# sp-uhh/disentangled-vae

Measured on AMD Instinct MI355X. Metric: spectrogram frames/sec (train step), M2 VAE 513-bin, higher is better.
Workload: dtype bf16x3; 1 GPU; M2 VAE train step (fwd+ELBO+bwd+Adam), x_dim 513, y_dim 513, z 16, h [128,128], 8192 frames/step/GPU, 16 kHz / 1024-pt STFT power frames; parallelism=dp1, min_hbm_bytes_per_frame=4168

## Files before the change

### disentangled-vae_amd/csrc/rows_common.hpp

```cpp
#pragma once
#include "fused_tiles.hpp"
#include "apply_types.hpp"
#include "../../include/dvae_train.h"

namespace dvae {
namespace fused {

__device__ __forceinline__ void philox_normal4(unsigned long long seed, unsigned long long frame, unsigned long long step, unsigned draw,
                                               float (&out)[4]) {
    unsigned c0 = (unsigned)frame, c1 = (unsigned)(frame >> 32), c2 = (unsigned)step, c3 = ((unsigned)(step >> 32) << 8) | draw;
    unsigned k0 = (unsigned)seed, k1 = (unsigned)(seed >> 32);
#pragma unroll
    for (int r = 0; r < 10; ++r) {
        const unsigned h0 = __umulhi(0xD2511F53u, c0), l0 = 0xD2511F53u * c0;
        const unsigned h1 = __umulhi(0xCD9E8D57u, c2), l1 = 0xCD9E8D57u * c2;
        c0 = h1 ^ c1 ^ k0; c1 = l1; c2 = h0 ^ c3 ^ k1; c3 = l0;
        k0 += 0x9E3779B9u; k1 += 0xBB67AE85u;
    }
    const float u0 = ((float)(c0 >> 8) + 0.5f) * (1.f / 16777216.f), u1 = ((float)(c1 >> 8) + 0.5f) * (1.f / 16777216.f);
    const float u2 = ((float)(c2 >> 8) + 0.5f) * (1.f / 16777216.f), u3 = ((float)(c3 >> 8) + 0.5f) * (1.f / 16777216.f);
    const float ra = sqrtf(-2.f * __logf(u0)), rb = sqrtf(-2.f * __logf(u2));
    float sa, ca, sb, cb;
    __sincosf(6.283185307179586f * u1, &sa, &ca);
    __sincosf(6.283185307179586f * u3, &sb, &cb);
    out[0] = ra * ca; out[1] = ra * sa; out[2] = rb * cb; out[3] = rb * sb;
}
__device__ __forceinline__ void frame_noise8(unsigned long long seed, unsigned long long frame, unsigned long long step, int h, float (&e)[8]) {
    float a[4], b[4];
    philox_normal4(seed, frame, step, 2u * h, a);
    philox_normal4(seed, frame, step, 2u * h + 1u, b);
#pragma unroll
    for (int j = 0; j < 4; ++j) { e[j] = a[j]; e[4 + j] = b[j]; }
}

struct RowsArgs {
    const float* x; const float* y; const float* eps;
    int ldx, ldy, ydim;
    int fastx, fasty;
    int64_t B, Bp;
    unsigned long long rng_seed, rng_step;
    const int64_t* rows;
    int64_t n_rows;
    int* bad_rows;
    int ntiles;
    float invB, elbo_eps;
    const void *W1s, *W2s, *Wmvs, *W3s, *W4s, *W5s, *W5t, *W4t, *W3zt, *Wmvt, *W2t;
    const float *b1, *b2, *bmu, *blv, *b3, *b4, *b5;
    const float* w5last;
    void *xT, *yT, *h1T, *h2T, *dh1T, *dh2T, *dmlvT, *zT, *d1T, *d2T, *dd1T, *dd2T, *daT;
    const void* wcopy; int64_t wcopy_bytes;
    int64_t spl;
    unsigned wpl_bytes;
    const void *Wc1s, *Wc2s, *Wc2t, *Wa1s, *Wa1t, *Wa2s, *Wa2t;
    const float *bc1, *bc2, *wc3, *bc3, *ba1, *ba2, *wa3, *ba3;
    void *c1T, *c2T, *dc1T, *dc2T, *dc3T, *a1T, *a2T, *da1T, *da2T, *da3T;
    float alpha, beta, gamma;
    int mode;
    float *out_r, *out_mu, *out_lv, *out_z;
    const float *g_r, *g_mu, *g_lv, *g_z;
    int ld_r, ld_gr;
    double* partials;
    unsigned long long* dbg;
    int ablate;
    int stash_inputs;
    unsigned* ylo_epoch; unsigned launch_id; int ylo_skip; int* ylo_dirty;
    DeferArgs defer;
};

#ifdef DVAE_FINE_STAMPS
#define DVAE_FSTAMP(i) do { if (g.dbg && tid == 0) g.dbg[(size_t)blockIdx.x * 32 + (i)] = wall_clock64(); } while (0)
#else
#define DVAE_FSTAMP(i) do { } while (0)
#endif
#define DVAE_STAMP(i) do { if (g.dbg && tid == 0) g.dbg[(size_t)blockIdx.x * 32 + (i)] = wall_clock64(); } while (0)


typedef short s16x4 __attribute__((ext_vector_type(4)));
__device__ __forceinline__ s16x4 lds_tr16(const __bf16* p) {
    return __builtin_amdgcn_ds_read_tr16_b64_v4i16((__attribute__((address_space(3))) s16x4*)(p));
}

#ifndef R2_STASH_AUX
#define R2_STASH_AUX 16
#endif
template <typename Frag>
__device__ __forceinline__ void stash_store16(void* base_uniform, int voff_bytes, const Frag& f) {
#if R2_STASH_AUX == 0
    *reinterpret_cast<Frag*>((char*)base_uniform + voff_bytes) = f;
#else
    typedef unsigned int u32x4_ __attribute__((ext_vector_type(4)));
    const __amdgpu_buffer_rsrc_t rs = __builtin_amdgcn_make_buffer_rsrc(base_uniform, 0, 0x7fffffff, 0x00020000);
    __builtin_amdgcn_raw_buffer_store_b128(__builtin_bit_cast(u32x4_, f), rs, voff_bytes, 0, R2_STASH_AUX);
#endif
}

template <typename P, bool SRC16 = false>
__device__ __forceinline__ void stash_tile(const typename P::T* lds, int ldl, int fbase, typename P::T* stash_tile_ptr, int64_t spl,
                                           int64_t b0, int l31, int h, float scale = 1.f, int col_limit = 1 << 30, int nplanes = P::NP) {
    typedef typename P::T T;
    typedef typename P::Frag Frag;
    constexpr int E = P::E;
    if (stash_tile_ptr == nullptr) return;
    T* const dbase = stash_tile_ptr + (b0 / P::KSTEP) * (64 * E);
    if constexpr (sizeof(T) == 2) {
        const int i16 = l31 & 15, q = i16 >> 2, pp = i16 & 3, cg = l31 >> 4;
        const T* blk = lds + q * ldl + fbase + 16 * cg + 4 * pp;
        const bool keep = fbase + l31 < col_limit;
        typedef short s16x8 __attribute__((ext_vector_type(8)));
#pragma unroll
        for (int i = 0; i < TB / (2 * E); ++i) {
            const int gq = h + 2 * i;
            Frag f[P::NP];
#pragma unroll
            for (int pl = 0; pl < P::NP; ++pl) {
                const T* bp = blk + pl * Pl<P>::lds;
                const s16x4 r0 = lds_tr16(bp + (8 * gq) * ldl), r1 = lds_tr16(bp + (8 * gq + 4) * ldl);
                s16x8 raw = {r0[0], r0[1], r0[2], r0[3], r1[0], r1[1], r1[2], r1[3]};
                f[pl] = __builtin_bit_cast(Frag, raw);
            }
            if constexpr (SRC16 && P::NP == 2) {
#pragma unroll
                for (int j = 0; j < E; ++j) {
                    const float v = (X16::val(f[0][j]) + X16::val(f[1][j])) * X16::XINV;
                    f[0][j] = P::cvt(v); f[1][j] = P::cvt(v - (float)f[0][j]);
                }
            } else
            if (scale != 1.f) {
#pragma unroll
                for (int j = 0; j < E; ++j) {
                    if constexpr (P::NP == 2) {
                        const float v = ((float)f[0][j] + (float)f[1][j]) * scale;
                        f[0][j] = P::cvt(v); f[1][j] = P::cvt(v - (float)f[0][j]);
                    } else f[0][j] = P::cvt((float)f[0][j] * scale);
                }
            }
            if (!keep) {
#pragma unroll
                for (int pl = 0; pl < P::NP; ++pl)
#pragma unroll
                    for (int j = 0; j < E; ++j) f[pl][j] = P::cvt(0.f);
            }
            stash_store16(dbase, (l31 * E + gq * 32 * E) * (int)sizeof(T), f[0]);
            if constexpr (P::NP == 2) { if (nplanes == 2) stash_store16(dbase + spl, (l31 * E + gq * 32 * E) * (int)sizeof(T), f[1]); }
        }
    } else {
#pragma unroll
        for (int i = 0; i < TB / (2 * E); ++i) {
            const int gq = h + 2 * i;
            Frag f;
#pragma unroll
            for (int j = 0; j < E; ++j) {
                const T v = lds[(gq * E + j) * ldl + fbase + l31];
                f[j] = scale == 1.f ? v : P::cvt((float)v * scale);
                if (fbase + l31 >= col_limit) f[j] = P::cvt(0.f);
            }
            stash_store16(dbase, (l31 * E + gq * 32 * E) * (int)sizeof(T), f);
        }
    }
}

template <typename P, bool F16 = false, typename RowOf>
__device__ __forceinline__ void load_rows_to_lds(const float* __restrict__ src, int ld, int ncols, int pcols, int64_t b0, int64_t B,
                                                 typename P::T* U, int ldu, int tid, RowOf rowof, float* xf = nullptr,
                                                 float* log2sum = nullptr, float eps = 0.f) {
    const int total = TB * pcols;
    for (int idx = tid; idx < total; idx += 256) {
        const int row = idx / pcols, col = idx - row * pcols;
        float v = 0.f;
        if (col < ncols && b0 + row < B) {
            v = src[rowof(row) * ld + col];
            if (log2sum && col < XD - 1) *log2sum += __builtin_amdgcn_logf(v + eps);
        }
        if constexpr (F16 && P::NP == 2) {
            const float vs = v * X16::XS;
            const typename P::T vh = X16::hi<typename P::T>(vs);
            U[row * ldu + col] = vh;
            U[Pl<P>::lds + row * ldu + col] = X16::hi<typename P::T>(vs - X16::val(vh));
        } else {
            const typename P::T vh = P::cvt(v);
            U[row * ldu + col] = vh;
            if constexpr (P::NP == 2) U[Pl<P>::lds + row * ldu + col] = P::cvt(v - (float)vh);
        }
        if (xf && col < ncols) xf[row * ncols + col] = v;
    }
}

constexpr int NQ513 = 17;
struct __attribute__((packed, aligned(4))) F4U { f32x4 v; };
#ifndef R2_IN_NT
#define R2_IN_NT 0
#endif
typedef f32x4 f32x4_a4 __attribute__((aligned(4)));
__device__ __forceinline__ f32x4 ld_in4(const float* p) {
#if R2_IN_NT >= 1
    return __builtin_nontemporal_load(reinterpret_cast<const f32x4_a4*>(p));
#else
    return reinterpret_cast<const F4U*>(p)->v;
#endif
}
__device__ __forceinline__ f32x4 ld_in4_again(const float* p) {
#if R2_IN_NT >= 2
    return __builtin_nontemporal_load(reinterpret_cast<const f32x4_a4*>(p));
#else
    return reinterpret_cast<const F4U*>(p)->v;
#endif
}
template <int I0, int I1, typename RowOf>
__device__ __forceinline__ void tile513_issue_part(const float* __restrict__ base, RowOf rowof, f32x4 (&v)[NQ513], int tid) {
#pragma unroll
    for (int i = I0; i < I1; ++i) {
        const int c = tid + 256 * i;
        v[i] = ld_in4(base + rowof(c >> 7) * XD + 4 * (c & 127));
    }
}
template <typename RowOf>
__device__ __forceinline__ void tile513_issue_last(const float* __restrict__ base, RowOf rowof, f32x4 (&v)[NQ513], int tid) {
    v[16][0] = base[rowof(tid & 31) * XD + XD - 1];
}
template <typename RowOf>
__device__ __forceinline__ void tile513_issue(const float* __restrict__ base, RowOf rowof, f32x4 (&v)[NQ513], int tid) {
    tile513_issue_part<0, 16>(base, rowof, v, tid);
    tile513_issue_last(base, rowof, v, tid);
    __builtin_amdgcn_sched_barrier(0);
}
template <typename P, int I0, int I1, bool F16 = false>
__device__ __forceinline__ void tile513_commit_part(const f32x4 (&v)[NQ513], typename P::T* U, int ldu, int tid, float* xf, unsigned long long& lo_bits) {
    typedef typename P::Pack4 Pack4;
#pragma unroll
    for (int i = I0; i < I1; ++i) {
        const int c = tid + 256 * i;
        const int row = c >> 7, col = 4 * (c & 127);
        if (xf) {
            float* d = xf + row * XD + col;
            d[0] = v[i][0]; d[1] = v[i][1]; d[2] = v[i][2]; d[3] = v[i][3];
        }
        if constexpr (F16 && P::NP == 2) {
            Pack4 pk, pl;
#pragma unroll
            for (int j = 0; j < 4; ++j) {
                const float vs = v[i][j] * X16::XS;
                pk[j] = X16::hi<typename P::T>(vs);
                pl[j] = X16::hi<typename P::T>(vs - X16::val(pk[j]));
            }
            *reinterpret_cast<Pack4*>(U + row * ldu + col) = pk;
            *reinterpret_cast<Pack4*>(U + Pl<P>::lds + row * ldu + col) = pl;
            continue;
        }
        Pack4 pk;
        pk[0] = P::cvt(v[i][0]); pk[1] = P::cvt(v[i][1]); pk[2] = P::cvt(v[i][2]); pk[3] = P::cvt(v[i][3]);
        *reinterpret_cast<Pack4*>(U + row * ldu + col) = pk;
        if constexpr (P::NP == 2) {
            Pack4 pl;
            pl[0] = P::cvt(v[i][0] - (float)pk[0]); pl[1] = P::cvt(v[i][1] - (float)pk[1]);
            pl[2] = P::cvt(v[i][2] - (float)pk[2]); pl[3] = P::cvt(v[i][3] - (float)pk[3]);
            *reinterpret_cast<Pack4*>(U + Pl<P>::lds + row * ldu + col) = pl;
            lo_bits |= __builtin_bit_cast(unsigned long long, pl) & 0x7fff7fff7fff7fffull;
        }
    }
}
template <typename P, int PCOLS, bool F16 = false>
__device__ __forceinline__ void tile513_commit_last(const f32x4 (&v)[NQ513], typename P::T* U, int ldu, int tid, float* xf, unsigned long long& lo_bits) {
    constexpr int PADC = PCOLS - XD;
    if (tid < TB) {
        if (xf) xf[tid * XD + XD - 1] = v[16][0];
        if constexpr (F16 && P::NP == 2) {
            const float vs = v[16][0] * X16::XS;
            const typename P::T vh = X16::hi<typename P::T>(vs);
            U[tid * ldu + XD - 1] = vh;
            U[Pl<P>::lds + tid * ldu + XD - 1] = X16::hi<typename P::T>(vs - X16::val(vh));
        } else {
        const typename P::T vh = P::cvt(v[16][0]);
        U[tid * ldu + XD - 1] = vh;
        if constexpr (P::NP == 2) {
            const typename P::T vl = P::cvt(v[16][0] - (float)vh);
            U[Pl<P>::lds + tid * ldu + XD - 1] = vl;
            if ((float)vl != 0.f) lo_bits |= 1ull;
        }
        }
    }
    for (int idx = tid; idx < TB * PADC; idx += 256) {
        const int r = idx / PADC, c = XD + idx - r * PADC;
        U[r * ldu + c] = P::cvt(0.f);
        if constexpr (P::NP == 2) U[Pl<P>::lds + r * ldu + c] = P::cvt(0.f);
    }
}
template <typename P, int PCOLS, bool F16 = false>
__device__ __forceinline__ void tile513_commit(const f32x4 (&v)[NQ513], typename P::T* U, int ldu, int tid, float* xf = nullptr, bool* any_lo = nullptr) {
    unsigned long long lo_bits = 0ull;
    tile513_commit_part<P, 0, 16, F16>(v, U, ldu, tid, xf, lo_bits);
    tile513_commit_last<P, PCOLS, F16>(v, U, ldu, tid, xf, lo_bits);
    if (any_lo) *any_lo = lo_bits != 0ull;
}
template <typename P, int Q0, int Q1, typename RowOf>
__device__ __forceinline__ void xstash_reload(const float* __restrict__ src, int ld, RowOf rowof, int64_t b0, int64_t B, typename P::T* xT,
                                              int64_t spl, int64_t Bp, int tid) {
    typedef typename P::Frag Frag;
    static_assert(P::NP == 2 && P::E == 8, "x stash by reload: split-bf16 planes");
    if (xT == nullptr) return;
    const int w = tid >> 6, lane = tid & 63;
    int64_t ro[8];
    bool live[8];
#pragma unroll
    for (int k = 0; k < 8; ++k) { ro[k] = rowof(8 * w + k) * (int64_t)ld; live[k] = b0 + 8 * w + k < B; }
    const int64_t kst = (b0 / P::KSTEP + (w >> 1)) * (64 * P::E) + (w & 1) * 32 * P::E;
    float v[Q1 - Q0][8];
#pragma unroll
    for (int q = Q0; q < Q1; ++q)
#pragma unroll
        for (int k = 0; k < 8; ++k) {
            const int f = 64 * q + lane;
            v[q - Q0][k] = src[ro[k] + (f < XD ? f : XD - 1)];
        }
    __builtin_amdgcn_sched_barrier(0);
#pragma unroll
    for (int q = Q0; q < Q1; ++q) {
        const int f = 64 * q + lane;
        if (q == 8 && lane >= 32) continue;
        Frag fh, fl;
#pragma unroll
        for (int k = 0; k < 8; ++k) {
            const float x = (f < XD && live[k]) ? v[q - Q0][k] : 0.f;
            fh[k] = P::cvt(x);
            fl[k] = P::cvt(x - (float)fh[k]);
        }
        const int64_t o = (int64_t)(f >> 5) * 32 * Bp + kst + (f & 31) * P::E;
        stash_store16(xT, (int)(o * (int64_t)sizeof(typename P::T)), fh);
        stash_store16(xT + spl, (int)(o * (int64_t)sizeof(typename P::T)), fl);
    }
}
__device__ __forceinline__ float tile513_log2sum(const f32x4 (&v)[NQ513], float eps, int tid) {
    float s0 = 0.f, s1 = 0.f;
#pragma unroll
    for (int i = 0; i < 16; ++i) {
        s0 += __builtin_amdgcn_logf(v[i][0] + eps) + __builtin_amdgcn_logf(v[i][1] + eps);
        s1 += __builtin_amdgcn_logf(v[i][2] + eps) + __builtin_amdgcn_logf(v[i][3] + eps);
    }
    return s0 + s1;
}

template <typename P, bool SRC16 = false>
__device__ __forceinline__ void stash_from_lds(const typename P::T* U, int ldu, int pcols, int srows, typename P::T* stash, int64_t spl,
                                               int64_t Bp, int64_t b0, int tid, int ft0 = 0, int ft1 = 1 << 30, int nplanes = P::NP) {
    typedef typename P::Frag Frag;
    constexpr int E = P::E;
    if constexpr (sizeof(typename P::T) == 2) {
        const int lane = tid & 63, wave = __builtin_amdgcn_readfirstlane(tid >> 6);
        const int fte = ft1 < srows / 32 ? ft1 : srows / 32;
        for (int ft = ft0 + wave; ft < fte; ft += 4)
            stash_tile<P, SRC16>(U, ldu, 32 * ft, stash + (int64_t)ft * 32 * Bp, spl, b0, lane & 31, lane >> 5, 1.f, pcols, nplanes);
        return;
    }
    constexpr int groups = TB / E;
    const int total = srows * groups;
    for (int idx = tid; idx < total; idx += 256) {
        const int gi = idx / srows, f = idx - gi * srows;
        Frag p;
#pragma unroll
        for (int j = 0; j < E; ++j) p[j] = (f < pcols) ? U[(gi * E + j) * ldu + f] : P::cvt(0.f);
        *reinterpret_cast<Frag*>(stash + (int64_t)(f >> 5) * 32 * Bp + (b0 / P::KSTEP) * (64 * E) + (gi * 32 + (f & 31)) * E) = p;
    }
}


static int current_device() { int dev = 0; (void)hipGetDevice(&dev); return dev < 0 || dev >= 64 ? 0 : dev; }
static inline bool is_bf(int precision) { return precision == DVAE_PREC_BF16 || precision == DVAE_PREC_BF16X3; }
template <typename F>
static auto with_policy(int precision, F&& f) {
    if (precision == DVAE_PREC_BF16X3) return f(PolX3{});
    if (precision == DVAE_PREC_BF16) return f(PolBF16{});
    return f(PolF32{});
}

int launch_rows1(int precision, int model, int y_dim, const RowsArgs& a, int grid, hipStream_t s);
int launch_noise(unsigned long long seed, unsigned long long step, int64_t B, float* out, hipStream_t s);
int launch_rows2(int precision, int model, int y_dim, const RowsArgs& a, int grid, hipStream_t s);
bool rows2_supported(int precision, int model);
int launch_rows3(int model, int y_dim, const RowsArgs& a, int grid, hipStream_t s);
bool rows3_supported(int precision, int model);

}
}
```

### disentangled-vae_amd/csrc/rows_helper.inc

```
        const int hw = wave_u - ROWS_CHAIN_WAVES, ht = tid - 64 * ROWS_CHAIN_WAVES;
        constexpr bool XFH = P::XF16 && NP == 2;
        constexpr int NBT = Ld<T>::nbias;
        constexpr int NB = (NBT + 255) / 256;
        float bvv[NB];
        auto load_bias = [&]() __attribute__((always_inline)) {
#pragma unroll
            for (int q = 0; q < NB; ++q) {
                int i = ht + 256 * q;
                i = i < NBT ? i : NBT - 1;
                const float* src;
                int k;
                if (i < OB2) { src = g.b1; k = i; }
                else if (i < OBMV) { src = g.b2; k = i - OB2; }
                else if (i < OBMV + ZD) { src = g.bmu; k = i - OBMV; }
                else if (i < OB3) { src = g.blv; k = i - OBMV - ZD; }
                else if (i < OB4) { src = g.b3; k = i - OB3; }
                else if (i < OB5) { src = g.b4; k = i - OB4; }
                else if (i < OB5 + NO) { src = g.b5; k = i - OB5; k = k < XD ? k : XD - 1; }
                else { src = g.w5last; k = i - OB5 - NO; }
                if constexpr (DEFER) bvv[q] = __hip_atomic_load(src + k, __ATOMIC_RELAXED, __HIP_MEMORY_SCOPE_AGENT);
                else bvv[q] = src[k];
            }
        };
        auto store_bias = [&]() __attribute__((always_inline)) {
#pragma unroll
            for (int q = 0; q < NB; ++q) {
                const int i = ht + 256 * q;
                if (i < NBT) Bias[i] = (i >= OB5 + XD && i < OB5 + NO) ? 0.f : bvv[q];
            }
        };
        if constexpr (!DEFER) load_bias();
        auto fill_rows = [&](int tl_, int half) {
            if (ht < TB) {
                const int64_t bf = (int64_t)tl_ * TB + ht;
                const int64_t br = bf < g.B ? bf : g.B - 1;
                int64_t r = g.rows[br];
                if (r < 0 || r >= g.n_rows) { r = 0; if (g.bad_rows && bf < g.B) atomicAdd(g.bad_rows, 1); }
                rowsrc[half * TB + ht] = r;
            }
        };
        typedef Sched<P, YP, YENC, (OFFL ? P::PDO : P::PD), INFO> SCc;
        typedef HSched<P, YP, YENC, DH, INFO> HS;
        typedef WStream<P, HS, DH> HWS;
        HWS hws;
        if constexpr (HS::any) {
            hws.rs = __builtin_amdgcn_make_buffer_rsrc(const_cast<void*>(g.wcopy), 0, (int)g.wcopy_bytes, 0x00020000);
            hws.voff = lane * 16;
            hws.pl = g.wpl_bytes;
            auto mo = [&](const void* Wp) { return (unsigned)((const char*)Wp - (const char*)g.wcopy); };
            constexpr unsigned FBB = HS::FBB;
            const unsigned tw = (unsigned)hw * FBB;
            hws.sb[H_W1X] = mo(g.W1s) + tw + (unsigned)SCc::NX1 * 4u * FBB;
            hws.sb[H_W3Y] = mo(g.W3s) + tw + (unsigned)(ZD / KS) * 4u * FBB;
            hws.sb[H_W3Z] = mo(g.W3s) + tw;
            hws.sb[H_PAD] = mo(g.W1s);
            if constexpr (INFO) { hws.sb[H_C1] = mo(g.Wc1s) + tw;  hws.sb[H_C2] = mo(g.Wc2s) + tw;  hws.sb[H_C2T] = mo(g.Wc2t) + tw; }
            else { hws.sb[H_C1] = hws.sb[H_C2] = hws.sb[H_C2T] = 0; }
            if constexpr (INFO) hws.fill();
        }
        const T* const Urh = U + l31 * LDU + h * E;
        const T* const Zbrh = Zb + l31 * LDZ + h * E;
        float lsum2 = 0.f;
        f32x4 xv[NQ513], yv[NQ513];
        bool x_in_regs = false;
        bool y_in_regs = false;
        const bool st1 = MODE != 1 && !(g.ablate & 1), st2 = MODE != 1 && !(g.ablate & 2) && (g.stash_inputs & 2), st2x = MODE != 1 && !(g.ablate & 2) && (g.stash_inputs & 1);
        for (int it = 0; it < ntl; ++it) {
            const int tile = tile0 + it * (int)gridDim.x;
            const int64_t b0 = (int64_t)tile * TB;
            const bool full = (b0 + TB) <= g.B;
            const int64_t* const rsrc = rowsrc + (it & 1) * TB;
            auto rowof = [&](int r) -> int64_t {
                if (gather) return rsrc[r];
                const int64_t br = b0 + r;
                return br < g.B ? br : g.B - 1;
            };
            int tl = ht;
            asm volatile("" : "+v"(tl));
            const bool yfast = Y513 && g.fasty && full;
            bool y_early = it > 0 && y_in_regs;
            if (it == 0) {
                if (gather) { fill_rows(tile, 0); wg_barrier(); }
                if (g.fastx && full) {
                    tile513_issue(g.x, rowof, xv, tl);
                    if constexpr (!DEFER) store_bias();
#if R2_EARLY_Y
                    if (YP > 0 && Y513 && g.fasty) {
                        unsigned long long lb = 0ull;
                        static_for<0, 4>([&](auto qc) {
                            constexpr int Q = decltype(qc)::value;
                            tile513_issue_part<4 * Q, 4 * Q + 4>(g.y, rowof, yv, tl);
                            __builtin_amdgcn_sched_barrier(0);
                            tile513_commit_part<P, 4 * Q, 4 * Q + 4, XFH>(xv, U, LDU, tl, nullptr, lb);
                            __builtin_amdgcn_sched_barrier(0);
                        });
                        tile513_issue_last(g.y, rowof, yv, tl);
                        __builtin_amdgcn_sched_barrier(0);
                        tile513_commit_last<P, ROWS_XP, XFH>(xv, U, LDU, tl, nullptr, lb);
                        y_early = true;
                    } else
#endif
                    {
                        tile513_commit<P, ROWS_XP, XFH>(xv, U, LDU, tl);
#pragma unroll
                        for (int i = 0; i < NQ513; ++i) yv[i] = f32x4{0.f, 0.f, 0.f, 0.f};
                    }
                } else {
#pragma unroll
                    for (int i = 0; i < NQ513; ++i) { xv[i] = f32x4{0.f, 0.f, 0.f, 0.f}; yv[i] = f32x4{0.f, 0.f, 0.f, 0.f}; }
                    if constexpr (!DEFER) store_bias();
                    load_rows_to_lds<P, XFH>(g.x, g.ldx, XD, ROWS_XP, b0, g.B, U, LDU, tl, rowof, nullptr, OFFL ? &lsum2 : nullptr, g.elbo_eps);
                }
                if constexpr (INFO) {
                    for (int i = ht; i < 6 * HD + 2; i += 256) {
                        const int q = i / HD, k = i - q * HD;
                        float v;
                        if (q == 0) v = g.bc1[k]; else if (q == 1) v = g.bc2[k]; else if (q == 2) v = g.wc3[k];
                        else if (q == 3) v = g.ba1[k]; else if (q == 4) v = g.ba2[k]; else if (q == 5) v = g.wa3[k];
                        else v = k == 0 ? g.bc3[0] : g.ba3[0];
                        Binfo[i] = v;
                    }
                }
                if (ht == 0) flags[0] = 0;
                if constexpr (DEFER) {
                    wg_barrier();
                    load_bias();
                    store_bias();
                }
                wg_barrier();
                if constexpr (OFFL) { if (g.fastx && full) lsum2 += tile513_log2sum(xv, g.elbo_eps, tl); }
            }
            if constexpr (HS::n(H_W1X) > 0) {
                f32x16 hacc;
                zero_acc<P>(hacc);
                hws.fill();
                gemm_seg<P, HS, DH, H_W1X, HWS, XFH>(hacc, hws, Urh + SCc::NX1 * 2 * E);
#pragma unroll
                for (int r = 0; r < 16; ++r) keep[r * 256 + ht] = XFH ? hacc[r] * X16::ACC : hacc[r];
            }
            float c1r[16], c2r[16], w3c[16];
            float bce_c = 0.f, ylab = 0.f;
            if constexpr (INFO) {
                ylab = g.y[rowof(l31) * g.ldy];
                if (it > 0) hws.fill();
                f32x16 cacc;
                zero_acc<P>(cacc);
                gemm_seg<P, HS, DH, H_C1, HWS, XFH>(cacc, hws, Urh);
                float bvc[16];
                bias16(Binfo + OBC1, 32 * hw, h, bvc);
#pragma unroll
                for (int r = 0; r < 16; ++r) c1r[r] = fmaxf((XFH ? cacc[r] * X16::ACC : cacc[r]) + bvc[r], 0.f);
            }
            f32x16 accy;
            int yplanes = NP;
            int ydirty = 0;
            if constexpr (NP == 2 && YP > 0) { if (g.ylo_skip && st2) ydirty = g.ylo_dirty[tile]; }
            if (YP > 0) {
                if (Y513 && yfast && !y_early) tile513_issue(g.y, rowof, yv, tl);
                R2_HSTAMP(16);
                if (st2x && !XFH) stash_from_lds<P>(U, LDU, ROWS_XP, NO, (T*)g.xT, g.spl, g.Bp, b0, tl);
                R2_HSTAMP(17);
                wg_barrier();
                if constexpr (HS::HELPY && HS::n(H_W1X) == 0) hws.fill();
                R2_HSTAMP(18);
                bool any = false;
                if (Y513 && yfast) tile513_commit<P, ROWS_XP>(yv, U, LDU, tl, nullptr, NP == 2 ? &any : nullptr);
                else load_rows_to_lds<P>(g.y, g.ldy, g.ydim, YP, b0, g.B, U, LDU, tl, rowof);
                R2_HSTAMP(19);
                if constexpr (NP == 2) {
                    if (Y513 && yfast) {
                    } else {
                        constexpr int YPD = YP > 0 ? YP : 1;
                        for (int idx = tl; idx < TB * YP; idx += 256) any |= (float)U[Pl<P>::lds + (idx / YPD) * LDU + idx % YPD] != 0.f;
                    }
                    if (__ballot(any) != 0ull && lane == 0) atomicOr(&flags[0], 1);
                }
                R2_HSTAMP(20);
                if constexpr (INFO) put_lds<P>(c1r, U + IMA, LDU, 32 * hw, l31, h);
                wg_barrier();
                if constexpr (NP == 2) {
                    const bool ylo_t = __builtin_amdgcn_readfirstlane(flags[0]) != 0;
                    if (g.ylo_skip && st2) {
                        ydirty = __builtin_amdgcn_readfirstlane(ydirty);
                        yplanes = (ylo_t || ydirty != 0) ? 2 : 1;
                        if (ht == 0) {
                            if (ylo_t) *g.ylo_epoch = g.launch_id;
                            if ((ylo_t ? 1 : 0) != ydirty) g.ylo_dirty[tile] = ylo_t ? 1 : 0;
                        }
                    }
                }
#if !R2_LATE_Y
                if (st2) stash_from_lds<P>(U, LDU, YP, (YP + 31) / 32 * 32, (T*)g.yT, g.spl, g.Bp, b0, tl, 0, 1 << 30, yplanes);
#endif
                if constexpr (HS::HELPY) {
                    const bool ylo = NP == 2 && __builtin_amdgcn_readfirstlane(flags[0]) != 0;
                    zero_acc<P>(accy);
                    if (!R2_YLOSEG) gemm_seg<P, HS, DH, H_W3Y>(accy, hws, Urh, ylo);
                    else if (ylo) gemm_seg<P, HS, DH, H_W3Y>(accy, hws, Urh, true);
                    else gemm_seg<P, HS, DH, H_W3Y>(accy, hws, Urh, false);
                }
                if constexpr (INFO) {
                    f32x16 a2c;
                    zero_acc<P>(a2c);
                    gemm_seg<P, HS, DH, H_C2>(a2c, hws, Urh + IMA);
                    float bvc[16];
                    bias16(Binfo + OBC2, 32 * hw, h, bvc);
                    bias16(Binfo + OWC3, 32 * hw, h, w3c);
                    float pd = 0.f;
#pragma unroll
                    for (int r = 0; r < 16; ++r) { c2r[r] = fmaxf(a2c[r] + bvc[r], 0.f); pd = fmaf(w3c[r], c2r[r], pd); }
                    put_lds<P>(c2r, U + IMB, LDU, 32 * hw, l31, h);
                    pd += __shfl_xor(pd, 32, 64);
                    if (h == 0) red2[hw * 32 + l31] = pd;
                }
            } else {
                if (st2x && !XFH) stash_from_lds<P>(U, LDU, ROWS_XP, NO, (T*)g.xT, g.spl, g.Bp, b0, tl);
                if constexpr (HS::n(H_W1X) > 0) wg_barrier();
            }
            wg_barrier();
            if constexpr (INFO) {
                const bool live_h = (b0 + l31) < g.B;
                const float logit = red2[l31] + red2[32 + l31] + red2[64 + l31] + red2[96 + l31] + Binfo[OS3];
                const float p = 1.f / (1.f + P::exp_(-logit));
                const float lp = P::log_(p + g.elbo_eps), lq = P::log_(1.f - p + g.elbo_eps);
                bce_c = (live_h && h == 0 && hw == 0) ? -(ylab * lp + (1.f - ylab) * lq) : 0.f;
                const float u = live_h ? -g.invB * (ylab / (p + g.elbo_eps) - (1.f - ylab) / (1.f - p + g.elbo_eps)) : 0.f;
                const float dpre3 = u * p * (1.f - p);
                float dv2[16];
#pragma unroll
                for (int r = 0; r < 16; ++r) dv2[r] = c2r[r] > 0.f ? w3c[r] * dpre3 : 0.f;
                put_lds<P>(dv2, U + IMC, LDU, 32 * hw, l31, h);
                if (st1) {
                    stash_tile<P>(U + IMA, LDU, 32 * hw, (T*)g.c1T + (int64_t)hw * 32 * g.Bp, g.spl, b0, l31, h);
                    stash_tile<P>(U + IMB, LDU, 32 * hw, (T*)g.c2T + (int64_t)hw * 32 * g.Bp, g.spl, b0, l31, h);
                    if (hw == 0 && h == 0) {
                        T* d3 = (T*)g.dc3T + (b0 / KS) * (64 * E) + (l31 / E) * 32 * E + (l31 % E);
                        const T d3h = P::cvt(dpre3 * g.alpha);
                        *d3 = d3h;
                        if constexpr (NP == 2) d3[g.spl] = P::cvt(dpre3 * g.alpha - (float)d3h);
                    }
                }
            }
            if (st1) stash_tile<P>(Ha, LDH, 32 * hw, (T*)g.h1T + (int64_t)hw * 32 * g.Bp, g.spl, b0, l31, h);
#ifndef R2_XSP
#define R2_XSP 1
#endif
            if constexpr (XFH && !INFO && R2_XSP == 0) { if (st2x) xstash_reload<P, 0, 4>(g.x, g.ldx, rowof, b0, g.B, (T*)g.xT, g.spl, g.Bp, tl); }
#if R2_LATE_Y
            if (YP > 0 && st2) stash_from_lds<P>(U, LDU, YP, (YP + 31) / 32 * 32, (T*)g.yT, g.spl, g.Bp, b0, tl, 0, R2_YSPREAD, yplanes);
#endif
            wg_barrier();
            if constexpr (INFO) {
                f32x16 a3c;
                zero_acc<P>(a3c);
                gemm_seg<P, HS, DH, H_C2T>(a3c, hws, Urh + IMC);
                float dv1[16];
#pragma unroll
                for (int r = 0; r < 16; ++r) dv1[r] = c1r[r] > 0.f ? a3c[r] : 0.f;
                put_lds<P>(dv1, U + IMA, LDU, 32 * hw, l31, h);
                if (st1) stash_tile<P>(U + IMC, LDU, 32 * hw, (T*)g.dc2T + (int64_t)hw * 32 * g.Bp, g.spl, b0, l31, h, g.alpha);
            }
            if (st1) stash_tile<P>(Hb, LDH, 32 * hw, (T*)g.h2T + (int64_t)hw * 32 * g.Bp, g.spl, b0, l31, h);
            if constexpr (XFH && !INFO) {
                if (st2x) {
                    if constexpr (R2_XSP == 0) xstash_reload<P, 4, 9>(g.x, g.ldx, rowof, b0, g.B, (T*)g.xT, g.spl, g.Bp, tl);
                    else if constexpr (R2_XSP == 1) xstash_reload<P, 0, 9>(g.x, g.ldx, rowof, b0, g.B, (T*)g.xT, g.spl, g.Bp, tl);
                    else xstash_reload<P, 0, 5>(g.x, g.ldx, rowof, b0, g.B, (T*)g.xT, g.spl, g.Bp, tl);
                }
            }
#if R2_LATE_Y
            if (YP > 0 && st2) stash_from_lds<P>(U, LDU, YP, (YP + 31) / 32 * 32, (T*)g.yT, g.spl, g.Bp, b0, tl, R2_YSPREAD, 1 << 30, yplanes);
#endif
            wg_barrier();
            if constexpr (HS::HELPY) {
                f32x16 az;
                zero_acc<P>(az);
                gemm_seg<P, HS, DH, H_W3Z>(az, hws, Zbrh);
                float hv[16], bv[16];
                bias16(Bias + OB3, 32 * hw, h, bv);
#pragma unroll
                for (int r = 0; r < 16; ++r) hv[r] = P::tanh_(az[r] + accy[r] + bv[r]);
                put_lds<P>(hv, Ha, LDH, 32 * hw, l31, h);
            }
            if (hw == 0 && st1) stash_tile<P>(Zb, LDZ, 0, (T*)g.zT, g.spl, b0, l31, h);
            if constexpr (XFH && !INFO && R2_XSP == 2) { if (st2x) xstash_reload<P, 5, 9>(g.x, g.ldx, rowof, b0, g.B, (T*)g.xT, g.spl, g.Bp, tl); }
            if (ht == 0) flags[0] = 0;
            if constexpr (INFO) {
                if (st1) stash_tile<P>(U + IMA, LDU, 32 * hw, (T*)g.dc1T + (int64_t)hw * 32 * g.Bp, g.spl, b0, l31, h, g.alpha);
                const float sa = g.gamma - g.beta;
                wg_barrier();
                if (st1) stash_tile<P>(Ha, LDH, 32 * hw, (T*)g.a1T + (int64_t)hw * 32 * g.Bp, g.spl, b0, l31, h);
                if constexpr (XFH) { if (st2x) xstash_reload<P, 0, 5>(g.x, g.ldx, rowof, b0, g.B, (T*)g.xT, g.spl, g.Bp, tl); }
                wg_barrier();
                if (st1) {
                    stash_tile<P>(Hb, LDH, 32 * hw, (T*)g.a2T + (int64_t)hw * 32 * g.Bp, g.spl, b0, l31, h);
                    if (hw == 0 && h == 0) {
                        const bool live_h = (b0 + l31) < g.B;
                        const float logit = red2[l31] + red2[32 + l31] + red2[64 + l31] + red2[96 + l31] + Binfo[OS3 + 1];
                        const float p = 1.f / (1.f + P::exp_(-logit));
                        const float u = live_h ? -g.invB * (ylab / (p + g.elbo_eps) - (1.f - ylab) / (1.f - p + g.elbo_eps)) : 0.f;
                        const float dpre3 = u * p * (1.f - p);
                        T* d3 = (T*)g.da3T + (b0 / KS) * (64 * E) + (l31 / E) * 32 * E + (l31 % E);
                        const T d3h = P::cvt(dpre3 * sa);
                        *d3 = d3h;
                        if constexpr (NP == 2) d3[g.spl] = P::cvt(dpre3 * sa - (float)d3h);
                    }
                }
                wg_barrier();
                if (st1) stash_tile<P>(Ha, LDH, 32 * hw, (T*)g.da2T + (int64_t)hw * 32 * g.Bp, g.spl, b0, l31, h, sa);
                if constexpr (XFH) { if (st2x) xstash_reload<P, 5, 9>(g.x, g.ldx, rowof, b0, g.B, (T*)g.xT, g.spl, g.Bp, tl); }
                wg_barrier();
                if (st1) stash_tile<P>(Hb, LDH, 32 * hw, (T*)g.da1T + (int64_t)hw * 32 * g.Bp, g.spl, b0, l31, h, sa);
            }
            wg_barrier();
            int lo_ = lane;
            asm volatile("" : "+v"(lo_));
            const int l31o = lo_ & 31, ho = lo_ >> 5;
            const float* const xrow_o = g.x + rowof(l31o) * g.ldx + 4 * ho;
            f32x4 xo[4], xnx[4];
            if constexpr (OFFL) {
#pragma unroll
                for (int gq = 0; gq < 4; ++gq) xo[gq] = ld_in4_again(xrow_o + 32 * hw + 8 * gq);
            }
            if (st1) stash_tile<P>(Ha, LDH, 32 * hw, (T*)g.d1T + (int64_t)hw * 32 * g.Bp, g.spl, b0, l31, h);
            wg_barrier();
            if (st1) stash_tile<P>(Hb, LDH, 32 * hw, (T*)g.d2T + (int64_t)hw * 32 * g.Bp, g.spl, b0, l31, h);
            float rec_h = 0.f;
            if constexpr (OFFL) {
                const bool live = (b0 + l31o) < g.B;
                const float invB_l = live ? g.invB : 0.f;
                const float* const xrow = xrow_o;
#pragma unroll 1
                for (int I = 0; I < 4; ++I) {
                    const int t = hw + 4 * I;
                    if (I < 3) {
#pragma unroll
                        for (int gq = 0; gq < 4; ++gq) xnx[gq] = ld_in4_again(xrow + 32 * (t + 4) + 8 * gq);
                    }
                    R2_HSTAMP(21 + 2 * I);
                    wg_barrier();
                    R2_HSTAMP(22 + 2 * I);
#if R2_HPRIO
                    __builtin_amdgcn_s_setprio(R2_HPRIO);
#endif
#pragma unroll
                    for (int gq = 0; gq < 4; ++gq) {
                        float a4[4], da4[4];
                        get_raw4<P>(a4, U, LDU, 32 * t + 8 * gq + 4 * ho, l31o);
#pragma unroll
                        for (int j = 0; j < 4; ++j) {
                            const float xe = xo[gq][j] * __builtin_amdgcn_exp2f(a4[j] * -1.44269504088896341f);
                            rec_h += xe;
                            rec_h += a4[j];
                            da4[j] = fmaf(-xe, invB_l, invB_l);
                        }
                        typename P::Pack4 ph, pl;
#pragma unroll
                        for (int j = 0; j < 4; ++j) { ph[j] = P::cvt(da4[j]); pl[j] = P::cvt(da4[j] - (float)ph[j]); }
                        *reinterpret_cast<typename P::Pack4*>(U + l31o * LDU + 32 * t + 8 * gq + 4 * ho) = ph;
                        *reinterpret_cast<typename P::Pack4*>(U + Pl<P>::lds + l31o * LDU + 32 * t + 8 * gq + 4 * ho) = pl;
                    }
#if R2_HPRIO
                    __builtin_amdgcn_s_setprio(0);
#endif
#pragma unroll
                    for (int gq = 0; gq < 4; ++gq) xo[gq] = xnx[gq];
                }
                rec_h = live ? rec_h - 64.f : 0.f;
            }
            wg_barrier();
            for (int t = hw; t < NT_OUT; t += 4) if (st1) stash_tile<P>(U, LDU, 32 * t, (T*)g.daT + (int64_t)t * 32 * g.Bp, g.spl, b0, l31, h);
            const bool more = it + 1 < ntl;
            const int ntile = tile + (int)gridDim.x;
            if (more && gather) fill_rows(ntile, (it + 1) & 1);
            wg_barrier();
            if (MODE == 1) {
                if (more) {
                    const int64_t fb0 = (int64_t)ntile * TB;
                    const int64_t* const fsrc = rowsrc + ((it + 1) & 1) * TB;
                    auto frowof = [&](int r) -> int64_t {
                        if (gather) return fsrc[r];
                        const int64_t br = fb0 + r;
                        return br < g.B ? br : g.B - 1;
                    };
                    if (g.fastx && (fb0 + TB) <= g.B) { tile513_issue(g.x, frowof, xv, tl); tile513_commit<P, ROWS_XP, XFH>(xv, U, LDU, tl); }
                    else load_rows_to_lds<P, XFH>(g.x, g.ldx, XD, ROWS_XP, fb0, g.B, U, LDU, tl, frowof);
                }
                wg_barrier();
                continue;
            }
            if (st1) stash_tile<P>(Hb, LDH, 32 * hw, (T*)g.dd2T + (int64_t)hw * 32 * g.Bp, g.spl, b0, l31, h);
            const int64_t nb0 = (int64_t)ntile * TB;
            const bool nfull = more && (nb0 + TB) <= g.B;
            const int64_t* const nsrc = rowsrc + ((it + 1) & 1) * TB;
            auto nrowof = [&](int r) -> int64_t {
                if (gather) return nsrc[r];
                const int64_t br = nb0 + r;
                return br < g.B ? br : g.B - 1;
            };
            x_in_regs = ROWS_PREFETCH && more && g.fastx && nfull;
            if (x_in_regs) tile513_issue(g.x, nrowof, xv, tl);
            else {
#pragma unroll
                for (int i = 0; i < NQ513; ++i) xv[i] = f32x4{0.f, 0.f, 0.f, 0.f};
            }
            wg_barrier();
            if (st1) stash_tile<P>(Ha, LDH, 32 * hw, (T*)g.dd1T + (int64_t)hw * 32 * g.Bp, g.spl, b0, l31, h);
            wg_barrier();
            if constexpr (YP > 0 && Y513) {
                y_in_regs = ROWS_PREFETCH && more && g.fasty && nfull;
                if (y_in_regs) tile513_issue(g.y, nrowof, yv, tl);
                else {
#pragma unroll
                    for (int i = 0; i < NQ513; ++i) yv[i] = f32x4{0.f, 0.f, 0.f, 0.f};
                }
            }
            if (hw == 0 && st1) stash_tile<P>(Zb, LDZ, 0, (T*)g.dmlvT, g.spl, b0, l31, h);
            wg_barrier();
            if (st1) stash_tile<P>(Hb, LDH, 32 * hw, (T*)g.dh2T + (int64_t)hw * 32 * g.Bp, g.spl, b0, l31, h);
            wg_barrier();
            if (st1) stash_tile<P>(Ha, LDH, 32 * hw, (T*)g.dh1T + (int64_t)hw * 32 * g.Bp, g.spl, b0, l31, h);
            if constexpr (OFFL) {
                const float rs = wave_sum(rec_h), ls = wave_sum(lsum2);
                if (lane == 0) { red[8 + hw] = rs; red[12 + hw] = ls; }
                lsum2 = 0.f;
            }
            if constexpr (INFO) { if (hw == 0) { const float bcs = wave_sum(bce_c); if (lane == 0) red2[128] = bcs; } }
            if (more) {
                if (x_in_regs) {
                    tile513_commit<P, ROWS_XP, XFH>(xv, U, LDU, tl);
                    if constexpr (OFFL) lsum2 = tile513_log2sum(xv, g.elbo_eps, tl);
                } else if (!ROWS_PREFETCH && g.fastx && nfull) {
                    tile513_issue(g.x, nrowof, xv, tl);
                    tile513_commit<P, ROWS_XP, XFH>(xv, U, LDU, tl);
                    if constexpr (OFFL) lsum2 = tile513_log2sum(xv, g.elbo_eps, tl);
                } else load_rows_to_lds<P, XFH>(g.x, g.ldx, XD, ROWS_XP, nb0, g.B, U, LDU, tl, nrowof, nullptr, OFFL ? &lsum2 : nullptr, g.elbo_eps);
            }
            wg_barrier();
        }
// ... 1 lines not shown
```

### disentangled-vae_amd/csrc/train_fused.hip

```cpp
#include <atomic>
#include <mutex>
#include <unordered_map>
#include <vector>
#include <map>
#include <algorithm>
#include <tuple>
#include <math.h>
#include <stdlib.h>
#include "fused_tiles.hpp"
#include "rows_common.hpp"
#include "wgrad_types.hpp"
#include "../../include/dvae_train.h"

namespace dvae {
namespace fused {

struct Layout {
    int64_t W1s, W2s, Wmvs, W3s, W4s, W5s, W5t, W4t, W3zt, Wmvt, W2t, wcopy_elems;
    int64_t Wc1s, Wc2s, Wc2t, Wa1s, Wa1t, Wa2s, Wa2t;
    int64_t c1T, c2T, dc1T, dc2T, dc3T, a1T, a2T, da1T, da2T, da3T;
    bool info;
    int ld1, ld3, yp, ye, yd;
    int64_t xT, yT, h1T, h2T, dh1T, dh2T, dmlvT, zT, d1T, d2T, dd1T, dd2T, daT, stash_rows;
    int64_t o_tiles, o_blocks, o_blocks4, o_items4, o_tensors, o_chunks, o_partials, o_flags, o_defer, o_wcopy, o_stash, o_grads, total;
    int ntiles, nblocks, nblocks4;
};
constexpr int DEFER_MAX_TASKS = 640;
constexpr int64_t DEFER_O_SHARD = (int64_t)DEFER_MAX_TASKS * (int64_t)sizeof(DeferTask);
constexpr int64_t DEFER_O_DONE = DEFER_O_SHARD + DEFER_SHARDS * 128;
constexpr int64_t DEFER_BYTES = DEFER_O_DONE + 128;

static inline int64_t al(int64_t v, int64_t a) { return (v + a - 1) / a * a; }

static inline int planes_of(int precision) { return precision == DVAE_PREC_BF16X3 ? 2 : 1; }

static int make_layout(const dvae_train_plan_t& p, Layout& L) {
    const int esz = is_bf(p.precision) ? 2 : 4;
    const int np = planes_of(p.precision);
    L.yp = p.y_dim == 0 ? 0 : (p.y_dim + 15) / 16 * 16;
    L.ye = p.model == DVAE_MODEL_M2 ? L.yp : 0;
    L.info = p.model == DVAE_MODEL_M2_INFO;
    L.yd = L.yp;
    const bool r3 = p.rows_kernel == 3;
    const int yk = p.y_dim == 0 ? 0 : (r3 ? (p.y_dim + 31) / 32 * 32 : L.yp);
    L.ld1 = (r3 ? 544 : XP) + (L.ye ? yk : 0);
    L.ld3 = (r3 ? 32 : ZD) + (L.yd ? yk : 0);
    int64_t o = 0;
    auto take = [&](int64_t n) { int64_t r = o; o += al(n, 128); return r; };
    L.W1s = take((int64_t)HD * L.ld1); L.W2s = take(HD * HD); L.Wmvs = take(32 * HD); L.W3s = take((int64_t)HD * L.ld3);
    L.W4s = take(HD * HD); L.W5s = take((int64_t)NO * HD); L.W5t = take((int64_t)HD * NO); L.W4t = take(HD * HD);
    L.W3zt = take(32 * HD); L.Wmvt = take(HD * 32); L.W2t = take(HD * HD);
    if (L.info) {
        L.Wc1s = take((int64_t)HD * XP); L.Wc2s = take(HD * HD); L.Wc2t = take(HD * HD);
        L.Wa1s = take(HD * ZD); L.Wa1t = take(32 * HD); L.Wa2s = take(HD * HD); L.Wa2t = take(HD * HD);
    }
    L.wcopy_elems = o;
    int64_t r = 0;
    auto rows = [&](int64_t n) { int64_t q = r; r += n; return q; };
    L.xT = rows(NO); L.yT = rows(L.yp ? al(L.yp, 32) : 0); L.h1T = rows(HD); L.h2T = rows(HD); L.dh1T = rows(HD); L.dh2T = rows(HD);
    L.dmlvT = rows(32); L.zT = rows(32); L.d1T = rows(HD); L.d2T = rows(HD); L.dd1T = rows(HD); L.dd2T = rows(HD); L.daT = rows(NO);
    if (L.info) {
        L.c1T = rows(HD); L.c2T = rows(HD); L.dc1T = rows(HD); L.dc2T = rows(HD); L.dc3T = rows(32);
        L.a1T = rows(HD); L.a2T = rows(HD); L.da1T = rows(HD); L.da2T = rows(HD); L.da3T = rows(32);
    }
    rows(32);
    L.stash_rows = r;
    const int nty = L.yp ? (int)(al(L.yp, 32) / 32) : 0;
    auto pr = [](int n) { return (n + 1) / 2; };
    L.ntiles = 2 * pr(NT_OUT + (L.ye ? nty : 0)) + 2 * 2 + 1 * 2 + 2 * pr(1 + (L.yd ? nty : 0)) + 2 * 2 + pr(NT_OUT) * 2;
    if (L.info) L.ntiles += 2 * pr(NT_OUT) + 2 * 2 + 1 * 2 + 2 * 1 + 2 * 2 + 1 * 2;
    auto q4 = [](int n) { return (n + 3) / 4; };
    L.nblocks = q4(4) * q4(NT_OUT + (L.ye ? nty : 0)) + 1 + 1 + q4(4) * q4(1 + (L.yd ? nty : 0)) + 1 + q4(NT_OUT) * 1;
    if (L.info) L.nblocks += q4(NT_OUT) + 1 + 1 + 1 + 1 + 1;
    L.nblocks4 = q4(4) * (q4(NT_OUT) + (L.ye ? q4(nty) : 0)) + 1 + 1 + q4(4) * (1 + (L.yd ? q4(nty) : 0)) + 1 + q4(NT_OUT) * 1;
    if (L.info) L.nblocks4 += q4(NT_OUT) + 1 + 1 + 1 + 1 + 1;
    int64_t b = 0;
    auto bytes = [&](int64_t n) { int64_t q = b; b += al(n, 256); return q; };
    L.o_tiles = bytes((int64_t)L.ntiles * sizeof(GroupDesc));
    L.o_blocks = bytes((int64_t)L.nblocks * sizeof(BlockDesc));
    L.o_blocks4 = bytes((int64_t)L.nblocks4 * sizeof(Block4));
    L.o_items4 = bytes((int64_t)3 * W4_MAX_ITEMS * sizeof(W4Item));
    L.o_tensors = bytes(DVAE_TRAIN_MAX_TENSORS * sizeof(TensorDesc));
    L.o_chunks = bytes(p.n_params / 64 + 64);
    L.o_partials = bytes(p.rows_grid * 4 * sizeof(double));
    L.o_flags = bytes(1024 + 4 * (p.Bp / TB + 1));
    L.o_defer = bytes(DEFER_BYTES);
    L.o_wcopy = bytes(L.wcopy_elems * esz * np);
    L.o_stash = bytes(L.stash_rows * p.Bp * esz * np);
    L.o_grads = bytes((int64_t)p.ksplit * p.n_params * sizeof(float));
    L.total = b;
    return 0;
}

static bool g_prof = false;
static unsigned long long* g_dbg = nullptr;
static double g_ms[4] = {0, 0, 0, 0};
static int64_t g_calls[4] = {0, 0, 0, 0};
struct PendingEv { hipEvent_t a, b; int which; };
static PendingEv g_pending[4096];
static int g_npending = 0;

struct ProfScope {
    hipStream_t s; int which; hipEvent_t a, b; bool on;
    __attribute__((noinline)) ProfScope(hipStream_t s_, int w) : s(s_), which(w), on(g_prof && g_npending < 4096) {
        if (on) { (void)hipEventCreate(&a); (void)hipEventCreate(&b); (void)hipEventRecord(a, s); }
    }
    ~ProfScope() {
        if (on) { (void)hipEventRecord(b, s); g_pending[g_npending++] = PendingEv{a, b, which}; }
    }
};

}
}

using namespace dvae;
using namespace dvae::fused;

static int env_int(const char* name, int dflt) { const char* v = getenv(name); return v ? atoi(v) : dflt; }
static long long env_ll(const char* name, long long dflt) { const char* v = getenv(name); return v ? atoll(v) : dflt; }
static int wgrad_form_env(bool* set = nullptr) {
    const char* wk = getenv("DVAE_WGRAD");
    if (set) *set = wk != nullptr;
    if (wk && strcmp(wk, "ring") == 0) return 2;
    if (wk && strcmp(wk, "lds") == 0) return 1;
    return 4;
}

static void w4_plan_classes(dvae_train_plan_t* plan, bool grouped);
constexpr int W4_GROUPED = 0x40000000;

extern "C" int dvae_train_plan(int model, int y_dim, int precision, int64_t B, int ksplit_hint, dvae_train_plan_t* plan) {
    DVAE_CHECK_ARG(plan != nullptr && B > 0, "train_plan: bad argument");
    if (!((model == DVAE_MODEL_M1 && y_dim == 0) || (model == DVAE_MODEL_M2 && (y_dim == 1 || y_dim == 513)) ||
          (model == DVAE_MODEL_M2_INFO && y_dim == 1) || (model == DVAE_MODEL_M2_DEC && y_dim == 1))) {
        set_error("train_plan: fused kernels cover M1 (y 0), M2 (y 1 or 513), M2_info and M2_DEC (y 1) at x 513 / h [128,128] / z 16; got model %d y_dim %d", model, y_dim);
        return DVAE_E_UNSUPPORTED;
    }
    DVAE_CHECK_ARG(precision == DVAE_PREC_F32 || precision == DVAE_PREC_BF16 || precision == DVAE_PREC_BF16X3, "train_plan: unknown precision %d", precision);
    memset(plan, 0, sizeof(*plan));
    plan->model = model; plan->y_dim = y_dim; plan->precision = precision; plan->B = B;
    plan->Bp = al(B, 128);
    const int ye = model == DVAE_MODEL_M2 ? y_dim : 0, yd = y_dim;
    const int rows[26] = {HD, HD, HD, HD, ZD, ZD, ZD, ZD, HD, HD, HD, HD, XD, XD,
                          HD, HD, HD, HD, 1, 1, HD, HD, HD, HD, 1, 1};
    const int cols[26] = {XD + ye, 1, HD, 1, HD, 1, HD, 1, ZD + yd, 1, HD, 1, HD, 1,
                          XD, 1, HD, 1, HD, 1, ZD, 1, HD, 1, HD, 1};
    int64_t off = 0;
    plan->n_tensors = model == DVAE_MODEL_M2_INFO ? 26 : 14;
    for (int i = 0; i < plan->n_tensors; ++i) {
        plan->tensor_offset[i] = off; plan->tensor_rows[i] = rows[i]; plan->tensor_cols[i] = cols[i];
        off += al((int64_t)rows[i] * cols[i], 64);
    }
    plan->n_params = off;
    const int64_t ntiles = (B + TB - 1) / TB;
    int want = env_int("DVAE_ROWS", 2);
    if (want < 1 || want > 3) want = 2;
    plan->rows_kernel = (want == 3 && rows3_supported(precision, model)) ? 3 : ((want >= 2 && rows2_supported(precision, model)) ? 2 : 1);
    if (!kDiagBuild && plan->rows_kernel == 1 && is_bf(precision)) {
        set_error("train_plan: DVAE_ROWS=1 (the 4-wave rows kernel) under the bf16 policies needs the diagnostic build (build.py --diag)");
        return DVAE_E_UNSUPPORTED;
    }
    if (model == DVAE_MODEL_M2_DEC && plan->rows_kernel != 2) {
        set_error("train_plan: M2_DEC exists in the 8-wave rows kernel only (bf16 / bf16x3 operands, DVAE_ROWS unset)");
        return DVAE_E_UNSUPPORTED;
    }
    const int64_t maxg = plan->rows_kernel >= 2 ? 256 : 256 * (precision == DVAE_PREC_BF16 ? 2 : 1);
    plan->rows_grid = ntiles < maxg ? ntiles : maxg;
    int ks = ksplit_hint;
    const bool wg4 = wgrad_form_env() == 4;
    if (ks <= 0 && wg4) {
        dvae_train_plan_t tmp = *plan;
        tmp.ksplit = 1;
        Layout L0;
        make_layout(tmp, L0);
        ks = 256 / L0.nblocks4;
        if (ks > plan->Bp / 128) ks = (int)(plan->Bp / 128);
        if (ks > 16) ks = 16;
        if (ks < 1) ks = 1;
    }
    if (ks <= 0) {
        const int cap = precision == DVAE_PREC_BF16X3 ? 12 : (is_bf(precision) ? (plan->Bp > 12288 ? 12 : 8) : 16);
        ks = (int)(plan->Bp / (precision == DVAE_PREC_BF16X3 ? 640 : (is_bf(precision) ? 1024 : 512))); if (ks < 1) ks = 1; if (ks > cap) ks = cap;
    }
    if (ks > 64) ks = 64;
    plan->ksplit = ks;
    plan->reserved0 = 0;
    const bool want_classes = getenv("DVAE_W4_CLASSES") != nullptr ? atoi(getenv("DVAE_W4_CLASSES")) != 0 : !is_bf(precision);
    const bool want_groups = getenv("DVAE_EXCHANGE_GROUPS") != nullptr && atoi(getenv("DVAE_EXCHANGE_GROUPS")) == 2;
    if ((want_classes || want_groups) && ksplit_hint <= 0 && wg4 && plan->Bp > 128 && getenv("DVAE_W4_UNIFORM") == nullptr &&
        getenv("DVAE_FOLD_APPLY") == nullptr && getenv("DVAE_DEFER_APPLY") == nullptr)
        w4_plan_classes(plan, want_groups);
    Layout L;
    make_layout(*plan, L);
    plan->workspace_bytes = L.total;
    plan->grad_offset_bytes = L.o_grads;
    const double mac = (double)HD * (XD + ye) + HD * HD + 2.0 * ZD * HD + (double)HD * (ZD + yd) + HD * HD + (double)XD * HD;
    const double dxm = (double)HD * HD + 2.0 * ZD * HD + (double)ZD * HD + HD * HD + (double)XD * HD;
    double macx = 0.0, dxx = 0.0;
    if (model == DVAE_MODEL_M2_INFO) {
        macx = ((double)HD * XD + HD * HD + HD) + 2.0 * ((double)HD * ZD + HD * HD + HD);
        dxx = ((double)HD * HD + HD) + ((double)HD * HD + HD + (double)ZD * HD);
    }
    plan->flops_per_step = 2.0 * (2.0 * mac + dxm) * (double)B + 2.0 * (2.0 * macx + dxx) * (double)B;
    plan->info_alpha = 0.0; plan->info_beta = 10.0; plan->info_gamma = 1.0;
    plan->min_hbm_bytes_per_step = 4.0 * (XD + y_dim + ZD) * (double)B;
    return 0;
}

static int64_t kper_of(const dvae_train_plan_t* p) {
    const int ks = is_bf(p->precision) ? 16 : 8;
    const int64_t unit = 4 * ks;
    return al((p->Bp + p->ksplit - 1) / p->ksplit, unit);
}

struct ABlock { int64_t row; int mvalid; int tensor; int m0; int bias_tensor; int tensor_hi; int bias_hi; };
struct BBlock { int64_t row; int nvalid; int col; int kind; int scol; int sncols; };

template <typename T>
static void fill_tables(const dvae_train_plan_t* p, const Layout& L, char* ws_dev, GroupDesc* groups, BlockDesc* blocks, Block4* blocks4, TensorDesc* td) {
    const int64_t Bp = p->Bp;
    T* stash = (T*)(ws_dev + L.o_stash);
    auto S = [&](int64_t row) { return (const void*)(stash + row * Bp); };
    int n = 0;
    ABlock ab[64];
    BBlock bb[64];
    int na = 0, nb = 0;
    auto addA = [&](int64_t row0, int M, int tensor, int bias_tensor) {
        for (int m0 = 0; m0 < M; m0 += 32) ab[na++] = ABlock{row0 + m0, M - m0 < 32 ? M - m0 : 32, tensor, m0, bias_tensor, -1, -1};
    };
    auto addB = [&](int64_t row0, int N, int col0, int kind = 0) {
        for (int n0 = 0; n0 < N; n0 += 32) bb[nb++] = BBlock{row0 + n0, N - n0 < 32 ? N - n0 : 32, col0 + n0, kind, n0, N};
    };
    int nblk = 0, nblk4 = 0, layer_id = 0;
    auto make_group = [&](int i, int j) {
        GroupDesc d;
        memset(&d, 0, sizeof(d));
        d.bias_off[0] = d.bias_off[1] = -1;
        if (i >= na || j >= nb) return d;
        for (int ii = 0; ii < 2; ++ii) {
            if (i + ii >= na) continue;
            const ABlock& a = ab[i + ii];
            d.A[ii] = S(a.row);
            d.ldo[ii] = p->tensor_cols[a.tensor];
            d.mvalid[ii] = a.mvalid;
            if (a.bias_tensor >= 0 && j == 0) d.bias_off[ii] = p->tensor_offset[a.bias_tensor] + a.m0;
            for (int jj = 0; jj < 2; ++jj) {
                if (j + jj >= nb) continue;
                d.out_off[ii][jj] = p->tensor_offset[a.tensor] + (int64_t)a.m0 * d.ldo[ii] + bb[j + jj].col;
                if (ii == 0 && a.tensor_hi >= 0) d.out_off_hi[jj] = p->tensor_offset[a.tensor_hi] + bb[j + jj].col;
            }
            if (ii == 0 && a.tensor_hi >= 0) {
                d.split16 = 1;
                d.ldo_hi = p->tensor_cols[a.tensor_hi];
                d.bias_off_hi = p->tensor_offset[a.bias_hi];
            }
        }
        for (int jj = 0; jj < 2; ++jj) {
            if (j + jj >= nb) continue;
            d.Bm[jj] = S(bb[j + jj].row);
            d.nvalid[jj] = bb[j + jj].nvalid;
        }
        return d;
    };
    auto emit = [&]() {
        for (int i = 0; i < na; i += 2)
            for (int j = 0; j < nb; j += 2) groups[n++] = make_group(i, j);
        for (int i0 = 0; i0 < na; i0 += 4)
            for (int j0 = 0; j0 < nb; j0 += 4) {
                BlockDesc b;
                memset(&b, 0, sizeof(b));
                for (int k = 0; k < 4; ++k) {
                    b.At[k] = i0 + k < na ? S(ab[i0 + k].row) : nullptr;
                    b.Bt[k] = j0 + k < nb ? S(bb[j0 + k].row) : nullptr;
                }
                for (int wr = 0; wr < 2; ++wr)
                    for (int wc = 0; wc < 2; ++wc) b.g[wr * 2 + wc] = make_group(i0 + 2 * wr, j0 + 2 * wc);
                blocks[nblk++] = b;
            }
        for (int r0 = 0; r0 < nb;) {
            int r1 = r0;
            while (r1 < nb && bb[r1].kind == bb[r0].kind) ++r1;
            for (int i0 = 0; i0 < na; i0 += 4)
                for (int j0 = r0; j0 < r1; j0 += 4) {
                    Block4 q;
                    memset(&q, 0, sizeof(q));
                    q.layer = layer_id;
                    q.raw = bb[r0].kind; q.rncols = bb[r0].sncols;
                    for (int k = 0; k < 4; ++k) {
                        q.bias_off[k] = -1;
                        if (i0 + k < na) {
                            const ABlock& a = ab[i0 + k];
                            q.At[k] = S(a.row);
                            q.ldo[k] = p->tensor_cols[a.tensor];
                            q.a_off[k] = p->tensor_offset[a.tensor] + (int64_t)a.m0 * q.ldo[k];
                            q.mvalid[k] = a.mvalid;
                            q.wt[k] = a.tensor; q.bt[k] = a.bias_tensor >= 0 ? a.bias_tensor : 0;
                            if (a.bias_tensor >= 0 && j0 == 0) q.bias_off[k] = p->tensor_offset[a.bias_tensor] + a.m0;
                            if (k == 0 && a.tensor_hi >= 0) {
                                q.wt_hi = a.tensor_hi; q.bt_hi = a.bias_hi;
                                q.split16 = 1;
                                q.ldo_hi = p->tensor_cols[a.tensor_hi];
                                q.a_off_hi = p->tensor_offset[a.tensor_hi];
                                q.bias_off_hi = p->tensor_offset[a.bias_hi];
                            }
                        }
                        if (j0 + k < r1) {
                            q.Bt[k] = S(bb[j0 + k].row);
                            q.bcol[k] = bb[j0 + k].col;
                            q.nvalid[k] = bb[j0 + k].nvalid;
                            q.rcol[k] = bb[j0 + k].scol;
                        }
                    }
                    blocks4[nblk4++] = q;
                }
            r0 = r1;
        }
        na = 0; nb = 0;
        ++layer_id;
    };
    const int ye = p->model == DVAE_MODEL_M2 ? p->y_dim : 0, yd = p->y_dim;
    addA(L.dh1T, HD, 0, 1); addB(L.xT, XD, 0, 1); if (ye) addB(L.yT, ye, XD, 2); emit();
    addA(L.dh2T, HD, 2, 3); addB(L.h1T, HD, 0); emit();
    ab[na++] = ABlock{L.dmlvT, 32, 4, 0, 5, 6, 7}; addB(L.h2T, HD, 0); emit();
    addA(L.dd1T, HD, 8, 9); addB(L.zT, ZD, 0); if (yd) addB(L.yT, yd, ZD, 2); emit();
    addA(L.dd2T, HD, 10, 11); addB(L.d1T, HD, 0); emit();
    addA(L.daT, XD, 12, 13); addB(L.d2T, HD, 0); emit();
    if (L.info) {
        addA(L.dc1T, HD, 14, 15); addB(L.xT, XD, 0, 1); emit();
        addA(L.dc2T, HD, 16, 17); addB(L.c1T, HD, 0); emit();
        addA(L.dc3T, 1, 18, 19); addB(L.c2T, HD, 0); emit();
        addA(L.da1T, HD, 20, 21); addB(L.zT, ZD, 0); emit();
        addA(L.da2T, HD, 22, 23); addB(L.a1T, HD, 0); emit();
        addA(L.da3T, 1, 24, 25); addB(L.a2T, HD, 0); emit();
    }
    if (n != L.ntiles || nblk != L.nblocks || nblk4 != L.nblocks4) { fprintf(stderr, "dvae: internal group / block count mismatch %d vs %d, %d vs %d, %d vs %d\n", n, L.ntiles, nblk, L.nblocks, nblk4, L.nblocks4); }
    for (int i = 0; i < p->n_tensors; ++i) {
        TensorDesc t;
        memset(&t, 0, sizeof(t));
        t.off = p->tensor_offset[i]; t.rows = p->tensor_rows[i]; t.cols = p->tensor_cols[i];
        t.sf_off = -1; t.st_off = -1; t.sf_split = 1 << 30;
        td[i] = t;
    }
    td[0].sf_ld = L.ld1; td[2].sf_ld = HD; td[4].sf_ld = HD; td[6].sf_ld = HD; td[8].sf_ld = L.ld3; td[10].sf_ld = HD; td[12].sf_ld = HD;
    td[2].st_ld = HD; td[4].st_ld = 32; td[6].st_ld = 32; td[8].st_ld = HD; td[10].st_ld = HD; td[12].st_ld = NO;
    td[0].sf_off = L.W1s; td[0].sf_nt = 4; td[0].sf_split = XD; td[0].sf_gap = XP - XD;
    const int f16c = (p->precision == DVAE_PREC_BF16X3 && p->rows_kernel >= 2 && PolX3v2::XF16) ? XD : 0;
    td[0].sf_f16_cols = f16c;
    td[2].sf_off = L.W2s; td[2].sf_nt = 4; td[2].st_off = L.W2t; td[2].st_nt = 4; td[2].st_cmax = HD;
    td[4].sf_off = L.Wmvs; td[4].sf_nt = 1; td[4].st_off = L.Wmvt; td[4].st_nt = 4; td[4].st_cmax = HD;
    td[6].sf_off = L.Wmvs; td[6].sf_nt = 1; td[6].sf_roff = 16; td[6].st_off = L.Wmvt; td[6].st_nt = 4; td[6].st_roff = 16; td[6].st_cmax = HD;
    td[8].sf_off = L.W3s; td[8].sf_nt = 4; td[8].st_off = L.W3zt; td[8].st_nt = 1; td[8].st_cmax = ZD;
    td[10].sf_off = L.W4s; td[10].sf_nt = 4; td[10].st_off = L.W4t; td[10].st_nt = 4; td[10].st_cmax = HD;
    td[12].sf_off = L.W5s; td[12].sf_nt = NT_OUT; td[12].st_off = L.W5t; td[12].st_nt = 4; td[12].st_cmax = HD;
    if (p->rows_kernel == 3) {
        for (int i = 0; i < 14; ++i) td[i].kind16 = 1;
        td[0].sf_nt = 8; td[0].sf_gap = 544 - XD;
        td[2].sf_nt = 8; td[2].st_nt = 8;
        td[4].sf_nt = 2; td[4].rowmap = 1; td[4].st_nt = 8;
        td[6].sf_nt = 2; td[6].rowmap = 2; td[6].sf_roff = 0; td[6].st_nt = 8;
        td[8].sf_nt = 8; td[8].sf_split = ZD; td[8].sf_gap = 32 - ZD; td[8].st_nt = 2; td[8].trowmap = 1;
        td[10].sf_nt = 8; td[10].st_nt = 8;
        td[12].sf_nt = NO / 16; td[12].st_nt = 8;
    }
    if (L.info) {
        td[14].sf_off = L.Wc1s; td[14].sf_nt = 4; td[14].sf_ld = XP; td[14].sf_split = XD; td[14].sf_gap = XP - XD; td[14].sf_f16_cols = f16c;
        td[16].sf_off = L.Wc2s; td[16].sf_nt = 4; td[16].sf_ld = HD; td[16].st_off = L.Wc2t; td[16].st_nt = 4; td[16].st_ld = HD; td[16].st_cmax = HD;
        td[20].sf_off = L.Wa1s; td[20].sf_nt = 4; td[20].sf_ld = ZD; td[20].st_off = L.Wa1t; td[20].st_nt = 1; td[20].st_ld = HD; td[20].st_cmax = ZD;
        td[22].sf_off = L.Wa2s; td[22].sf_nt = 4; td[22].sf_ld = HD; td[22].st_off = L.Wa2t; td[22].st_nt = 4; td[22].st_ld = HD; td[22].st_cmax = HD;
    }
}

static std::mutex g_fold_mu;
static std::unordered_map<const void*, unsigned> g_fold_seq;
struct W4Grids { int g[3]; };
static std::unordered_map<const void*, W4Grids> g_w4_grid;
static void w4_grid_put(const void* ws, const W4Grids& grids) { std::lock_guard<std::mutex> lk(g_fold_mu); g_w4_grid[ws] = grids; }
static int w4_grid_get(const void* ws, int table) { std::lock_guard<std::mutex> lk(g_fold_mu); auto it = g_w4_grid.find(ws); return it == g_w4_grid.end() ? -1 : it->second.g[table]; }
static unsigned fold_seq_next(const void* ws) { std::lock_guard<std::mutex> lk(g_fold_mu); return ++g_fold_seq[ws]; }
static void fold_seq_reset(const void* ws) { std::lock_guard<std::mutex> lk(g_fold_mu); g_fold_seq.erase(ws); }

struct PendingUpdate { float* params; float* m; float* v; int step; double lr, beta1, beta2, adam_eps; int n_slabs; };
struct DeferState { bool pending = false; PendingUpdate u{}; unsigned seq_arrive = 0, seq_done = 0; int ntasks = 0; };
static std::mutex g_defer_mu;
static std::unordered_map<const void*, DeferState> g_defer_state;
static DeferState defer_state_get(const void* ws) { std::lock_guard<std::mutex> lk(g_defer_mu); return g_defer_state[ws]; }
static void defer_state_put(const void* ws, const DeferState& st) { std::lock_guard<std::mutex> lk(g_defer_mu); g_defer_state[ws] = st; }
static void defer_state_reset(const void* ws) { std::lock_guard<std::mutex> lk(g_defer_mu); g_defer_state.erase(ws); }
struct DeferRequest { bool on = false, have = false; PendingUpdate u{}; unsigned seq_arrive = 0, seq_done = 0; float* losses3 = nullptr; };

static int build_defer_tasks(const dvae_train_plan_t* p, const TensorDesc* td, DeferTask* out, int cap) {
    int n = 0;
    auto put = [&](int t, int r0, int cbeg, int cend, int kind) { if (n < cap) out[n] = DeferTask{t, r0, cbeg, cend, kind, 0, 0, 0}; ++n; };
    for (int t = 0; t < p->n_tensors; ++t) {
        const int rows = p->tensor_rows[t], cols = p->tensor_cols[t];
        if (td[t].sf_off < 0 && td[t].st_off < 0) {
            for (int e0 = 0; e0 < rows * cols; e0 += 1024) put(t, 0, e0, rows * cols, 1);
            continue;
        }
        const int split = td[t].sf_off >= 0 && td[t].sf_split < cols ? td[t].sf_split : cols;
        for (int r0 = 0; r0 < rows; r0 += 32) {
            for (int cb = 0; cb < split; cb += 32) put(t, r0, cb, split, 0);
            for (int cb = split; cb < cols; cb += 32) put(t, r0, cb, cols, 0);
        }
    }
    return n;
}

static ApplyArgs make_apply_args(const dvae_train_plan_t* plan, const Layout& L, float* params, float* m, float* v, char* ws, int n_slabs,
                                 bool adam, int step, double lr, double beta1, double beta2, double adam_eps, double grad_scale, float* losses3) {
    ApplyArgs a;
    memset(&a, 0, sizeof(a));
    a.p = params; a.m = m; a.v = v;
    a.slabs = (const float*)(ws + L.o_grads); a.slab_stride = plan->n_params; a.nslabs = n_slabs;
    a.tensors = (const TensorDesc*)(ws + L.o_tensors); a.ntensors = plan->n_tensors;
    a.chunk_tensor = (const unsigned char*)(ws + L.o_chunks); a.n_params = plan->n_params;
    a.wcopy = ws + L.o_wcopy; a.wpl = L.wcopy_elems;
    if (adam) {
        const double bc1 = 1.0 - pow(beta1, (double)step), bc2 = 1.0 - pow(beta2, (double)step);
        a.one_minus_b1 = (float)(1.0 - beta1); a.b2 = (float)beta2; a.one_minus_b2 = (float)(1.0 - beta2);
        a.step_size = (float)(lr / bc1); a.bc2_sqrt = (float)sqrt(bc2); a.eps = (float)adam_eps; a.gscale = (float)grad_scale;
    }
    a.partials = (const double*)(ws + L.o_partials); a.npartials = (int)plan->rows_grid; a.B = plan->B; a.losses3 = losses3; a.accum = (double*)(uintptr_t)plan->loss_accum;
    a.info = plan->model == DVAE_MODEL_M2_INFO; a.alpha = (float)plan->info_alpha; a.beta = (float)plan->info_beta; a.gamma = (float)plan->info_gamma;
    return a;
}

static int launch_apply(const dvae_train_plan_t* plan, const Layout& L, float* params, float* m, float* v, char* ws, int n_slabs,
                        bool adam, int step, double lr, double beta1, double beta2, double adam_eps, double grad_scale,
                        float* losses3, hipStream_t s) {
    const ApplyArgs a = make_apply_args(plan, L, params, m, v, ws, n_slabs, adam, step, lr, beta1, beta2, adam_eps, grad_scale, losses3);
    const int ntasks = defer_state_get(ws).ntasks;
    const char* ak = getenv("DVAE_APPLY");
#ifdef DVAE_DIAG
    if (adam && is_bf(plan->precision) && n_slabs <= 12 && ntasks > 0 && ntasks <= DEFER_MAX_TASKS && ak && strcmp(ak, "units") == 0)
        return launch_apply_units(plan->precision, a, (const DeferTask*)(ws + L.o_defer), 4 * ntasks, s);
#else
    (void)ntasks; (void)ak;
#endif
    return launch_apply_kernel(plan->precision, adam, a, s);
}

struct W4Sched { std::vector<W4Item> items; int grid = 0; };

static void w4_host_blocks(const dvae_train_plan_t& p, const Layout& L, std::vector<Block4>& out) {
    std::vector<GroupDesc> tiles((size_t)L.ntiles + 8);
    std::vector<BlockDesc> blocks((size_t)L.nblocks + 8);
    out.assign((size_t)L.nblocks4 + 8, Block4{});
    TensorDesc td[DVAE_TRAIN_MAX_TENSORS];
    memset(td, 0, sizeof(td));
    char* const base = reinterpret_cast<char*>((uintptr_t)1 << 20);
    if (is_bf(p.precision)) fill_tables<__bf16>(&p, L, base, tiles.data(), blocks.data(), out.data(), td);
    else fill_tables<float>(&p, L, base, tiles.data(), blocks.data(), out.data(), td);
    out.resize((size_t)L.nblocks4);
}

static double w4_block_cost(const dvae_train_plan_t& p, const Block4& b) {
    int na = 0, nb = 0;
    bool bias = b.split16 && b.bias_off_hi >= 0;
    for (int k = 0; k < 4; ++k) { if (b.At[k]) na = k + 1; if (b.Bt[k]) nb = k + 1; bias = bias || b.bias_off[k] >= 0; }
    const bool x3 = p.precision == DVAE_PREC_BF16X3, bf = is_bf(p.precision);
    const bool one_plane_b = x3 && b.raw == 2 && p.rows_kernel >= 2;
    double mfma, load, fsum;
    static const double kb_clocks = getenv("DVAE_W4_KB_CLOCKS") ? atof(getenv("DVAE_W4_KB_CLOCKS")) : 70.0;
    if (bf) {
        mfma = (double)na * nb * (x3 ? (one_plane_b ? 2 : 3) : 1) * 32.0;
        load = ((double)na * (x3 ? 2 : 1) + (double)nb * (x3 ? (one_plane_b ? 1 : 2) : 1)) * kb_clocks;
        fsum = bias ? (double)na * (x3 ? 2 : 1) * 16 * 4 * 0.5 : 0.0;
    } else {
        mfma = (double)na * nb * 2 * 4 * 64.0;
        load = (double)(na + nb) * 2 * 70.0;
        fsum = bias ? (double)na * 2 * 8 * 4 * 0.5 : 0.0;
    }
    if (b.raw != 0 && p.B >= 131072 && bf) load *= 2.0;
    return std::max(mfma, load) + 0.3 * std::min(mfma, load) + fsum;
}

static int64_t w4_kper(const dvae_train_plan_t& p, int slices) {
    const int64_t unit = 4 * (is_bf(p.precision) ? 16 : 8);
    return al((p.Bp + slices - 1) / slices, unit);
}

static inline bool w4_classed(const dvae_train_plan_t& p) { return (p.reserved0 & ~W4_GROUPED) > 0; }
static inline bool w4_grouped(const dvae_train_plan_t& p) { return (p.reserved0 & W4_GROUPED) != 0; }
static int used_slabs(const dvae_train_plan_t* plan) {
    if (w4_classed(*plan)) return plan->ksplit;
    const int64_t kper = kper_of(plan);
    return (int)((plan->Bp + kper - 1) / kper);
}
static inline int w4_group_of(const Block4& b) { return b.layer <= 2 ? 1 : 0; }

static void w4_class_slices(const dvae_train_plan_t& p, const std::vector<Block4>& blocks, int max_items, std::vector<int>& s, int group = -1) {
    const int n = (int)blocks.size();
    s.assign(n, 1);
    std::vector<double> cost(n);
    for (int b = 0; b < n; ++b) cost[b] = (group < 0 || w4_group_of(blocks[b]) == group) ? w4_block_cost(p, blocks[b]) : 0.0;
    for (int b = 0; b < n; ++b) if (cost[b] == 0.0) s[b] = 0;
    int cap = (int)std::min<int64_t>(16, p.Bp / 128);
    if (cap < 1) cap = 1;
    int total = 0;
    for (int b = 0; b < n; ++b) total += s[b];
    for (;;) {
        int worst = -1;
        double tw = 0.0;
        for (int b = 0; b < n; ++b) { if (s[b] == 0) continue; const double t = cost[b] * (double)w4_kper(p, s[b]); if (t > tw) { tw = t; worst = b; } }
        if (worst < 0) break;
        int s2 = s[worst] + 1;
        while (s2 <= cap && w4_kper(p, s2) >= w4_kper(p, s[worst])) ++s2;
        if (s2 > cap || total + (s2 - s[worst]) > max_items) break;
        total += s2 - s[worst];
        s[worst] = s2;
    }
}

static void w4_debug_print(const dvae_train_plan_t& p, const std::vector<Block4>& blocks, const std::vector<int>& s) {
    if (getenv("DVAE_W4_DEBUG") == nullptr) return;
    {
        for (int b = 0; b < (int)blocks.size(); ++b) {
            if (s[b] == 0) continue;
            int na = 0, nb = 0;
            for (int k = 0; k < 4; ++k) { if (blocks[b].At[k]) na = k + 1; if (blocks[b].Bt[k]) nb = k + 1; }
            const int64_t kper = w4_kper(p, s[b]);
            fprintf(stderr, "dvae w4: block %2d layer %d %d x %d kind %d bias %d cost %6.0f slices %2d of %lld frames -> %.0f clocks per wave\n", b, blocks[b].layer, na, nb,
                    blocks[b].raw, (int)(blocks[b].bias_off[0] >= 0), w4_block_cost(p, blocks[b]), (int)((p.Bp + kper - 1) / kper), (long long)kper,
                    w4_block_cost(p, blocks[b]) * (double)kper / 64.0);
        }
    }
}

static void w4_plan_classes(dvae_train_plan_t* plan, bool grouped) {
    dvae_train_plan_t tmp = *plan;
    tmp.ksplit = 1;
    Layout L0;
    make_layout(tmp, L0);
    std::vector<Block4> blocks;
    w4_host_blocks(tmp, L0, blocks);
    int nslabs = 1, items_max = 0;
    for (int grp = grouped ? 0 : -1; grp <= (grouped ? 1 : -1); ++grp) {
        std::vector<int> s;
        w4_class_slices(tmp, blocks, 256, s, grp);
        w4_debug_print(tmp, blocks, s);
        int items = 0;
        for (size_t b = 0; b < blocks.size(); ++b) {
            if (s[b] == 0) continue;
            const int64_t kper = w4_kper(tmp, s[b]);
            const int eff = (int)((tmp.Bp + kper - 1) / kper);
            nslabs = std::max(nslabs, eff);
            items += eff;
        }
        items_max = std::max(items_max, items);
    }
    plan->ksplit = nslabs;
    plan->reserved0 = items_max | (grouped ? W4_GROUPED : 0);
}

static void w4_build_items(const dvae_train_plan_t& p, const Layout& L, W4Sched& out, int group = -1) {
    out.items.clear();
    out.grid = 0;
    if (!w4_classed(p)) {
        const int64_t kper = w4_kper(p, p.ksplit);
        const int ks = (int)((p.Bp + kper - 1) / kper), nblocks = L.nblocks4;
        const int a8 = ks >> 3, r8 = ks & 7, npure = a8 * nblocks, per = (r8 * nblocks + 7) >> 3;
        out.grid = 8 * (a8 * nblocks + per);
        for (int w = 0; w < out.grid; ++w) {
            const int xcd = w & 7, j = w >> 3;
            W4Item it{-1, 0, 0, 0};
            if (j < npure) { it.slice = xcd + 8 * (j / nblocks); it.block = j % nblocks; }
            else {
                const int e = xcd * per + (j - npure);
                if (j - npure < per && e < r8 * nblocks) { it.slice = 8 * a8 + e / nblocks; it.block = e % nblocks; }
            }
            if (it.block >= 0) { it.kbeg = (int64_t)it.slice * kper; it.kend = std::min<int64_t>(it.kbeg + kper, p.Bp); }
            out.items.push_back(it);
        }
        return;
    }
    std::vector<Block4> blocks;
    w4_host_blocks(p, L, blocks);
    dvae_train_plan_t tmp = p;
    std::vector<int> s;
    w4_class_slices(tmp, blocks, 256, s, group);
    struct It { W4Item it; double cost; };
    std::map<std::tuple<int, int64_t, int>, std::vector<It>> groups;
    for (int b = 0; b < (int)blocks.size(); ++b) {
        if (s[b] == 0) continue;
        const int64_t kper = w4_kper(p, s[b]);
        const int eff = (int)((p.Bp + kper - 1) / kper);
        const double c = w4_block_cost(p, blocks[b]);
        for (int i = 0; i < eff; ++i) {
            W4Item it{b, i, (int64_t)i * kper, std::min<int64_t>((int64_t)(i + 1) * kper, p.Bp)};
            groups[std::make_tuple(blocks[b].layer, kper, i)].push_back(It{it, c * (double)(it.kend - it.kbeg)});
        }
    }
    std::vector<std::vector<It>> gl;
    for (auto& kv : groups) gl.push_back(kv.second);
    auto gcost = [](const std::vector<It>& g) { double t = 0; for (const It& i : g) t += i.cost; return t; };
    std::stable_sort(gl.begin(), gl.end(), [&](const std::vector<It>& a, const std::vector<It>& b) { return gcost(a) > gcost(b); });
    std::vector<It> lists[8];
    double load[8] = {0, 0, 0, 0, 0, 0, 0, 0};
    const int cap = 32;
    auto lightest = [&](int need) { int best = -1; for (int x = 0; x < 8; ++x) if ((int)lists[x].size() + need <= cap && (best < 0 || load[x] < load[best])) best = x; return best; };
    for (auto& g : gl) {
        int x = lightest((int)g.size());
        if (x >= 0) { for (const It& i : g) { lists[x].push_back(i); load[x] += i.cost; } continue; }
        for (const It& i : g) {
            x = lightest(1);
            if (x < 0) { x = 0; for (int q = 1; q < 8; ++q) if (lists[q].size() < lists[x].size()) x = q; }
            lists[x].push_back(i); load[x] += i.cost;
        }
    }
    size_t maxlen = 0;
    for (int x = 0; x < 8; ++x) {
        std::stable_sort(lists[x].begin(), lists[x].end(), [](const It& a, const It& b) { return a.cost > b.cost; });
        maxlen = std::max(maxlen, lists[x].size());
    }
    out.grid = (int)(8 * maxlen);
    out.items.assign((size_t)out.grid, W4Item{-1, 0, 0, 0});
    for (int x = 0; x < 8; ++x)
        for (size_t q = 0; q < lists[x].size(); ++q) out.items[q * 8 + x] = lists[x][q].it;
}

extern "C" int dvae_train_repack(const dvae_train_plan_t* plan, const float* params, void* ws, void* stream) {
    DVAE_CHECK_ARG(plan && params && ws, "train_repack: bad argument");
    DVAE_CHECK_ARG(!defer_state_get(ws).pending, "train_repack: an optimizer update is pending on this workspace (dvae_train_step_deferred): call dvae_train_flush BEFORE writing parameters");
    Layout L;
    make_layout(*plan, L);
    return launch_apply(plan, L, const_cast<float*>(params), nullptr, nullptr, (char*)ws, 0, false, 1, 0, 0, 0, 0, 0, nullptr, (hipStream_t)stream);
}

extern "C" int dvae_train_init(const dvae_train_plan_t* plan, const float* params, void* ws, void* stream) {
    DVAE_CHECK_ARG(plan && params && ws, "train_init: bad argument");
    Layout L;
    make_layout(*plan, L);
    DVAE_CHECK_ARG(L.total == plan->workspace_bytes, "train_init: plan does not match this library (workspace %lld vs %lld)",
                   (long long)plan->workspace_bytes, (long long)L.total);
    hipStream_t s = (hipStream_t)stream;
    char* w = (char*)ws;
    DVAE_HIP(hipMemsetAsync(w, 0, (size_t)L.total, s));
    fold_seq_reset(ws);
    defer_state_reset(ws);
    GroupDesc* tiles = new GroupDesc[L.ntiles + 8];
    BlockDesc* blocks = new BlockDesc[L.nblocks + 8];
    Block4* blocks4 = new Block4[L.nblocks4 + 8];
    TensorDesc td[DVAE_TRAIN_MAX_TENSORS];
    memset(td, 0, sizeof(td));
    if (is_bf(plan->precision)) fill_tables<__bf16>(plan, L, w, tiles, blocks, blocks4, td);
    else fill_tables<float>(plan, L, w, tiles, blocks, blocks4, td);
    hipError_t e1 = hipMemcpyAsync(w + L.o_tiles, tiles, (size_t)L.ntiles * sizeof(GroupDesc), hipMemcpyHostToDevice, s);
    hipError_t e2 = hipMemcpyAsync(w + L.o_tensors, td, sizeof(td), hipMemcpyHostToDevice, s);
    hipError_t e5 = hipMemcpyAsync(w + L.o_blocks, blocks, (size_t)L.nblocks * sizeof(BlockDesc), hipMemcpyHostToDevice, s);
    hipError_t e6 = hipMemcpyAsync(w + L.o_blocks4, blocks4, (size_t)L.nblocks4 * sizeof(Block4), hipMemcpyHostToDevice, s);
    W4Sched sched[3];
    W4Grids grids{{0, 0, 0}};
    hipError_t e8 = hipSuccess;
    for (int t = 0; t < 3; ++t) {
        const bool grouped = w4_grouped(*plan);
        if ((t == 0) == grouped) continue;
        w4_build_items(*plan, L, sched[t], t - 1);
        DVAE_CHECK_ARG(sched[t].grid > 0 && sched[t].grid <= W4_MAX_ITEMS, "train_init: weight-gradient schedule of %d workgroups does not fit the item table", sched[t].grid);
        grids.g[t] = sched[t].grid;
        const hipError_t e = hipMemcpyAsync(w + L.o_items4 + (int64_t)t * W4_MAX_ITEMS * sizeof(W4Item), sched[t].items.data(), sched[t].items.size() * sizeof(W4Item), hipMemcpyHostToDevice, s);
        if (e8 == hipSuccess) e8 = e;
    }
    const int64_t nchunks = plan->n_params / 64;
    unsigned char* ct = new unsigned char[nchunks + 64];
    memset(ct, 255, (size_t)nchunks + 64);
    for (int t = 0; t < plan->n_tensors; ++t) {
        const int64_t c0 = plan->tensor_offset[t] / 64, ne = (int64_t)plan->tensor_rows[t] * plan->tensor_cols[t];
        for (int64_t c = c0; c < c0 + (ne + 63) / 64; ++c) ct[c] = (unsigned char)t;
    }
    hipError_t e4 = hipMemcpyAsync(w + L.o_chunks, ct, (size_t)nchunks, hipMemcpyHostToDevice, s);
    DeferTask* dt = new DeferTask[DEFER_MAX_TASKS];
    memset(dt, 0, sizeof(DeferTask) * DEFER_MAX_TASKS);
    { DeferState st; st.ntasks = build_defer_tasks(plan, td, dt, DEFER_MAX_TASKS); defer_state_put(ws, st); }
    hipError_t e7 = hipMemcpyAsync(w + L.o_defer, dt, sizeof(DeferTask) * DEFER_MAX_TASKS, hipMemcpyHostToDevice, s);
    hipError_t e3 = hipStreamSynchronize(s);
    delete[] dt;
    delete[] tiles;
    delete[] blocks;
    delete[] blocks4;
    delete[] ct;
    DVAE_HIP(e1); DVAE_HIP(e2); DVAE_HIP(e4); DVAE_HIP(e5); DVAE_HIP(e6); DVAE_HIP(e7); DVAE_HIP(e8); DVAE_HIP(e3);
    w4_grid_put(ws, grids);
    return dvae_train_repack(plan, params, ws, stream);
}

struct FoldRequest { bool want = false, done = false; PendingUpdate u{}; float* losses3 = nullptr; };

static int device_cu_count(int dev) {
    static int cus[64] = {};
    if (cus[dev] == 0) {
        int n = 0;
        if (hipDeviceGetAttribute(&n, hipDeviceAttributeMultiprocessorCount, dev) != hipSuccess || n <= 0) n = 1;
        cus[dev] = n;
    }
    return cus[dev];
}

extern "C" int dvae_train_flush(const dvae_train_plan_t* plan, void* ws, void* stream) {
    DVAE_CHECK_ARG(plan && ws, "train_flush: bad argument");
    DeferState st = defer_state_get(ws);
    if (!st.pending) return 0;
    Layout L;
    make_layout(*plan, L);
    st.pending = false;
    defer_state_put(ws, st);
    ProfScope ps((hipStream_t)stream, 3);
    return launch_apply(plan, L, st.u.params, st.u.m, st.u.v, (char*)ws, st.u.n_slabs, true, st.u.step, st.u.lr, st.u.beta1, st.u.beta2, st.u.adam_eps,
                        1.0, nullptr , (hipStream_t)stream);
}

extern "C" int dvae_train_pending(const void* ws) { return defer_state_get(ws).pending ? 1 : 0; }

static bool defer_possible(const dvae_train_plan_t* plan, const void* ws) {
    if (!(plan->rows_kernel == 2 && rows2_supported(plan->precision, plan->model))) return false;
    if (!(plan->model == DVAE_MODEL_M1 || plan->model == DVAE_MODEL_M2)) return false;
    if (plan->row_index != 0 && plan->row_count <= 0) return false;
    const int dev = current_device();
    const int nt = defer_state_get(ws).ntasks;
    if (nt <= 0 || nt > DEFER_MAX_TASKS) return false;
    if (plan->rows_grid > device_cu_count(dev) || 8 * plan->rows_grid < 4 * nt) return false;
    if (wgrad_form_env() != 4 || plan->Bp <= 128) return false;
    const int64_t kper = kper_of(plan);
    return (plan->Bp + kper - 1) / kper <= 12;
}

extern "C" int dvae_train_can_defer(const dvae_train_plan_t* plan, const void* ws) {
    if (!plan || !ws) return 0;
    if (!kDiagBuild || env_int("DVAE_DEFER_APPLY", 0) != 1 || getenv("DVAE_FOLD_APPLY") != nullptr) return 0;
    return defer_possible(plan, ws) ? 1 : 0;
}

struct GradsOptions {
    int mode = 0;
    float *out_r = nullptr, *out_mu = nullptr, *out_lv = nullptr, *out_z = nullptr;
    const float *g_r = nullptr, *g_mu = nullptr, *g_lv = nullptr, *g_z = nullptr;
    int ld_r = 0, ld_gr = 0;
    bool rows_only = false;
    long long rng_step = -1;
    int group = -1;
    DeferRequest defer;
    FoldRequest fold;
};

namespace {
struct StepEnv {
    bool wgrad_set = false;
    int wgrad_form = wgrad_form_env(&wgrad_set);
    int ablate = env_int("DVAE_ABLATE", 0);
    int raw_inputs = -1;
    int64_t raw_auto_b = env_ll("DVAE_RAW_AUTO_B", 131072);
    bool ylo_always = getenv("DVAE_YLO_ALWAYS") != nullptr;
    int wgrad_repeat = std::max(env_int("DVAE_WGRAD_REPEAT", 1), 1);
    int gpw = env_int("DVAE_GPW", 2);
    unsigned fold_max_polls = 1u << 20;
    int defer_diag = env_int("DVAE_DEFER_DIAG", 0);
    long long defer_timeout_ms = std::max(env_ll("DVAE_DEFER_TIMEOUT_MS", 2000), 0ll);
    StepEnv() {
        if (const char* v = getenv("DVAE_RAW_INPUTS")) raw_inputs = strcmp(v, "0") == 0 ? 0 : (strcmp(v, "x") == 0 ? 1 : 3);
        if (gpw < 1 || gpw > 4) gpw = 2;
        if (const char* v = getenv("DVAE_FOLD_MAX_POLLS")) fold_max_polls = (unsigned)strtoul(v, nullptr, 10);
    }
};
}

static thread_local struct GroupPairing { unsigned last_id = 0; const void* last_ws = nullptr; } g_pairing;

static int fill_rows_args(const dvae_train_plan_t* plan, const Layout& L, const GradsOptions& o, const StepEnv& env, const float* params, char* w,
                          const float* x, int ldx, const float* y, int ldy, const float* eps_noise, float elbo_eps, RowsArgs& a) {
    const int esz = is_bf(plan->precision) ? 2 : 4;
    memset(&a, 0, sizeof(a));
    a.rows = (const int64_t*)(uintptr_t)plan->row_index;
    a.n_rows = plan->row_count; a.bad_rows = (int*)(uintptr_t)plan->bad_row_counter;
    DVAE_CHECK_ARG(a.rows == nullptr || a.n_rows > 0, "train_grads: row_index set but row_count <= 0");
    a.rng_seed = plan->rng_seed; a.rng_step = o.rng_step >= 0 ? (unsigned long long)o.rng_step : plan->rng_step;
    a.x = x; a.y = y; a.eps = eps_noise; a.ldx = ldx; a.ldy = plan->y_dim ? ldy : 0; a.ydim = plan->y_dim;
    a.fastx = (ldx == XD) && (((uintptr_t)x & 15) == 0);
    a.fasty = (plan->y_dim == XD) && (ldy == XD) && (((uintptr_t)y & 15) == 0);
    a.B = plan->B; a.Bp = plan->Bp; a.ntiles = (int)((plan->B + TB - 1) / TB);
    a.invB = (float)(1.0 / (double)plan->B); a.elbo_eps = elbo_eps;
    char* wc = w + L.o_wcopy;
    auto WC = [&](int64_t off) { return (const void*)(wc + off * esz); };
    a.W1s = WC(L.W1s); a.W2s = WC(L.W2s); a.Wmvs = WC(L.Wmvs); a.W3s = WC(L.W3s); a.W4s = WC(L.W4s); a.W5s = WC(L.W5s);
    a.W5t = WC(L.W5t); a.W4t = WC(L.W4t); a.W3zt = WC(L.W3zt); a.Wmvt = WC(L.Wmvt); a.W2t = WC(L.W2t);
    a.b1 = params + plan->tensor_offset[1]; a.b2 = params + plan->tensor_offset[3];
    a.bmu = params + plan->tensor_offset[5]; a.blv = params + plan->tensor_offset[7];
    a.b3 = params + plan->tensor_offset[9]; a.b4 = params + plan->tensor_offset[11]; a.b5 = params + plan->tensor_offset[13];
    a.w5last = params + plan->tensor_offset[12] + (int64_t)(XD - 1) * HD;
    if (L.info) {
        a.Wc1s = WC(L.Wc1s); a.Wc2s = WC(L.Wc2s); a.Wc2t = WC(L.Wc2t); a.Wa1s = WC(L.Wa1s); a.Wa1t = WC(L.Wa1t); a.Wa2s = WC(L.Wa2s); a.Wa2t = WC(L.Wa2t);
        a.bc1 = params + plan->tensor_offset[15]; a.bc2 = params + plan->tensor_offset[17]; a.wc3 = params + plan->tensor_offset[18]; a.bc3 = params + plan->tensor_offset[19];
        a.ba1 = params + plan->tensor_offset[21]; a.ba2 = params + plan->tensor_offset[23]; a.wa3 = params + plan->tensor_offset[24]; a.ba3 = params + plan->tensor_offset[25];
        a.alpha = (float)plan->info_alpha; a.beta = (float)plan->info_beta; a.gamma = (float)plan->info_gamma;
    }
    a.partials = (double*)(w + L.o_partials);
    a.wcopy = wc; a.wcopy_bytes = L.wcopy_elems * esz * planes_of(plan->precision);
    a.spl = L.stash_rows * plan->Bp; a.wpl_bytes = (unsigned)(L.wcopy_elems * esz);
    a.dbg = g_dbg; a.ablate = env.ablate;
    if (o.defer.on) {
        const PendingUpdate& u = o.defer.u;
        a.defer.on = 1; a.defer.have = o.defer.have ? 1 : 0;
        a.defer.diag = env.defer_diag;
        a.defer.a = o.defer.have ? make_apply_args(plan, L, u.params, u.m, u.v, w, u.n_slabs, true, u.step, u.lr, u.beta1, u.beta2, u.adam_eps, 1.0, o.defer.losses3)
                                 : make_apply_args(plan, L, const_cast<float*>(params), nullptr, nullptr, w, 1, false, 1, 0, 0, 0, 0, 0, o.defer.losses3);
        a.defer.tasks = (const DeferTask*)(w + L.o_defer); a.defer.ntasks = defer_state_get(w).ntasks;
        a.defer.shard = (unsigned*)(w + L.o_defer + DEFER_O_SHARD);
        a.defer.done = (unsigned*)(w + L.o_defer + DEFER_O_DONE); a.defer.err = a.defer.done + 1;
        a.defer.seq_arrive = o.defer.seq_arrive; a.defer.seq_done = o.defer.seq_done;
        a.defer.timeout_ticks = (unsigned long long)env.defer_timeout_ms * 100000ull;
    }
    const bool raw_possible = plan->rows_kernel >= 2 && rows2_supported(plan->precision, plan->model) && a.rows == nullptr &&
                              env.wgrad_form == 4 && o.mode != 1;
    const bool raw_auto = env.raw_inputs < 0 && raw_possible && o.mode == 0 && plan->B >= env.raw_auto_b;
    const int raw_mask = !raw_possible ? 0 : (raw_auto ? 3 : std::max(env.raw_inputs, 0));
    a.stash_inputs = 3 & ~raw_mask;
    a.mode = o.mode;
    a.ylo_epoch = (unsigned*)(w + L.o_flags); a.ylo_dirty = (int*)(w + L.o_flags + 1024);
    static std::atomic<unsigned> launch_counter{1};
    if (o.group == 1) {
        DVAE_CHECK_ARG(g_pairing.last_ws == w && g_pairing.last_id != 0, "train_grads_group: group 1 must follow a group 0 call on the same workspace");
        a.launch_id = g_pairing.last_id;
    } else {
        a.launch_id = launch_counter.fetch_add(1, std::memory_order_relaxed);
        if (a.launch_id == 0) a.launch_id = launch_counter.fetch_add(1, std::memory_order_relaxed);
        g_pairing = GroupPairing{a.launch_id, w};
    }
    a.out_r = o.out_r; a.out_mu = o.out_mu; a.out_lv = o.out_lv; a.out_z = o.out_z; a.ld_r = o.ld_r;
    a.g_r = o.g_r; a.g_mu = o.g_mu; a.g_lv = o.g_lv; a.g_z = o.g_z; a.ld_gr = o.ld_gr;
    DVAE_CHECK_ARG(a.mode == 0 || plan->rows_kernel == 2, "rows-kernel modes 1 / 2 exist in the 8-wave kernel only (plan->rows_kernel == 2)");
    char* st = w + L.o_stash;
    auto ST = [&](int64_t row) { return (void*)(st + row * plan->Bp * esz); };
    a.xT = ST(L.xT); a.yT = ST(L.yT); a.h1T = ST(L.h1T); a.h2T = ST(L.h2T); a.dh1T = ST(L.dh1T); a.dh2T = ST(L.dh2T);
    a.dmlvT = ST(L.dmlvT); a.zT = ST(L.zT); a.d1T = ST(L.d1T); a.d2T = ST(L.d2T); a.dd1T = ST(L.dd1T); a.dd2T = ST(L.dd2T); a.daT = ST(L.daT);
    if (L.info) {
        a.c1T = ST(L.c1T); a.c2T = ST(L.c2T); a.dc1T = ST(L.dc1T); a.dc2T = ST(L.dc2T); a.dc3T = ST(L.dc3T);
        a.a1T = ST(L.a1T); a.a2T = ST(L.a2T); a.da1T = ST(L.da1T); a.da2T = ST(L.da2T); a.da3T = ST(L.da3T);
    }
    return 0;
}

static int launch_rows_kernel(const dvae_train_plan_t* plan, const RowsArgs& a, hipStream_t s) {
    const int grid = (int)plan->rows_grid;
    if (plan->rows_kernel == 3 && rows3_supported(plan->precision, plan->model)) return launch_rows3(plan->model, plan->y_dim, a, grid, s);
    if (plan->rows_kernel == 2 && rows2_supported(plan->precision, plan->model)) return launch_rows2(plan->precision, plan->model, plan->y_dim, a, grid, s);
    return launch_rows1(plan->precision, plan->model, plan->y_dim, a, grid, s);
}

static int launch_wgrad_pass(const dvae_train_plan_t* plan, const Layout& L, GradsOptions& o, const StepEnv& env, const RowsArgs& a, bool wg4,
                             char* w, int reduce_slabs, hipStream_t s) {
    const bool x3 = plan->precision == DVAE_PREC_BF16X3;
    const int64_t kper = kper_of(plan);
    const int ks = used_slabs(plan);
    DVAE_CHECK_ARG(ks <= plan->ksplit, "train_grads: internal k-split mismatch");
    DVAE_CHECK_ARG(!w4_classed(*plan) || env.wgrad_form == 4,
                   "train_grads: the plan was made for the workgroup k-split weight-gradient kernel (class-sliced schedule); DVAE_WGRAD changed since");
    float* slabs = (float*)(w + L.o_grads);
    const WgradArgs wa{ks, plan->Bp, a.spl, kper, slabs, plan->n_params};
    for (int rep = 0; rep < env.wgrad_repeat; ++rep) {
        if (wg4) {
            const int tb0 = !w4_grouped(*plan) ? 0 : (o.group == 1 ? 2 : 1), tb1 = !w4_grouped(*plan) ? 0 : (o.group == 0 ? 1 : 2);
            for (int tb = tb0; tb <= tb1; ++tb) {
                ProfScope ps(s, rep == 0 ? 1 : 2);
                const int w4grid = w4_grid_get(w, tb);
                DVAE_CHECK_ARG(w4grid > 0, "train_grads: workspace was not set up by dvae_train_init");
                const dim3 g3((unsigned)w4grid);
                const RawIn ri{a.x, a.y, a.ldx, a.ldy, a.B};
                const int use_raw = 3 & ~a.stash_inputs;
                const Block4* bl = (const Block4*)(w + L.o_blocks4);
                const W4Item* w4items = (const W4Item*)(w + L.o_items4) + (size_t)tb * W4_MAX_ITEMS;
                ApplyArgs fa_apply;
                memset(&fa_apply, 0, sizeof(fa_apply));
                FoldArgs fold{nullptr, 0u, 0u};
                const PendingUpdate& u = o.fold.u;
                if (o.fold.want && !w4_classed(*plan) && env.wgrad_repeat == 1 && a.mode == 0 && ks > 1 && ks <= 16 && L.nblocks4 <= FOLD_MAXB && (int)g3.x <= device_cu_count(current_device())) {
                    fa_apply = make_apply_args(plan, L, u.params, u.m, u.v, w, ks, true, u.step, u.lr, u.beta1, u.beta2, u.adam_eps, 1.0, o.fold.losses3);
                    fold.cnt = (unsigned*)(w + L.o_flags);
                    fold.target = (unsigned)ks * fold_seq_next(w);
                    fold.max_polls = env.fold_max_polls;
                    o.fold.done = true;
                }
                int fin_block = -1;
                const unsigned* fin_err = nullptr;
                dim3 g3l = g3;
                if (a.defer.on) {
                    fa_apply = a.defer.a;
                    fin_block = (int)g3.x; fin_err = a.defer.err;
                    g3l = dim3(g3.x + 1);
                }
                const Wgrad4Args w4a{bl, w4items, ks, plan->Bp, a.spl, slabs, plan->n_params, ri, use_raw,
                                     a.ylo_skip ? a.ylo_epoch : nullptr, x3 ? a.launch_id : 0u , fa_apply, fold, fin_block, fin_err};
                const int rc = launch_wgrad4(plan->precision, w4a, (int)g3l.x, s);
                if (rc) return rc;
            }
        } else if (is_bf(plan->precision) && env.wgrad_form == 1) {
            ProfScope ps(s, rep == 0 ? 1 : 2);
            const int rc = launch_wgrad_lds(plan->precision, (const BlockDesc*)(w + L.o_blocks), L.nblocks, wa, s);
            if (rc) return rc;
        } else {
            ProfScope ps(s, rep == 0 ? 1 : 2);
            const int rc = launch_wgrad_ring(plan->precision, (const GroupDesc*)(w + L.o_tiles), L.ntiles, wa, env.gpw, s);
            if (rc) return rc;
        }
    }
    if (reduce_slabs && ks > 1) {
        ProfScope ps(s, 2);
        int64_t lo, hi;
        dvae_train_group_range(plan, o.group, &lo, &hi, nullptr);
        return launch_slab_reduce(slabs + lo, hi - lo, ks, plan->n_params, s);
    }
    return 0;
}

static int run_grads(const dvae_train_plan_t* plan, const float* params, void* ws, const float* x, int ldx, const float* y, int ldy,
                     const float* eps_noise, float elbo_eps, int reduce_slabs, void* stream, GradsOptions& o) {
    DVAE_CHECK_ARG(plan && params && ws && x && ldx >= XD, "train_grads: bad argument");
    DVAE_CHECK_ARG(plan->y_dim == 0 || (y != nullptr && ldy >= plan->y_dim), "train_grads: y missing or ldy < y_dim");
    if (!o.defer.on) { const int frc = dvae_train_flush(plan, ws, stream); if (frc) return frc; }
    const StepEnv env;
    Layout L;
    make_layout(*plan, L);
    hipStream_t s = (hipStream_t)stream;
    RowsArgs a;
    { const int rc = fill_rows_args(plan, L, o, env, params, (char*)ws, x, ldx, y, ldy, eps_noise, elbo_eps, a); if (rc) return rc; }
    const bool wg4 = env.wgrad_form == 4 && (plan->Bp > 128 || a.stash_inputs != 3  || env.wgrad_set);
    a.ylo_skip = (plan->precision == DVAE_PREC_BF16X3 && plan->y_dim > 0 && plan->rows_kernel >= 2 && rows2_supported(plan->precision, plan->model) && wg4 &&
                  (a.stash_inputs & 2) && !env.ylo_always) ? 1 : 0;
    DVAE_CHECK_ARG(o.group < 0 || (w4_grouped(*plan) && o.mode == 0 && !o.rows_only), "train_grads_group: the plan was not made for two weight-gradient launches (DVAE_EXCHANGE_GROUPS=2 when the plan is made)");
    if (o.group != 1) {
        ProfScope ps(s, 0);
        const int rc = launch_rows_kernel(plan, a, s);
        if (rc) return rc;
    }
    if (o.rows_only || a.mode == 1) return 0;
    return launch_wgrad_pass(plan, L, o, env, a, wg4, (char*)ws, reduce_slabs, s);
}

extern "C" int dvae_train_grads(const dvae_train_plan_t* plan, const float* params, void* ws, const float* x, int ldx,
                                const float* y, int ldy, const float* eps_noise, float elbo_eps, int reduce_slabs, void* stream) {
    GradsOptions o;
    return run_grads(plan, params, ws, x, ldx, y, ldy, eps_noise, elbo_eps, reduce_slabs, stream, o);
}

extern "C" int dvae_train_grads_group(const dvae_train_plan_t* plan, const float* params, void* ws, const float* x, int ldx, const float* y, int ldy,
                                      const float* eps_noise, float elbo_eps, int group, int reduce_slabs, void* stream) {
    DVAE_CHECK_ARG(plan && (group == 0 || group == 1), "train_grads_group: group must be 0 or 1");
    DVAE_CHECK_ARG(w4_grouped(*plan), "train_grads_group: the plan was not made for two weight-gradient launches (DVAE_EXCHANGE_GROUPS=2 when the plan is made)");
    GradsOptions o;
    o.group = group;
    return run_grads(plan, params, ws, x, ldx, y, ldy, eps_noise, elbo_eps, reduce_slabs, stream, o);
}

extern "C" int dvae_train_group_range(const dvae_train_plan_t* plan, int group, int64_t* lo, int64_t* hi, int* ngroups) {
    DVAE_CHECK_ARG(plan && lo && hi && group >= -1 && group <= 1, "train_group_range: bad argument");
    *lo = 0; *hi = plan->n_params;
    if (group == 0) *lo = plan->tensor_offset[8];
    if (group == 1) *hi = plan->tensor_offset[8];
    if (ngroups) *ngroups = w4_grouped(*plan) ? 2 : 1;
    return 0;
}

extern "C" int dvae_train_apply(const dvae_train_plan_t* plan, float* params, float* m, float* v, void* ws, int n_slabs,
                                int step, double lr, double beta1, double beta2, double adam_eps, double grad_scale,
                                float* losses3, void* stream) {
    DVAE_CHECK_ARG(plan && params && m && v && ws && step >= 1, "train_apply: bad argument");
    { const int frc = dvae_train_flush(plan, ws, stream); if (frc) return frc; }
    Layout L;
    make_layout(*plan, L);
    if (n_slabs <= 0) n_slabs = used_slabs(plan);
    DVAE_CHECK_ARG(n_slabs <= plan->ksplit, "train_apply: n_slabs %d > plan ksplit %d", n_slabs, plan->ksplit);
    ProfScope ps((hipStream_t)stream, 3);
    return launch_apply(plan, L, params, m, v, (char*)ws, n_slabs, true, step, lr, beta1, beta2, adam_eps, grad_scale, losses3,
                        (hipStream_t)stream);
}

extern "C" int dvae_train_step(const dvae_train_plan_t* plan, float* params, float* m, float* v, void* ws,
                               const float* x, int ldx, const float* y, int ldy, const float* eps_noise, float elbo_eps,
                               int step, double lr, double beta1, double beta2, double adam_eps, float* losses3, void* stream) {
    DVAE_CHECK_ARG(plan && params && m && v && ws && step >= 1, "train_step: bad argument");
    const bool fold_on = kDiagBuild && env_int("DVAE_FOLD_APPLY", 0) != 0;
    GradsOptions o;
    o.rng_step = step;
    o.fold = FoldRequest{fold_on, false, PendingUpdate{params, m, v, step, lr, beta1, beta2, adam_eps, 0 }, losses3};
    const int rc = run_grads(plan, params, ws, x, ldx, y, ldy, eps_noise, elbo_eps, 0, stream, o);
    if (rc) return rc;
    if (o.fold.done) return 0;
    return dvae_train_apply(plan, params, m, v, ws, 0, step, lr, beta1, beta2, adam_eps, 1.0, losses3, stream);
}

extern "C" int dvae_train_step_deferred(const dvae_train_plan_t* plan, float* params, float* m, float* v, void* ws,
                                        const float* x, int ldx, const float* y, int ldy, const float* eps_noise, float elbo_eps,
                                        int step, double lr, double beta1, double beta2, double adam_eps, float* losses3, void* stream) {
    DVAE_CHECK_ARG(plan && params && m && v && ws && step >= 1 && losses3, "train_step_deferred: bad argument");
    if (!dvae_train_can_defer(plan, ws))
        return dvae_train_step(plan, params, m, v, ws, x, ldx, y, ldy, eps_noise, elbo_eps, step, lr, beta1, beta2, adam_eps, losses3, stream);
    DeferState st = defer_state_get(ws);
    GradsOptions o;
    o.rng_step = step;
    o.defer = DeferRequest{true, st.pending, st.u, st.seq_arrive + (st.pending ? 1u : 0u), st.seq_done + 1u, losses3};
    const int rc = run_grads(plan, params, ws, x, ldx, y, ldy, eps_noise, elbo_eps, 0, stream, o);
    if (rc) return rc;
    st.seq_arrive += st.pending ? 1u : 0u; st.seq_done += 1u;
    st.pending = true;
    st.u = PendingUpdate{params, m, v, step, lr, beta1, beta2, adam_eps, used_slabs(plan)};
    defer_state_put(ws, st);
    return 0;
}

extern "C" int dvae_module_forward(const dvae_train_plan_t* plan, const float* params, void* ws, const float* x, int ldx,
                                   const float* y, int ldy, const float* eps_noise, float* out_r, int ld_r, float* out_mu,
                                   float* out_lv, float* out_z, int repack, void* stream) {
    DVAE_CHECK_ARG(plan && params && ws && x && eps_noise && out_r && out_mu && out_lv && ld_r >= XD, "module_forward: bad argument");
    DVAE_CHECK_ARG(plan->rows_kernel == 2 && plan->row_index == 0, "module_forward: needs the 8-wave rows kernel and no gather table");
    { const int frc = dvae_train_flush(plan, ws, stream); if (frc) return frc; }
    if (repack) { int rc = dvae_train_repack(plan, params, ws, stream); if (rc) return rc; }
    GradsOptions o;
    o.mode = 1; o.out_r = out_r; o.ld_r = ld_r; o.out_mu = out_mu; o.out_lv = out_lv; o.out_z = out_z;
    return run_grads(plan, params, ws, x, ldx, y, ldy, eps_noise, 0.f, 0, stream, o);
}

extern "C" int dvae_module_backward(const dvae_train_plan_t* plan, const float* params, void* ws, const float* x, int ldx,
                                    const float* y, int ldy, const float* eps_noise, const float* g_r, int ld_gr,
                                    const float* g_mu, const float* g_lv, const float* g_z, float* grad_flat, int accumulate,
                                    void* stream) {
    DVAE_CHECK_ARG(plan && params && ws && x && eps_noise && grad_flat, "module_backward: bad argument");
    DVAE_CHECK_ARG(plan->rows_kernel == 2 && plan->row_index == 0, "module_backward: needs the 8-wave rows kernel and no gather table");
    DVAE_CHECK_ARG(g_r == nullptr || ld_gr >= XD, "module_backward: ld_gr < 513");
    GradsOptions o;
    o.mode = 2; o.g_r = g_r; o.ld_gr = ld_gr; o.g_mu = g_mu; o.g_lv = g_lv; o.g_z = g_z;
    const int rc = run_grads(plan, params, ws, x, ldx, y, ldy, eps_noise, 0.f, 0, stream, o);
    if (rc) return rc;
    Layout L;
    make_layout(*plan, L);
    const float* slabs = (const float*)((const char*)ws + L.o_grads);
    return launch_slab_sum(slabs, plan->n_params, used_slabs(plan), plan->n_params, grad_flat, accumulate, (hipStream_t)stream);
}

extern "C" int dvae_train_debug_stamps(void* buf) {
    g_dbg = (unsigned long long*)buf;
    return 0;
}

extern "C" int dvae_train_eval(const dvae_train_plan_t* plan, const float* params, void* ws, const float* x, int ldx,
                               const float* y, int ldy, const float* eps_noise, float elbo_eps, float* losses3, void* stream) {
    DVAE_CHECK_ARG(plan && params && ws && x && losses3, "train_eval: bad argument");
    Layout L;
    make_layout(*plan, L);
    GradsOptions o;
    o.rows_only = true;
    const int rc = run_grads(plan, params, ws, x, ldx, y, ldy, eps_noise, elbo_eps, 0, stream, o);
    if (rc) return rc;
    ApplyArgs a;
    memset(&a, 0, sizeof(a));
    char* w = (char*)ws;
    a.partials = (const double*)(w + L.o_partials); a.npartials = (int)plan->rows_grid; a.B = plan->B; a.losses3 = losses3; a.accum = (double*)(uintptr_t)plan->loss_accum;
    a.info = plan->model == DVAE_MODEL_M2_INFO; a.alpha = (float)plan->info_alpha; a.beta = (float)plan->info_beta; a.gamma = (float)plan->info_gamma;
    return launch_apply_losses(a, (hipStream_t)stream);
}

extern "C" int dvae_train_noise(const dvae_train_plan_t* plan, uint64_t step, float* eps_out, void* stream) {
    DVAE_CHECK_ARG(plan && eps_out, "train_noise: null argument");
    return launch_noise((unsigned long long)plan->rng_seed, (unsigned long long)step, plan->B, eps_out, (hipStream_t)stream);
}

extern "C" int dvae_train_profile(int enable) {
    g_prof = enable != 0;
    return 0;
}

extern "C" int dvae_train_profile_read(double ms[4], int64_t calls[4]) {
    hipError_t e = hipDeviceSynchronize();
    for (int i = 0; i < g_npending; ++i) {
        float t = 0.f;
        if (hipEventElapsedTime(&t, g_pending[i].a, g_pending[i].b) == hipSuccess) {
            g_ms[g_pending[i].which] += (double)t;
            g_calls[g_pending[i].which] += 1;
        }
        (void)hipEventDestroy(g_pending[i].a);
        (void)hipEventDestroy(g_pending[i].b);
    }
    g_npending = 0;
    for (int i = 0; i < 4; ++i) { ms[i] = g_ms[i]; calls[i] = g_calls[i]; g_ms[i] = 0; g_calls[i] = 0; }
    DVAE_HIP(e);
    return 0;
}
```

### disentangled-vae_amd/csrc/train_wgrad.hip

```cpp
#include <type_traits>
#include "fused_tiles.hpp"
#include "rows_common.hpp"
#include "apply_common.hpp"
#include "wgrad_types.hpp"
#include "../../include/dvae_train.h"

namespace dvae {
namespace fused {

template <typename P, bool A1, bool B1>
__device__ __forceinline__ void wgrad_body(const GroupDesc& d, int64_t kbeg, int64_t kend, int64_t Bp, int64_t spl, float* __restrict__ slab,
                                           int l31, int h) {
    typedef typename P::T T;
    typedef typename P::Frag Frag;
    constexpr int E = P::E, KS = P::KSTEP, NP = P::NP;
    const int lane = h * 32 + l31;
    constexpr int FB = 64 * E;
    const T* a0p = (const T*)d.A[0] + lane * E;
    const T* a1p = A1 ? (const T*)d.A[1] + lane * E : a0p;
    const T* b0p = (const T*)d.Bm[0] + lane * E;
    const T* b1p = B1 ? (const T*)d.Bm[1] + lane * E : b0p;
    const bool bias0 = d.bias_off[0] >= 0, bias1 = A1 && d.bias_off[1] >= 0;
    f32x16 c00, c01, c10, c11, cb0, cb1;
#pragma unroll
// ... 62 lines not shown
template <typename P>
__global__ __launch_bounds__(256, DVAE_WGRAD_OCC) void wgrad_kernel(const GroupDesc* __restrict__ groups, int ngroups, int ksplit, int64_t Bp,
                                                    int64_t spl, int64_t kper, float* __restrict__ slabs, int64_t slab_stride) {
    const int lane = threadIdx.x & 63, wave = threadIdx.x >> 6;
    const int l31 = lane & 31, h = lane >> 5;
    const int slice = blockIdx.x % ksplit, wg = blockIdx.x / ksplit;
    const int gi = wg * (blockDim.x >> 6) + wave;
    if (gi >= ngroups) return;
    const GroupDesc d = groups[gi];
    const int64_t kbeg = (int64_t)slice * kper;
    int64_t kend = kbeg + kper;
    if (kend > Bp) kend = Bp;
    float* slab = slabs + (int64_t)slice * slab_stride;
    const bool a1 = d.A[1] != nullptr, b1 = d.Bm[1] != nullptr;
    if (a1 && b1) wgrad_body<P, true, true>(d, kbeg, kend, Bp, spl, slab, l31, h);
    else if (a1) wgrad_body<P, true, false>(d, kbeg, kend, Bp, spl, slab, l31, h);
    else if (b1) wgrad_body<P, false, true>(d, kbeg, kend, Bp, spl, slab, l31, h);
    else wgrad_body<P, false, false>(d, kbeg, kend, Bp, spl, slab, l31, h);
}
#ifdef DVAE_DIAG
template <typename P> struct WgLds {
    static constexpr int KPS = 2;
    static constexpr int NSTG = 4;
    static constexpr int FRAG = 1024;
    static constexpr int STAGE = 8 * P::NP * KPS * FRAG;
    static constexpr int BYTES = NSTG * STAGE;
    static constexpr int LOADS = 2 * P::NP * KPS;
};

template <typename P>
__global__ __launch_bounds__(256, 1) void wgrad_lds_kernel(const BlockDesc* __restrict__ blocks, int nblocks, int ksplit, int64_t Bp,
                                                           int64_t spl, int64_t kper, float* __restrict__ slabs, int64_t slab_stride) {
    typedef typename P::T T;
    typedef typename P::Frag Frag;
    typedef WgLds<P> W;
    constexpr int E = P::E, KS = P::KSTEP, NP = P::NP, KPS = W::KPS, NSTG = W::NSTG;
    constexpr int FB = 64 * E;
    extern __shared__ __attribute__((aligned(16))) char wsm[];
    const int lane = threadIdx.x & 63;
    const int wave = __builtin_amdgcn_readfirstlane(threadIdx.x >> 6);
    const int l31 = lane & 31, h = lane >> 5;
    const int slice = blockIdx.x % ksplit, bi = blockIdx.x / ksplit;
    if (bi >= nblocks) return;
    const BlockDesc& bd = blocks[bi];
    const GroupDesc d = bd.g[wave];
    const int64_t kbeg = (int64_t)slice * kper;
    int64_t kend = kbeg + kper;
    if (kend > Bp) kend = Bp;
    const int64_t sbeg = kbeg / KS, send = kend / KS;
    const int nst = (int)((send - sbeg + KPS - 1) / KPS);
    float* slab = slabs + (int64_t)slice * slab_stride;
    const T* src[2];
    src[0] = (const T*)(bd.At[wave] ? bd.At[wave] : bd.At[0]);
    src[1] = (const T*)(bd.Bt[wave] ? bd.Bt[wave] : bd.At[0]);
    auto issue = [&](int st) {
        char* base = wsm + (st % NSTG) * W::STAGE;
#pragma unroll
        for (int q = 0; q < 2; ++q)
#pragma unroll
            for (int pl = 0; pl < NP; ++pl)
#pragma unroll
                for (int kk = 0; kk < KPS; ++kk) {
                    int64_t sk = sbeg + (int64_t)st * KPS + kk; sk = sk < send ? sk : send - 1;
                    const T* gp = src[q] + pl * spl + sk * FB + lane * E;
                    char* lp = base + (((q * 4 + wave) * NP + pl) * KPS + kk) * W::FRAG;
                    __builtin_amdgcn_global_load_lds((const __attribute__((address_space(1))) void*)gp, (__attribute__((address_space(3))) void*)lp, 16, 0, 0);
                }
    };
    f32x16 c00, c01, c10, c11, cb0, cb1;
#pragma unroll
    for (int i = 0; i < 16; ++i) { c00[i] = 0.f; c01[i] = 0.f; c10[i] = 0.f; c11[i] = 0.f; cb0[i] = 0.f; cb1[i] = 0.f; }
    const bool have = d.A[0] != nullptr;
    const bool A1 = d.A[1] != nullptr, B1 = d.Bm[1] != nullptr;
    const bool bias0 = have && d.bias_off[0] >= 0, bias1 = A1 && d.bias_off[1] >= 0;
    const Frag one = P::ones();
    const int wr = wave >> 1, wc = wave & 1;
#pragma unroll
    for (int st = 0; st < NSTG - 1; ++st) issue(st);
    for (int st = 0; st < nst; ++st) {
        if constexpr (W::LOADS * (NSTG - 2) == 8) asm volatile("s_waitcnt vmcnt(8)" ::: "memory");
        else if constexpr (W::LOADS * (NSTG - 2) == 16) asm volatile("s_waitcnt vmcnt(16)" ::: "memory");
        else asm volatile("s_waitcnt vmcnt(0)" ::: "memory");
        asm volatile("s_barrier" ::: "memory");
        issue(st + NSTG - 1);
        const char* base = wsm + (st % NSTG) * W::STAGE;
#pragma unroll
        for (int kk = 0; kk < KPS; ++kk) {
            if (sbeg + (int64_t)st * KPS + kk >= send) break;
            auto frag = [&](int slot, int pl) -> Frag {
                return *reinterpret_cast<const Frag*>(base + ((slot * NP + pl) * KPS + kk) * W::FRAG + lane * 16);
            };
            Frag a0[NP], a1[NP], b0[NP], b1[NP];
#pragma unroll
            for (int pl = 0; pl < NP; ++pl) { a0[pl] = frag(2 * wr, pl); a1[pl] = frag(2 * wr + 1, pl); b0[pl] = frag(4 + 2 * wc, pl); b1[pl] = frag(5 + 2 * wc, pl); }
            if (have) {
                mmap<P>(c00, a0, b0);
                if (B1) mmap<P>(c01, a0, b1);
                if (A1) mmap<P>(c10, a1, b0);
                if (A1 && B1) mmap<P>(c11, a1, b1);
                if (bias0) { P::mma(cb0, a0[0], one); if constexpr (NP == 2) P::mma(cb0, a0[1], one); }
                if (bias1) { P::mma(cb1, a1[0], one); if constexpr (NP == 2) P::mma(cb1, a1[1], one); }
            }
        }
    }
    asm volatile("s_waitcnt vmcnt(0)" ::: "memory");
    if (!have) return;
#pragma unroll
    for (int r = 0; r < 16; ++r) {
        const int row = feat_of(r, h);
        if (row < d.mvalid[0]) {
            const bool hi = d.split16 && row >= 16;
            const int rr = hi ? row - 16 : row;
            const int ldo = hi ? d.ldo_hi : d.ldo[0];
            if (l31 < d.nvalid[0]) slab[(hi ? d.out_off_hi[0] : d.out_off[0][0]) + (int64_t)rr * ldo + l31] = c00[r];
            if (B1) { if (l31 < d.nvalid[1]) slab[(hi ? d.out_off_hi[1] : d.out_off[0][1]) + (int64_t)rr * ldo + l31] = c01[r]; }
            if (bias0 && l31 == 0) slab[(hi ? d.bias_off_hi : d.bias_off[0]) + rr] = cb0[r];
        }
        if (A1) {
            if (row < d.mvalid[1]) {
                if (l31 < d.nvalid[0]) slab[d.out_off[1][0] + (int64_t)row * d.ldo[1] + l31] = c10[r];
                if (B1) { if (l31 < d.nvalid[1]) slab[d.out_off[1][1] + (int64_t)row * d.ldo[1] + l31] = c11[r]; }
                if (bias1 && l31 == 0) slab[d.bias_off[1] + row] = cb1[r];
            }
        }
    }
}
#endif
template <int I, int N, typename F>
__device__ __forceinline__ void static_for_w(F&& f) {
    if constexpr (I < N) { f(std::integral_constant<int, I>{}); static_for_w<I + 1, N>(f); }
}

#ifndef W4_SLAB_AUX
#define W4_SLAB_AUX 16
#endif
__device__ __forceinline__ void slab_store(float* p, float v) {
#if W4_SLAB_AUX
    __hip_atomic_store(p, v, __ATOMIC_RELAXED, __HIP_MEMORY_SCOPE_AGENT);
#else
    *p = v;
#endif
}
template <typename P> struct Wg4 {
#ifndef DVAE_W4RING_X3
#define DVAE_W4RING_X3 2
#endif
#ifndef DVAE_W4RING
#define DVAE_W4RING 4
#endif
    static constexpr int RD = P::NP == 2 ? DVAE_W4RING_X3 : DVAE_W4RING;
    static constexpr size_t BYTES = (size_t)(8 * 16) * 64 * 16 + 12 * 64 * 4;
};

template <typename P, int NA, int NB, int RAW, bool BLO = true, bool BIAS = true>
__device__ __forceinline__ void wgrad4_body(const Block4& bd, const Block4* __restrict__ bdg, char* wsm, int slice, int64_t Bp, int64_t spl, int64_t kbeg, int64_t kend_,
                                            float* __restrict__ slabs, int64_t slab_stride, int lane, int wave, const RawIn& ri) {
    typedef typename P::T T;
    typedef typename P::Frag Frag;
    typedef Wg4<P> W;
    typedef const __attribute__((address_space(1))) char* gptr;
    typedef const __attribute__((address_space(1))) Frag* gfrag;
    constexpr int E = P::E, KS = P::KSTEP, NP = P::NP, RD = RAW == 2 ? 2 : W::RD;
    constexpr int64_t FBB = 64 * 16;
    constexpr int SLD = 128 + 8, SPL = 16 * SLD;
    const int l31 = lane & 31, h = lane >> 5;
    int64_t kend = kend_;
    if (kend > Bp) kend = Bp;
    const int64_t s0 = kbeg / KS, s1 = kend / KS;
    const int64_t nq = (s1 - s0 + 3) / 4;
    int64_t sbeg = s0 + (int64_t)wave * nq, send = sbeg + nq;
    if (send > s1) send = s1;
    if (sbeg > send) sbeg = send;
    gptr ap[NA], bp[NB];
    const int rot = NA == 4 ? wave : 0;
#pragma unroll
    for (int k = 0; k < NA; ++k) { const void* q = NA == 4 ? bdg->At[(k + rot) & 3] : bd.At[k]; ap[k] = (gptr)(uintptr_t)(q ? q : bd.At[0]); }
#pragma unroll
    for (int k = 0; k < NB; ++k) bp[k] = (gptr)(uintptr_t)(bd.Bt[k] ? bd.Bt[k] : bd.Bt[0]);
    const int64_t plb = spl * (int64_t)sizeof(T);
    const unsigned loff = (unsigned)lane * 16u;
    f32x16 c[NA][NB];
#pragma unroll
    for (int i = 0; i < NA; ++i)
#pragma unroll
        for (int j = 0; j < NB; ++j)
#pragma unroll
            for (int r = 0; r < 16; ++r) c[i][j][r] = 0.f;
    float bs[4] = {0.f, 0.f, 0.f, 0.f};
    Frag a[RD][NA][NP], b[RAW == 1 ? 1 : (RAW == 2 ? 1 : RD)][RAW == 1 ? 1 : NB][NP];
    float braw[RAW == 1 ? RD : 1][RAW == 1 ? NB : 1][E];
    f32x4 rawq[RAW == 2 ? RD : 1][RAW == 2 ? 8 : 1];
    typedef const __attribute__((address_space(1))) float* gflt;
    const gflt rsrc = (gflt)(uintptr_t)(RAW ? (bd.raw == 1 ? ri.x : ri.y) : nullptr);
    const int rld = RAW ? (bd.raw == 1 ? ri.ldx : ri.ldy) : 0;
    int rcolv[RAW == 1 ? NB : 1];
    if constexpr (RAW == 1) {
#pragma unroll
        for (int k = 0; k < NB; ++k) { const int cc = bd.rcol[k] + l31; rcolv[k] = cc < bd.rncols ? cc : bd.rncols - 1; }
    }
    T* const stg = reinterpret_cast<T*>(wsm) + wave * (SPL * NP);
    const int rcol4 = RAW == 2 ? bd.rcol[0] + 4 * l31 : 0;
    auto load = [&](auto sc, int64_t sk) __attribute__((always_inline)) {
        constexpr int s = decltype(sc)::value;
        const int64_t o = sk * FBB;
#pragma unroll
        for (int k = 0; k < NA; ++k) {
            a[s][k][0] = *(gfrag)(ap[k] + o + loff);
            if constexpr (NP == 2) a[s][k][1] = *(gfrag)(ap[k] + plb + o + loff);
        }
        if constexpr (RAW == 1) {
            const int64_t f0 = sk * KS + h * E;
#pragma unroll
            for (int e = 0; e < E; ++e) {
                int64_t fr = f0 + e; fr = fr < ri.B ? fr : ri.B - 1;
                const gflt rowp = rsrc + fr * rld;
#pragma unroll
                for (int k = 0; k < NB; ++k) braw[s][k][e] = rowp[rcolv[k]];
            }
        } else if constexpr (RAW == 2) {
#pragma unroll
            for (int u = 0; u < 8; ++u) {
                int64_t fr = sk * KS + 2 * u + h; fr = fr < ri.B ? fr : ri.B - 1;
                rawq[s][u] = reinterpret_cast<const __attribute__((address_space(1))) F4U*>(rsrc + fr * rld + rcol4)->v;
            }
        } else {
#pragma unroll
            for (int k = 0; k < NB; ++k) {
                b[s][k][0] = *(gfrag)(bp[k] + o + loff);
                if constexpr (NP == 2 && BLO) b[s][k][1] = *(gfrag)(bp[k] + plb + o + loff);
            }
        }
    };
    auto fsum = [&](const Frag& f) __attribute__((always_inline)) {
        float t = 0.f;
#pragma unroll
        for (int q = 0; q < E; ++q) t += (float)f[q];
        return t;
    };
    auto prepare = [&](auto sc) __attribute__((always_inline)) {
        constexpr int s = decltype(sc)::value;
        if constexpr (RAW == 2) {
            typedef typename P::Pack4 Pack4;
#pragma unroll
            for (int u = 0; u < 8; ++u) {
                Pack4 ph, pl;
#pragma unroll
                for (int e = 0; e < 4; ++e) { ph[e] = P::cvt(rawq[s][u][e]); pl[e] = P::cvt(rawq[s][u][e] - (float)ph[e]); }
                T* const rowp = stg + (2 * u + h) * SLD + 4 * l31;
                *reinterpret_cast<Pack4*>(rowp) = ph;
                if constexpr (NP == 2) *reinterpret_cast<Pack4*>(rowp + SPL) = pl;
            }
            const int i16 = l31 & 15, q = i16 >> 2, pp = i16 & 3, cg = l31 >> 4;
            typedef short s16x8 __attribute__((ext_vector_type(8)));
#pragma unroll
            for (int j = 0; j < NB; ++j)
#pragma unroll
                for (int pln = 0; pln < NP; ++pln) {
                    const T* bpj = stg + pln * SPL + q * SLD + 32 * j + 16 * cg + 4 * pp;
                    const s16x4 r0 = lds_tr16(bpj + (8 * h) * SLD), r1 = lds_tr16(bpj + (8 * h + 4) * SLD);
                    const s16x8 raw8 = {r0[0], r0[1], r0[2], r0[3], r1[0], r1[1], r1[2], r1[3]};
                    b[0][j][pln] = __builtin_bit_cast(Frag, raw8);
                }
        }
    };
    auto compute = [&](auto sc) __attribute__((always_inline)) {
        constexpr int s = decltype(sc)::value;
#ifdef W4_NOMFMA
        if constexpr (RAW == 0) {
#pragma unroll
            for (int i = 0; i < NA; ++i) {
                bs[i] += fsum(a[s][i][0]);
                if constexpr (NP == 2) bs[i] += fsum(a[s][i][1]);
#pragma unroll
                for (int j = 0; j < NB; ++j) { c[i][j][0] += (float)b[s][j][0][0]; if constexpr (NP == 2 && BLO) c[i][j][1] += (float)b[s][j][1][0]; }
            }
            return;
        }
#endif
        if constexpr (RAW == 2) {
#pragma unroll
            for (int i = 0; i < NA; ++i) {
#pragma unroll
                for (int j = 0; j < NB; ++j) mmap<P>(c[i][j], a[s][i], b[0][j]);
                if constexpr (BIAS) {
                    bs[i] += fsum(a[s][i][0]);
                    if constexpr (NP == 2) bs[i] += fsum(a[s][i][1]);
                }
            }
        } else if constexpr (RAW == 1) {
#pragma unroll
            for (int j = 0; j < NB; ++j) {
                Frag bj[NP];
#pragma unroll
                for (int e = 0; e < E; ++e) {
                    bj[0][e] = P::cvt(braw[s][j][e]);
                    if constexpr (NP == 2) bj[1][e] = P::cvt(braw[s][j][e] - (float)bj[0][e]);
                }
#pragma unroll
                for (int i = 0; i < NA; ++i) mmap<P>(c[i][j], a[s][i], bj);
            }
            if constexpr (BIAS) {
#pragma unroll
                for (int i = 0; i < NA; ++i) {
                    bs[i] += fsum(a[s][i][0]);
                    if constexpr (NP == 2) bs[i] += fsum(a[s][i][1]);
                }
            }
        } else {
#pragma unroll
            for (int i = 0; i < NA; ++i) {
#pragma unroll
                for (int j = 0; j < NB; ++j) mmap<P>(c[i][j], a[s][i], b[s][j], BLO);
#ifndef W4_NOFSUM
                if constexpr (BIAS) {
                    bs[i] += fsum(a[s][i][0]);
                    if constexpr (NP == 2) bs[i] += fsum(a[s][i][1]);
                }
#endif
            }
        }
    };
    {
        const int64_t slast = (send > s0 ? send : s0 + 1) - 1;
        static_for_w<0, RD>([&](auto sc) {
            int64_t sk = sbeg + decltype(sc)::value; sk = sk < slast ? sk : slast;
            load(sc, sk);
        });
        __builtin_amdgcn_sched_barrier(0);
        if constexpr (RAW == 2) prepare(std::integral_constant<int, 0>{});
#pragma unroll 1
        for (int64_t sk = sbeg; sk < send; sk += RD) {
            static_for_w<0, RD>([&](auto sc) {
                constexpr int s = decltype(sc)::value;
                if (sk + s < send) compute(sc);
                int64_t sn = sk + RD + s; sn = sn < slast ? sn : slast;
                if constexpr (RAW == 2) {
                    prepare(std::integral_constant<int, (s + 1) % RD>{});
                }
#ifndef W4_NOLOAD
                load(sc, sn);
#else
                (void)sn;
#endif
                __builtin_amdgcn_sched_barrier(0);
            });
        }
        if constexpr (RAW == 2) __syncthreads();
    }
#ifdef W4_NOEPI
    {
        float t = bs[0] + bs[1] + bs[2] + bs[3];
#pragma unroll
        for (int i = 0; i < NA; ++i)
#pragma unroll
            for (int j = 0; j < NB; ++j)
#pragma unroll
                for (int r = 0; r < 16; ++r) t += c[i][j][r];
        if (t == 123.456f) slabs[0] = t;
        return;
    }
#endif
    constexpr int ROWQ = 4 * 4 * 64;
    f32x4* const lds = reinterpret_cast<f32x4*>(wsm);
    float* const lbias = reinterpret_cast<float*>(lds + 8 * ROWQ);
    auto put_row = [&](auto ic, int slot) __attribute__((always_inline)) {
        constexpr int i = decltype(ic)::value;
#pragma unroll
        for (int j = 0; j < NB; ++j)
#pragma unroll
            for (int q = 0; q < 4; ++q)
                lds[slot * ROWQ + (j * 4 + q) * 64 + lane] = f32x4{c[i][j][4 * q], c[i][j][4 * q + 1], c[i][j][4 * q + 2], c[i][j][4 * q + 3]};
    };
    auto add_row0 = [&](int slot) __attribute__((always_inline)) {
#pragma unroll
        for (int j = 0; j < NB; ++j)
#pragma unroll
            for (int q = 0; q < 4; ++q) {
                const f32x4 v = lds[slot * ROWQ + (j * 4 + q) * 64 + lane];
#pragma unroll
                for (int e = 0; e < 4; ++e) c[0][j][4 * q + e] += v[e];
            }
    };
    typedef std::integral_constant<int, 0> I0; typedef std::integral_constant<int, 1> I1;
    typedef std::integral_constant<int, 2> I2; typedef std::integral_constant<int, 3> I3;
    if constexpr (NA == 1) {
        if (wave != 0) { put_row(I0{}, wave); lbias[wave * 64 + lane] = bs[0]; }
        __syncthreads();
        if (wave != 0) return;
        add_row0(1); add_row0(2); add_row0(3);
        bs[0] += lbias[64 + lane]; bs[0] += lbias[128 + lane]; bs[0] += lbias[192 + lane];
    } else {
        const int d1 = (wave + 1) & 3, d2 = (wave + 2) & 3, d3 = (wave + 3) & 3;
        put_row(I1{}, 2 * d1); put_row(I2{}, 2 * d2 + 1);
        lbias[(3 * d1 + 0) * 64 + lane] = bs[1]; lbias[(3 * d2 + 1) * 64 + lane] = bs[2]; lbias[(3 * d3 + 2) * 64 + lane] = bs[3];
        __syncthreads();
        add_row0(2 * wave); add_row0(2 * wave + 1);
        __syncthreads();
        put_row(I3{}, d3);
        __syncthreads();
        add_row0(wave);
        bs[0] += lbias[(3 * wave + 0) * 64 + lane]; bs[0] += lbias[(3 * wave + 1) * 64 + lane]; bs[0] += lbias[(3 * wave + 2) * 64 + lane];
    }
    float* const slab = slabs + (int64_t)slice * slab_stride;
    const int mv = bdg->mvalid[rot], ldo = bdg->ldo[rot];
    const int64_t a_off = bdg->a_off[rot], bias_off = bdg->bias_off[rot];
    const bool split = rot == 0 && bd.split16;
    if (mv == 32 && !split) {
        const unsigned lo = (unsigned)(4 * h * ldo + l31);
#if W4_SLAB_AUX
        const __amdgpu_buffer_rsrc_t srs = __builtin_amdgcn_make_buffer_rsrc(slab + a_off, 0, 0x7fffffff, 0x00020000);
#endif
#pragma unroll
        for (int j = 0; j < NB; ++j) {
            if (l31 < bd.nvalid[j]) {
                float* const t0 = slab + a_off + bd.bcol[j];
#pragma unroll
                for (int r = 0; r < 16; ++r) {
#if W4_SLAB_AUX
                    __builtin_amdgcn_raw_buffer_store_b32(__float_as_uint(c[0][j][r]), srs, (int)(4u * lo), (int)(4u * (unsigned)(bd.bcol[j] + ((r & 3) + 8 * (r >> 2)) * ldo)), W4_SLAB_AUX);
#else
                    float* const rowp = t0 + (int64_t)((r & 3) + 8 * (r >> 2)) * ldo;
                    rowp[lo] = c[0][j][r];
#endif
                }
                (void)t0;
            }
        }
    } else {
#pragma unroll
        for (int j = 0; j < NB; ++j) {
#pragma unroll
            for (int r = 0; r < 16; ++r) {
                const int row = feat_of(r, h);
                if (row < mv && l31 < bd.nvalid[j]) {
                    const bool hi = split && row >= 16;
                    const int rr = hi ? row - 16 : row;
                    const int ld = hi ? bd.ldo_hi : ldo;
                    slab_store(&slab[(hi ? bd.a_off_hi : a_off) + (int64_t)rr * ld + bd.bcol[j] + l31], c[0][j][r]);
                }
            }
        }
    }
    const float tot = bs[0] + __shfl_xor(bs[0], 32, 64);
    if (h == 0 && l31 < mv && bias_off >= 0) {
        const bool hi = split && l31 >= 16;
        slab_store(&slab[hi ? bd.bias_off_hi + (l31 - 16) : bias_off + l31], tot);
    }
}
#ifdef DVAE_DIAG
template <typename T, int NP>
__device__ __forceinline__ void fold_tail(const ApplyArgs& g, const FoldArgs& fa, const Block4& bd, const Block4* __restrict__ bdg, int bi, int slice,
                                          int ks, int lane, int wave, char* wsm) {
    int* const flag = reinterpret_cast<int*>(wsm);
#if W4_SLAB_AUX
    asm volatile("s_waitcnt vmcnt(0)" ::: "memory");
#else
    __builtin_amdgcn_fence(__ATOMIC_RELEASE, "agent");
#endif
    __syncthreads();
    if (threadIdx.x == 0) {
        __hip_atomic_fetch_add(fa.cnt + 16 + bi, 1u, __ATOMIC_RELAXED, __HIP_MEMORY_SCOPE_AGENT);
        unsigned polls = 0;
        int ok = 1;
        while ((int)(__hip_atomic_load(fa.cnt + 16 + bi, __ATOMIC_RELAXED, __HIP_MEMORY_SCOPE_AGENT) - fa.target) < 0) {
            __builtin_amdgcn_s_sleep(1);
            if (++polls > fa.max_polls) { ok = 0; break; }
        }
        if (!ok) __hip_atomic_store(fa.cnt + 2, 1u, __ATOMIC_RELAXED, __HIP_MEMORY_SCOPE_AGENT);
        flag[0] = ok;
    }
    __syncthreads();
    const int ok = flag[0];
#if !W4_SLAB_AUX
    __builtin_amdgcn_fence(__ATOMIC_ACQUIRE, "agent");
#endif
#ifndef FOLD_DIAG
#define FOLD_DIAG 0
#endif
    if (ok && FOLD_DIAG != 1) {
        int nb = 0;
#pragma unroll
        for (int k = 0; k < 4; ++k) if (bd.Bt[k] != nullptr) nb = k + 1;
        const int gw = slice * 4 + wave, nw = ks * 4;
        constexpr int UB = 4;
        for (int u0 = gw; u0 < 132; u0 += UB * nw) {
            int64_t idx[UB][2];
            float pi[UB][2], mo[UB][2], vo[UB][2], gi[UB][2];
            int tq[UB][2];
#pragma unroll
            for (int b = 0; b < UB; ++b) {
                const int u = u0 + b * nw;
                idx[b][0] = idx[b][1] = -1;
                tq[b][0] = tq[b][1] = 0;
                if (u < 128) {
                    const int rot = u >> 5, rr = u & 31;
                    if (rr < bdg->mvalid[rot]) {
                        const bool hi = rot == 0 && bd.split16 && rr >= 16;
                        const int64_t base = hi ? bd.a_off_hi + (int64_t)(rr - 16) * bd.ldo_hi : bdg->a_off[rot] + (int64_t)rr * bdg->ldo[rot];
                        tq[b][0] = tq[b][1] = hi ? bd.wt_hi : bdg->wt[rot];
#pragma unroll
                        for (int q = 0; q < 2; ++q) {
                            const int j = (lane >> 5) + 2 * q, l = lane & 31;
                            if (j < nb && l < bdg->nvalid[j]) idx[b][q] = base + bdg->bcol[j] + l;
                        }
                    }
                } else if (u < 132) {
                    const int rot = u - 128;
                    const int64_t bo = bdg->bias_off[rot];
                    const int mv = bdg->mvalid[rot];
                    if (bo >= 0) {
                        const bool split = rot == 0 && bd.split16;
                        tq[b][0] = bdg->bt[rot]; tq[b][1] = bd.bt_hi;
                        if (lane < (split ? 16 : 32) && lane < mv) idx[b][0] = bo + lane;
                        if (split && lane >= 16 && lane < 32 && lane < mv) idx[b][1] = bd.bias_off_hi + (lane - 16);
                    }
                }
#pragma unroll
                for (int q = 0; q < 2; ++q) {
                    const int64_t i = idx[b][q] >= 0 ? idx[b][q] : 0;
                    pi[b][q] = g.p[i]; mo[b][q] = g.m[i]; vo[b][q] = g.v[i];
                    gi[b][q] = slab_sum_at<W4_SLAB_AUX != 0>(g, i);
                }
            }
#pragma unroll
            for (int b = 0; b < UB; ++b)
#pragma unroll
                for (int q = 0; q < 2; ++q) {
                    const TensorDesc& d = g.tensors[tq[b][q]];
                    if (FOLD_DIAG == 2) { if (idx[b][q] >= 0) g.p[idx[b][q]] = pi[b][q] + mo[b][q] + vo[b][q] + gi[b][q]; continue; }
                    if (idx[b][q] >= 0) apply_element<T, true, NP>(g, idx[b][q], d, pi[b][q], mo[b][q], vo[b][q], gi[b][q]);
                }
        }
    }
    if (blockIdx.x == 0 && g.losses3 != nullptr && FOLD_DIAG == 0) {
        __syncthreads();
        finalize_losses(g, reinterpret_cast<double (*)[4]>(wsm + 64));
        if (threadIdx.x == 0 && __hip_atomic_load(fa.cnt + 2, __ATOMIC_RELAXED, __HIP_MEMORY_SCOPE_AGENT) != 0u) g.losses3[0] = __builtin_nanf("");
    }
    if (!ok && threadIdx.x == 0 && g.losses3 != nullptr) g.losses3[0] = __builtin_nanf("");
}
#endif

template <typename P>
__global__ __launch_bounds__(256, 1) void wgrad4_kernel(const Block4* __restrict__ blocks, const W4Item* __restrict__ items, int ksplit, int64_t Bp,
                                                        int64_t spl, float* __restrict__ slabs, int64_t slab_stride,
                                                        const RawIn ri, int use_raw, const unsigned* __restrict__ ylo_epoch, unsigned launch_id,
                                                        const ApplyArgs fold_apply, const FoldArgs fold, int fin_block, const unsigned* fin_err) {
    extern __shared__ __attribute__((aligned(16))) char wsm[];
    const int lane = threadIdx.x & 63;
    const int wave = __builtin_amdgcn_readfirstlane(threadIdx.x >> 6);
    if (fin_block >= 0 && (int)blockIdx.x == fin_block) {
        finalize_losses(fold_apply, reinterpret_cast<double (*)[4]>(wsm));
        if (threadIdx.x == 0 && fin_err != nullptr && __hip_atomic_load(fin_err, __ATOMIC_RELAXED, __HIP_MEMORY_SCOPE_AGENT) != 0u)
            fold_apply.losses3[0] = __builtin_nanf("");
        return;
    }
    const W4Item it = items[blockIdx.x];
    if (it.block < 0) return;
    const int slice = it.slice, bi = it.block;
    const Block4 bd = blocks[bi];
    int na = 0, nb = 0;
#pragma unroll
    for (int k = 0; k < 4; ++k) { if (bd.At[k] != nullptr) na = k + 1; if (bd.Bt[k] != nullptr) nb = k + 1; }
#define W4_GO_(NA_, NB_, RAW_, BLO_) wgrad4_body<P, NA_, NB_, RAW_, BLO_, true>(bd, blocks + bi, wsm, slice, Bp, spl, it.kbeg, it.kend, slabs, slab_stride, lane, wave, ri)
#define W4_GO(NA_, NB_, RAW_) W4_GO_(NA_, NB_, RAW_, true)
    bool raw = false;
    if constexpr (sizeof(typename P::T) == 2) raw = (use_raw & bd.raw) != 0;
    if (raw) {
        if constexpr (sizeof(typename P::T) == 2) {
            if (nb == 4 && bd.rcol[0] + 128 <= bd.rncols) W4_GO(4, 4, 2);
            else if (nb == 1) W4_GO(4, 1, 1);
            else if (nb == 2) W4_GO(4, 2, 1);
            else W4_GO(4, 4, 1);
        }
    } else if (sizeof(typename P::T) == 2 && P::NP == 2 && bd.raw == 2 && ylo_epoch != nullptr && *ylo_epoch != launch_id) {
        if (nb == 1) W4_GO_(4, 1, 0, false);
        else if (nb == 2) W4_GO_(4, 2, 0, false);
        else W4_GO_(4, 4, 0, false);
    } else if (na == 1) {
        if (nb == 1) W4_GO(1, 1, 0);
        else if (nb == 2) W4_GO(1, 2, 0);
        else W4_GO(1, 4, 0);
    } else {
        if (nb == 1) W4_GO(4, 1, 0);
        else if (nb == 2) W4_GO(4, 2, 0);
        else W4_GO(4, 4, 0);
    }
#undef W4_GO
#undef W4_GO_
#ifndef W4_FOLD
#ifdef DVAE_DIAG
#define W4_FOLD 1
#else
#define W4_FOLD 0
#endif
#endif
#if W4_FOLD
    if (fold.cnt != nullptr) fold_tail<typename P::T, P::NP>(fold_apply, fold, bd, blocks + bi, bi, slice, ksplit, lane, wave, wsm);
#endif
}
template <int NS>
__device__ __forceinline__ float slab_total(const float* __restrict__ slabs, int64_t i, int nslabs, int64_t stride) {
    float part[NS];
#pragma unroll
    for (int k = 0; k < NS; ++k) part[k] = slabs[(int64_t)(k < nslabs ? k : 0) * stride + i];
    float t = part[0];
#pragma unroll
    for (int k = 1; k < NS; ++k) if (k < nslabs) t += part[k];
    return t;
}
__device__ __forceinline__ float slab_total_any(const float* __restrict__ slabs, int64_t i, int nslabs, int64_t stride) {
    if (nslabs <= 8) return slab_total<8>(slabs, i, nslabs, stride);
    if (nslabs <= 16) return slab_total<16>(slabs, i, nslabs, stride);
    float s = slabs[i];
    for (int k = 1; k < nslabs; ++k) s += slabs[k * stride + i];
    return s;
}

__global__ __launch_bounds__(256) void slab_sum_kernel(const float* __restrict__ slabs, int64_t n, int nslabs, int64_t stride, float* __restrict__ dst, int accumulate) {
    for (int64_t i = (int64_t)blockIdx.x * blockDim.x + threadIdx.x; i < n; i += (int64_t)gridDim.x * blockDim.x) {
        const float s = slab_total_any(slabs, i, nslabs, stride);
        dst[i] = accumulate ? dst[i] + s : s;
    }
}

__global__ __launch_bounds__(256) void slab_reduce_kernel(float* __restrict__ slabs, int64_t n, int nslabs, int64_t stride) {
    for (int64_t i = (int64_t)blockIdx.x * blockDim.x + threadIdx.x; i < n; i += (int64_t)gridDim.x * blockDim.x)
        slabs[i] = slab_total_any(slabs, i, nslabs, stride);
}

template <typename T, bool ADAM, int NP = 1>
__global__ __launch_bounds__(256) void apply_kernel(const ApplyArgs g) {
    if (blockIdx.x == gridDim.x - 1) {
        if (!ADAM || g.losses3 == nullptr) return;
        __shared__ double red[4][4];
        finalize_losses(g, red);
        return;
    }
    const int64_t idx = (int64_t)blockIdx.x * 256 + threadIdx.x;
    if (idx >= g.n_params) return;
    const float pi = g.p[idx];
    float m_old = 0.f, v_old = 0.f, gi = 0.f;
    if (ADAM) {
        m_old = g.m[idx]; v_old = g.v[idx];
        gi = slab_sum_at(g, idx);
    }
    const int t = g.chunk_tensor[__builtin_amdgcn_readfirstlane((int)(idx >> 6))];
    if (t == 255) return;
    const TensorDesc d = g.tensors[t];
    apply_element<T, ADAM, NP>(g, idx, d, pi, m_old, v_old, gi);
}

#ifdef DVAE_DIAG
template <typename T, int NP>
__global__ __launch_bounds__(256) void apply_units_kernel(const ApplyArgs g, const DeferTask* __restrict__ tasks, int nunits) {
    __shared__ __attribute__((aligned(16))) char sm[4 * DeferLds<T, NP>::wave_elems * sizeof(T) > 128 ? 4 * DeferLds<T, NP>::wave_elems * sizeof(T) : 128];
    if (blockIdx.x == gridDim.x - 1) {
        if (g.losses3 == nullptr) return;
        finalize_losses(g, reinterpret_cast<double (*)[4]>(sm));
        return;
    }
    const int wave = __builtin_amdgcn_readfirstlane(threadIdx.x >> 6), lane = threadIdx.x & 63;
    const int un = wave * ((int)gridDim.x - 1) + (int)blockIdx.x;
    if (un >= nunits) return;
    T* const tile = reinterpret_cast<T*>(sm) + wave * DeferLds<T, NP>::wave_elems;
    defer_unit<T, NP, false>(g, tasks[un >> 2], un & 3, tile, lane);
}
#endif

int launch_wgrad_ring(int precision, const GroupDesc* groups, int ngroups, const WgradArgs& a, int gpw, hipStream_t s) {
    const dim3 g2((unsigned)(((ngroups + gpw - 1) / gpw) * a.ksplit));
    with_policy(precision, [&](auto pol) {
        hipLaunchKernelGGL((wgrad_kernel<decltype(pol)>), g2, dim3(64 * gpw), 0, s, groups, ngroups, a.ksplit, a.Bp, a.spl, a.kper, a.slabs, a.slab_stride);
    });
    DVAE_LAUNCH_OK("wgrad_kernel");
    return 0;
}

int launch_wgrad_lds(int precision, const BlockDesc* blocks, int nblocks, const WgradArgs& a, hipStream_t s) {
#ifdef DVAE_DIAG
    const int dev = current_device();
    const dim3 g3((unsigned)(nblocks * a.ksplit));
    auto lds = [&](auto pol) -> int {
        using P = decltype(pol);
        static bool attr_done[64] = {};
        if (!attr_done[dev]) { DVAE_HIP(hipFuncSetAttribute((const void*)wgrad_lds_kernel<P>, hipFuncAttributeMaxDynamicSharedMemorySize, WgLds<P>::BYTES)); attr_done[dev] = true; }
        hipLaunchKernelGGL((wgrad_lds_kernel<P>), g3, dim3(256), WgLds<P>::BYTES, s, blocks, nblocks, a.ksplit, a.Bp, a.spl, a.kper, a.slabs, a.slab_stride);
        return 0;
    };
    const int rc = precision == DVAE_PREC_BF16X3 ? lds(PolX3{}) : lds(PolBF16{});
    if (rc) return rc;
    DVAE_LAUNCH_OK("wgrad_lds_kernel");
    return 0;
#else
    set_error("train_grads: DVAE_WGRAD=lds exists in the diagnostic build only (build.py --diag)");
    return DVAE_E_UNSUPPORTED;
#endif
}

int launch_wgrad4(int precision, const Wgrad4Args& a, int grid, hipStream_t s) {
    const int dev = current_device();
    const int rc = with_policy(precision, [&](auto pol) -> int {
        using P = decltype(pol);
        static bool attr_done[64] = {};
        if (!attr_done[dev]) { DVAE_HIP(hipFuncSetAttribute((const void*)wgrad4_kernel<P>, hipFuncAttributeMaxDynamicSharedMemorySize, (int)Wg4<P>::BYTES)); attr_done[dev] = true; }
        hipLaunchKernelGGL((wgrad4_kernel<P>), dim3((unsigned)grid), dim3(256), Wg4<P>::BYTES, s, a.blocks, a.items, a.ksplit, a.Bp, a.spl, a.slabs, a.slab_stride, a.ri, a.use_raw,
                           a.ylo_epoch, a.launch_id, a.fold_apply, a.fold, a.fin_block, a.fin_err);
        return 0;
    });
    if (rc) return rc;
    DVAE_LAUNCH_OK("wgrad4_kernel");
    return 0;
}

int launch_slab_reduce(float* slabs, int64_t n, int nslabs, int64_t stride, hipStream_t s) {
    hipLaunchKernelGGL(slab_reduce_kernel, dim3(512), dim3(256), 0, s, slabs, n, nslabs, stride);
    DVAE_LAUNCH_OK("slab_reduce_kernel");
    return 0;
}

int launch_slab_sum(const float* slabs, int64_t n, int nslabs, int64_t stride, float* dst, int accumulate, hipStream_t s) {
    hipLaunchKernelGGL(slab_sum_kernel, dim3(512), dim3(256), 0, s, slabs, n, nslabs, stride, dst, accumulate);
    DVAE_LAUNCH_OK("slab_sum_kernel");
    return 0;
}

int launch_apply_kernel(int precision, bool adam, const ApplyArgs& a, hipStream_t s) {
    const dim3 grid((unsigned)((a.n_params + 255) / 256 + 1));
    if (precision == DVAE_PREC_BF16X3) {
        if (adam) hipLaunchKernelGGL((apply_kernel<__bf16, true, 2>), grid, dim3(256), 0, s, a);
        else hipLaunchKernelGGL((apply_kernel<__bf16, false, 2>), grid, dim3(256), 0, s, a);
    } else if (precision == DVAE_PREC_BF16) {
        if (adam) hipLaunchKernelGGL((apply_kernel<__bf16, true>), grid, dim3(256), 0, s, a);
        else hipLaunchKernelGGL((apply_kernel<__bf16, false>), grid, dim3(256), 0, s, a);
    } else {
        if (adam) hipLaunchKernelGGL((apply_kernel<float, true>), grid, dim3(256), 0, s, a);
        else hipLaunchKernelGGL((apply_kernel<float, false>), grid, dim3(256), 0, s, a);
    }
    DVAE_LAUNCH_OK("apply_kernel");
    return 0;
}

int launch_apply_losses(const ApplyArgs& a, hipStream_t s) {
    hipLaunchKernelGGL((apply_kernel<float, true>), dim3(1), dim3(256), 0, s, a);
    DVAE_LAUNCH_OK("apply_kernel(loss only)");
    return 0;
}

#ifdef DVAE_DIAG
int launch_apply_units(int precision, const ApplyArgs& a, const DeferTask* tasks, int nunits, hipStream_t s) {
    const dim3 gu((unsigned)((nunits + 3) / 4 + 1));
    if (precision == DVAE_PREC_BF16X3) hipLaunchKernelGGL((apply_units_kernel<__bf16, 2>), gu, dim3(256), 0, s, a, tasks, nunits);
    else hipLaunchKernelGGL((apply_units_kernel<__bf16, 1>), gu, dim3(256), 0, s, a, tasks, nunits);
    DVAE_LAUNCH_OK("apply_units_kernel");
    return 0;
}
#endif

}
}
```

### disentangled-vae_amd/csrc/wgrad_types.hpp

```cpp
#pragma once
#include <stdint.h>
#include <hip/hip_runtime.h>
#include "apply_types.hpp"

namespace dvae {
namespace fused {

struct GroupDesc {
    const void* A[2];
    const void* Bm[2];
    int64_t out_off[2][2];
    int64_t bias_off[2];
    int32_t ldo[2];
    int32_t mvalid[2];
    int32_t nvalid[2];
    int32_t split16;
    int32_t ldo_hi;
    int64_t out_off_hi[2];
    int64_t bias_off_hi;
};

struct BlockDesc {
    const void* At[4];
    const void* Bt[4];
    GroupDesc g[4];
};

struct Block4 {
    const void* At[4];
    const void* Bt[4];
    int64_t a_off[4];
    int64_t bias_off[4];
    int32_t ldo[4];
    int32_t mvalid[4];
    int32_t bcol[4];
    int32_t nvalid[4];
    int32_t split16;
    int32_t ldo_hi;
    int64_t a_off_hi;
    int64_t bias_off_hi;
    int32_t raw, rncols;
    int32_t rcol[4];
    int32_t wt[4], bt[4], wt_hi, bt_hi;
    int32_t layer, pad_;
};

struct W4Item { int32_t block, slice; int64_t kbeg, kend; };
constexpr int W4_MAX_ITEMS = 4096;

struct RawIn { const float* x; const float* y; int ldx, ldy; int64_t B; };

constexpr int FOLD_MAXB = 120;
struct FoldArgs { unsigned* cnt; unsigned target; unsigned max_polls; };

struct WgradArgs { int ksplit; int64_t Bp, spl, kper; float* slabs; int64_t slab_stride; };
int launch_wgrad_ring(int precision, const GroupDesc* groups, int ngroups, const WgradArgs& a, int gpw, hipStream_t s);
int launch_wgrad_lds(int precision, const BlockDesc* blocks, int nblocks, const WgradArgs& a, hipStream_t s);
struct Wgrad4Args {
    const Block4* blocks; const W4Item* items; int ksplit; int64_t Bp, spl; float* slabs; int64_t slab_stride;
    RawIn ri; int use_raw; const unsigned* ylo_epoch; unsigned launch_id;
    ApplyArgs fold_apply; FoldArgs fold; int fin_block; const unsigned* fin_err;
};
int launch_wgrad4(int precision, const Wgrad4Args& a, int grid, hipStream_t s);
int launch_slab_reduce(float* slabs, int64_t n, int nslabs, int64_t stride, hipStream_t s);
int launch_slab_sum(const float* slabs, int64_t n, int nslabs, int64_t stride, float* dst, int accumulate, hipStream_t s);
int launch_apply_kernel(int precision, bool adam, const ApplyArgs& a, hipStream_t s);
int launch_apply_losses(const ApplyArgs& a, hipStream_t s);
#ifdef DVAE_DIAG
int launch_apply_units(int precision, const ApplyArgs& a, const DeferTask* tasks, int nunits, hipStream_t s);
#endif

}
}
```

### disentangled-vae_amd/native.py

```python
import ctypes
import os

import torch

_HERE = os.path.dirname(os.path.abspath(__file__))
LIB_PATH = os.environ.get("DVAE_LIB") or os.path.join(_HERE, "libdvae_hip.so")

ACT_NONE, ACT_TANH, ACT_RELU, ACT_SIGMOID, ACT_EXP = 0, 1, 2, 3, 4
ABI_VERSION = 1

_lib = None

c_vp, c_i, c_i64, c_f, c_d, c_sz = (ctypes.c_void_p, ctypes.c_int, ctypes.c_int64, ctypes.c_float,
                                    ctypes.c_double, ctypes.c_size_t)

SIGNATURES = {
    "dvae_build_has_diag": (c_i, []),
    "dvae_abi_version": (c_i, []),
    "dvae_last_error": (ctypes.c_char_p, []),
    "dvae_device_count": (c_i, []),
    "dvae_linear_act_fwd": (c_i, [c_vp, c_i, c_i, c_vp, c_i, c_i, c_vp, c_i, c_vp, c_vp, c_i, c_i64, c_i, c_i, c_vp]),
    "dvae_act_bwd": (c_i, [c_vp, c_i, c_vp, c_i, c_vp, c_i, c_i64, c_i, c_i, c_vp]),
    "dvae_linear_bwd_data": (c_i, [c_vp, c_i, c_vp, c_i, c_i, c_vp, c_i, c_i64, c_i, c_i, c_i, c_vp]),
    "dvae_linear_bwd_weight": (c_i, [c_vp, c_i, c_vp, c_i, c_i, c_vp, c_i, c_i, c_vp, c_i, c_vp, c_i64, c_i, c_i, c_vp]),
    "dvae_linear_bwd_weight_det": (c_i, [c_vp, c_i, c_vp, c_i, c_i, c_vp, c_i, c_i, c_vp, c_i, c_vp, c_i64, c_i, c_i, c_vp, c_vp]),
    "dvae_linear_bwd_weight_workspace_bytes": (ctypes.c_size_t, [c_i64, c_i, c_i, c_i]),
    "dvae_reparam_fwd": (c_i, [c_vp, c_vp, c_vp, c_vp, c_i64, c_vp]),
    "dvae_reparam_bwd": (c_i, [c_vp, c_vp, c_vp, c_vp, c_vp, c_i64, c_vp]),
    "dvae_elbo_workspace_bytes": (c_sz, [c_i64]),
    "dvae_elbo_fwd": (c_i, [c_vp, c_i, c_vp, c_i, c_vp, c_vp, c_f, c_i64, c_i, c_i, c_vp, c_vp, c_vp, c_vp]),
    "dvae_elbo_bwd": (c_i, [c_vp, c_i, c_vp, c_i, c_vp, c_vp, c_vp, c_i64, c_i, c_i, c_vp, c_i, c_vp, c_vp, c_vp]),
    "dvae_elbo_bwd3": (c_i, [c_vp, c_i, c_vp, c_i, c_vp, c_vp, c_vp, c_vp, c_vp, c_i64, c_i, c_i, c_vp, c_i, c_vp, c_vp, c_vp]),
    "dvae_bce_fwd": (c_i, [c_vp, c_vp, c_f, c_i64, c_i, c_i, c_vp, c_vp, c_vp]),
    "dvae_bce_bwd": (c_i, [c_vp, c_vp, c_f, c_vp, c_i64, c_i, c_i, c_vp, c_vp, c_vp]),
    "dvae_isrows_fwd": (c_i, [c_vp, c_i, c_vp, c_i, c_vp, c_vp, c_f, c_i64, c_i, c_i, c_vp, c_vp, c_vp]),
    "dvae_isrows_bwd": (c_i, [c_vp, c_i, c_vp, c_i, c_vp, c_vp, c_vp, c_vp, c_i64, c_i, c_i, c_vp, c_i, c_vp, c_vp, c_vp]),
    "dvae_bce2_fwd": (c_i, [c_vp, c_vp, c_vp, c_f, c_i64, c_i, c_vp, c_vp, c_vp]),
    "dvae_bce2_bwd": (c_i, [c_vp, c_vp, c_vp, c_f, c_vp, c_i64, c_i, c_vp, c_vp, c_vp, c_vp]),
    "dvae_sqerr_fwd": (c_i, [c_i, c_vp, c_vp, c_vp, c_i64, c_i, c_vp, c_vp, c_vp]),
    "dvae_sqerr_bwd": (c_i, [c_i, c_vp, c_vp, c_vp, c_vp, c_i64, c_i, c_vp, c_vp, c_vp, c_vp]),
    "dvae_adam_step": (c_i, [c_vp, c_vp, c_vp, c_vp, c_i64, c_d, c_d, c_d, c_d, c_i, c_d, c_vp]),
    "dvae_stft": (c_i, [c_vp, c_i, c_i64, c_vp, c_i, c_i, c_i64, c_vp, c_i, c_vp]),
    "dvae_stft_f32": (c_i, [c_vp, c_i64, c_vp, c_i, c_i, c_i64, c_vp, c_i, c_vp]),
    "dvae_istft_workspace_bytes": (c_sz, [c_i64, c_i]),
    "dvae_istft_workspace_bytes_hop": (c_sz, [c_i64, c_i, c_i]),
    "dvae_istft": (c_i, [c_vp, c_i64, c_i64, c_vp, c_i, c_i, c_i64, c_vp, c_i64, c_vp, c_vp]),
    "dvae_istft_frames": (c_i, [c_vp, c_i64, c_i64, c_vp, c_i, c_i, c_i64, c_vp, c_i64, c_vp, c_vp]),
    "dvae_istft_f32": (c_i, [c_vp, c_i64, c_i64, c_i, c_vp, c_i, c_i, c_i64, c_vp, c_i64, c_vp, c_vp]),
    "dvae_stft_batch": (c_i, [c_vp, c_i, c_i64, c_vp, c_i, c_i, c_i, c_vp, c_i64, c_i, c_i64, c_vp, c_i, c_vp]),
    "dvae_istft_batch": (c_i, [c_vp, c_i64, c_vp, c_i, c_i, c_i, c_vp, c_i64, c_i, c_i64, c_vp, c_i64, c_vp, c_vp, c_i64, c_vp, c_vp]),
    "dvae_transpose": (c_i, [c_vp, c_i64, c_i64, c_i64, c_vp, c_i64, c_vp]),
    "dvae_gather_rows": (c_i, [c_vp, c_i64, c_i64, c_vp, c_i64, c_i, c_vp, c_i64, c_vp, c_vp]),
    "dvae_vad_workspace_bytes": (c_sz, [c_i64]),
    "dvae_vad_labels": (c_i, [c_vp, c_i, c_i64, c_i, c_i, c_i64, c_d, c_vp, c_vp, c_vp]),
    "dvae_ibm_workspace_bytes": (c_sz, []),
    "dvae_ibm_labels": (c_i, [c_vp, c_i64, c_i64, c_f, c_f, c_vp, c_vp, c_vp, c_vp]),
    "dvae_peak_normalise_workspace_bytes": (c_sz, [c_i64]),
    "dvae_peak_normalise_batch": (c_i, [c_vp, c_i64, c_i, c_vp, c_i64, c_i, c_vp, c_vp, c_vp]),
    "dvae_vad_batch_workspace_bytes": (c_sz, [c_i64, c_i64]),
    "dvae_vad_labels_batch": (c_i, [c_vp, c_i, c_i64, c_i, c_i, c_d, c_i, c_vp, c_i64, c_i, c_i64, c_vp, c_vp, c_vp]),
    "dvae_ibm_batch_workspace_bytes": (c_sz, [c_i64]),
    "dvae_ibm_labels_batch": (c_i, [c_vp, c_i64, c_f, c_f, c_i, c_vp, c_i64, c_i, c_vp, c_i64, c_vp, c_vp, c_vp]),
    "dvae_si_ratios_workspace_bytes": (c_sz, [c_i64]),
    "dvae_si_ratios_batch": (c_i, [c_vp, c_i64, c_i, c_vp, c_i64, c_i, c_vp, c_i64, c_i, c_i, c_vp, c_i64, c_vp, c_vp, c_vp, c_vp]),
    "dvae_estoi_workspace_bytes": (c_sz, [c_i64, c_i64, c_i64, c_i]),
    "dvae_estoi_batch": (c_i, [c_vp, c_i64, c_i, c_vp, c_i64, c_i, c_i, c_vp, c_i64, c_i64, c_i64, c_i64, c_i64, c_vp, c_i, c_i, c_i, c_vp, c_vp, c_i,
                               c_vp, c_vp, c_vp, c_vp, c_vp]),
    "dvae_mix_snr_workspace_bytes": (c_sz, [c_i64, c_i]),
    "dvae_mix_snr_batch": (c_i, [c_vp, c_i64, c_i, c_vp, c_i64, c_i, c_i, c_vp, c_i64, c_vp, c_i, c_vp, c_vp, c_vp, c_i64, c_i, c_vp, c_vp, c_vp]),
    "dvae_resample_run": (c_i, [c_i, c_i, c_i]),
    "dvae_resample_batch": (c_i, [c_vp, c_i64, c_i, c_i64, c_vp, c_i64, c_i, c_i, c_vp, c_i64, c_vp, c_i, c_i, c_i, c_vp]),
    "dvae_classify_weights_floats": (c_sz, [c_i]),
    "dvae_classify_batch": (c_i, [c_vp, c_i, c_i64, c_i64, c_i, c_vp, c_vp, c_i, c_vp, c_vp, c_vp, c_vp]),
    "dvae_label_counts_batch": (c_i, [c_vp, c_i64, c_vp, c_i64, c_i64, c_i, c_i, c_vp, c_vp, c_vp, c_vp]),
    "dvae_train_plan": (c_i, [c_i, c_i, c_i, c_i64, c_i, c_vp]),
    "dvae_train_init": (c_i, [c_vp, c_vp, c_vp, c_vp]),
    "dvae_train_repack": (c_i, [c_vp, c_vp, c_vp, c_vp]),
    "dvae_train_grads": (c_i, [c_vp, c_vp, c_vp, c_vp, c_i, c_vp, c_i, c_vp, c_f, c_i, c_vp]),
    "dvae_train_grads_group": (c_i, [c_vp, c_vp, c_vp, c_vp, c_i, c_vp, c_i, c_vp, c_f, c_i, c_i, c_vp]),
    "dvae_train_group_range": (c_i, [c_vp, c_i, c_vp, c_vp, c_vp]),
    "dvae_train_apply": (c_i, [c_vp, c_vp, c_vp, c_vp, c_vp, c_i, c_i, c_d, c_d, c_d, c_d, c_d, c_vp, c_vp]),
    "dvae_train_step": (c_i, [c_vp, c_vp, c_vp, c_vp, c_vp, c_vp, c_i, c_vp, c_i, c_vp, c_f, c_i, c_d, c_d, c_d, c_d, c_vp, c_vp]),
    "dvae_train_step_deferred": (c_i, [c_vp, c_vp, c_vp, c_vp, c_vp, c_vp, c_i, c_vp, c_i, c_vp, c_f, c_i, c_d, c_d, c_d, c_d, c_vp, c_vp]),
    "dvae_train_flush": (c_i, [c_vp, c_vp, c_vp]),
    "dvae_train_pending": (c_i, [c_vp]),
    "dvae_train_can_defer": (c_i, [c_vp, c_vp]),
    "dvae_train_eval": (c_i, [c_vp, c_vp, c_vp, c_vp, c_i, c_vp, c_i, c_vp, c_f, c_vp, c_vp]),
    "dvae_train_noise": (c_i, [c_vp, ctypes.c_uint64, c_vp, c_vp]),
    "dvae_module_forward": (c_i, [c_vp, c_vp, c_vp, c_vp, c_i, c_vp, c_i, c_vp, c_vp, c_i, c_vp, c_vp, c_vp, c_i, c_vp]),
    "dvae_module_backward": (c_i, [c_vp, c_vp, c_vp, c_vp, c_i, c_vp, c_i, c_vp, c_vp, c_i, c_vp, c_vp, c_vp, c_vp, c_i, c_vp]),
    "dvae_train_profile": (c_i, [c_i]),
    "dvae_train_debug_stamps": (c_i, [c_vp]),
    "dvae_mcem_debug_stamps": (c_i, [c_vp]),
    "dvae_train_profile_read": (c_i, [c_vp, c_vp]),
    "dvae_comm_create": (c_i, [c_i, c_i, c_i64, c_vp, c_vp]),
    "dvae_comm_connect": (c_i, [c_vp, c_vp]),
    "dvae_allreduce_flat": (c_i, [c_vp, c_vp, c_i, c_i64, c_vp, c_vp]),
    "dvae_comm_set_timeout_ms": (c_i, [c_vp, c_i64]),
    "dvae_comm_status": (c_i, [c_vp, c_vp]),
    "dvae_comm_destroy": (c_i, [c_vp]),
    "dvae_mcem_plan": (c_i, [c_i, c_i, c_vp]),
    "dvae_mcem_pack": (c_i, [c_vp, c_vp, c_i, c_vp, c_vp, c_i, c_vp, c_vp, c_i, c_vp, c_vp, c_vp]),
    "dvae_mcem_sample": (c_i, [c_vp, c_vp, c_vp, c_vp, c_vp, c_vp, c_vp, c_vp, c_vp, c_i, c_i, c_f, c_i64, c_vp, c_vp, c_vp, c_vp, c_vp]),
    "dvae_mcem_decode": (c_i, [c_vp, c_vp, c_vp, c_vp, c_i, c_i64, c_vp, c_vp]),
    "dvae_mcem_m_step_workspace_bytes": (c_sz, [c_i64, c_i, c_i]),
    "dvae_mcem_m_step_batch": (c_i, [c_vp, c_vp, c_i, c_i64, c_i, c_i, c_vp, c_vp, c_vp, c_vp, c_vp, c_vp, c_vp, c_vp, c_vp, c_vp]),
    "dvae_mcem_m_step": (c_i, [c_vp, c_vp, c_i, c_i64, c_i, c_vp, c_vp, c_vp, c_vp, c_vp, c_vp, c_vp]),
    "dvae_mcem_em_iteration": (c_i, [c_vp, c_vp, c_vp, c_vp, c_vp, c_vp, c_vp, c_vp, c_vp, c_i, c_i, c_f, c_i64, c_i, c_i, c_vp, c_vp, c_vp, c_vp, c_vp,
                                     c_vp, c_vp, c_vp, c_vp, c_vp]),
    "dvae_mcem_em_iteration_lazy": (c_i, [c_vp, c_vp, c_vp, c_vp, c_vp, c_vp, c_vp, c_vp, c_vp, c_i, c_i, c_f, c_i64, c_i, c_i, c_vp, c_vp, c_vp, c_vp, c_vp,
                                     c_vp, c_vp, c_vp, c_vp, c_vp]),
    "dvae_mcem_cost_flush": (c_i, [c_i, c_i64, c_i, c_i, c_vp, c_vp, c_vp, c_vp, c_vp]),
    "dvae_mcem_wiener": (c_i, [c_vp, c_i, c_i64, c_vp, c_vp, c_vp, c_vp, c_vp]),
    "dvae_mcem_spec_init": (c_i, [c_vp, c_i64, c_i, c_vp, c_vp, c_i64, c_vp]),
}


def load(path=None):
    global _lib
    if _lib is not None and path is None:
        return _lib
    p = path or LIB_PATH
    if not os.path.exists(p):
        raise RuntimeError(
            f"libdvae_hip.so not found at {p}: build it with `python disentangled-vae_amd/build.py` "
            "(there is no CPU fallback for CUDA tensors)")
    lib = ctypes.CDLL(p)
    for name, (res, args) in SIGNATURES.items():
        fn = getattr(lib, name)
        fn.restype = res
        fn.argtypes = args
    if lib.dvae_abi_version() != ABI_VERSION:
        raise RuntimeError(f"libdvae_hip.so ABI {lib.dvae_abi_version()} != binding {ABI_VERSION}")
    if path is None:
        _lib = lib
    return lib


def is_built():
    return os.path.exists(LIB_PATH)


def check(rc, what):
    if rc != 0:
        msg = load().dvae_last_error().decode("utf-8", "replace")
        raise RuntimeError(f"{what} failed (code {rc}): {msg}")


_raw_stream = getattr(torch._C, "_cuda_getCurrentRawStream", None)


def stream():
    if _raw_stream is not None:
        return ctypes.c_void_p(_raw_stream(torch.cuda.current_device()))
    return ctypes.c_void_p(torch.cuda.current_stream().cuda_stream)


def ptr(t):
    return None if t is None else ctypes.c_void_p(t.data_ptr())


def as_f32_2d(t, what):
    if not t.is_cuda:
        raise RuntimeError(f"{what}: expected a CUDA tensor")
    if t.dtype != torch.float32:
        raise TypeError(f"{what}: the HIP path computes in float32, got {t.dtype}")
    t2 = t.reshape(-1, t.shape[-1])
    if t2.stride(-1) != 1 or (t2.shape[0] > 1 and t2.stride(0) < t2.shape[1]):
        t2 = t2.contiguous()
    return t2


def ld(t2):
    return t2.stride(0) if t2.shape[0] > 1 else max(t2.shape[1], 1)
```

### include/dvae_train.h

```cpp
#ifndef DVAE_TRAIN_H
#define DVAE_TRAIN_H

#include <stddef.h>
#include <stdint.h>

#ifdef __cplusplus
extern "C" {
#endif

enum { DVAE_MODEL_M1 = 1, DVAE_MODEL_M2 = 2, DVAE_MODEL_M2_INFO = 3,
       DVAE_MODEL_M2_DEC = 4 };
enum { DVAE_PREC_F32 = 0, DVAE_PREC_BF16 = 1, DVAE_PREC_BF16X3 = 2 };
#define DVAE_TRAIN_MAX_TENSORS 32

typedef struct {
    int32_t model;
    int32_t y_dim;
    int32_t precision;
    int32_t ksplit;
    int64_t B;
    int32_t n_tensors;
    int32_t reserved0;
    int64_t n_params;
    int64_t tensor_offset[DVAE_TRAIN_MAX_TENSORS];
    int32_t tensor_rows[DVAE_TRAIN_MAX_TENSORS];
    int32_t tensor_cols[DVAE_TRAIN_MAX_TENSORS];
    int64_t workspace_bytes;
    int64_t grad_offset_bytes;
    int64_t Bp;
    int64_t rows_grid;
    double  flops_per_step;
    double  min_hbm_bytes_per_step;
    double  info_alpha, info_beta, info_gamma;
    uint64_t rng_seed;
    uint64_t rng_step;
    uint64_t loss_accum;
    uint64_t row_index;
    int64_t  row_count;
    uint64_t bad_row_counter;
    int32_t  rows_kernel;
    int32_t  reserved1;
} dvae_train_plan_t;

int dvae_train_plan(int model, int y_dim, int precision, int64_t B, int ksplit_hint, dvae_train_plan_t* plan);

int dvae_train_init(const dvae_train_plan_t* plan, const float* params, void* ws, void* stream);

int dvae_train_grads(const dvae_train_plan_t* plan, const float* params, void* ws, const float* x, int ldx,
                     const float* y, int ldy, const float* eps_noise, float elbo_eps, int reduce_slabs, void* stream);

int dvae_train_grads_group(const dvae_train_plan_t* plan, const float* params, void* ws, const float* x, int ldx, const float* y, int ldy,
                           const float* eps_noise, float elbo_eps, int group, int reduce_slabs, void* stream);
int dvae_train_group_range(const dvae_train_plan_t* plan, int group, int64_t* lo, int64_t* hi, int* ngroups);

int dvae_train_apply(const dvae_train_plan_t* plan, float* params, float* m, float* v, void* ws, int n_slabs,
                     int step, double lr, double beta1, double beta2, double adam_eps, double grad_scale,
                     float* losses3, void* stream);

int dvae_train_step(const dvae_train_plan_t* plan, float* params, float* m, float* v, void* ws,
                    const float* x, int ldx, const float* y, int ldy, const float* eps_noise, float elbo_eps,
                    int step, double lr, double beta1, double beta2, double adam_eps, float* losses3, void* stream);

int dvae_train_step_deferred(const dvae_train_plan_t* plan, float* params, float* m, float* v, void* ws,
                             const float* x, int ldx, const float* y, int ldy, const float* eps_noise, float elbo_eps,
                             int step, double lr, double beta1, double beta2, double adam_eps, float* losses3, void* stream);
int dvae_train_flush(const dvae_train_plan_t* plan, void* ws, void* stream);
int dvae_train_pending(const void* ws);
int dvae_train_can_defer(const dvae_train_plan_t* plan, const void* ws);

int dvae_train_eval(const dvae_train_plan_t* plan, const float* params, void* ws, const float* x, int ldx,
                    const float* y, int ldy, const float* eps_noise, float elbo_eps, float* losses3, void* stream);

int dvae_module_forward(const dvae_train_plan_t* plan, const float* params, void* ws, const float* x, int ldx,
                        const float* y, int ldy, const float* eps_noise, float* out_r, int ld_r, float* out_mu,
                        float* out_lv, float* out_z, int repack, void* stream);
int dvae_module_backward(const dvae_train_plan_t* plan, const float* params, void* ws, const float* x, int ldx,
                         const float* y, int ldy, const float* eps_noise, const float* g_r, int ld_gr,
                         const float* g_mu, const float* g_lv, const float* g_z, float* grad_flat, int accumulate, void* stream);

int dvae_train_noise(const dvae_train_plan_t* plan, uint64_t step, float* eps_out, void* stream);

int dvae_train_repack(const dvae_train_plan_t* plan, const float* params, void* ws, void* stream);

int dvae_train_profile(int enable);
int dvae_train_debug_stamps(void* buf);
int dvae_train_profile_read(double ms[4], int64_t calls[4]);

#define DVAE_IPC_HANDLE_BYTES 128
typedef struct dvae_comm dvae_comm_t;
int dvae_comm_create(int rank, int world, int64_t n_floats, dvae_comm_t** out, unsigned char handle[DVAE_IPC_HANDLE_BYTES]);
int dvae_comm_connect(dvae_comm_t* c, const unsigned char* handles );
int dvae_allreduce_flat(dvae_comm_t* c, const float* slabs, int n_slabs, int64_t slab_stride, float* out, void* stream);
int dvae_comm_set_timeout_ms(dvae_comm_t* c, int64_t ms);
int dvae_comm_status(dvae_comm_t* c, int* failed);
int dvae_comm_destroy(dvae_comm_t* c);

#ifdef __cplusplus
}
#endif
#endif
```

Before: 109.0 million frames/s.

## Stash binary label inputs as packed bit planes for weight-gradient reads

```diff
diff --git a/disentangled-vae_amd/csrc/rows_common.hpp b/disentangled-vae_amd/csrc/rows_common.hpp
--- a/disentangled-vae_amd/csrc/rows_common.hpp
+++ b/disentangled-vae_amd/csrc/rows_common.hpp
@@ -64,6 +64,7 @@
     int ablate;
     int stash_inputs;
     unsigned* ylo_epoch; unsigned launch_id; int ylo_skip; int* ylo_dirty;
+    unsigned char* ybT; unsigned* ybit_tile; unsigned* ynonbin_epoch;
     DeferArgs defer;
 };
 
@@ -94,9 +95,19 @@
 #endif
 }
 
+__device__ __forceinline__ void stash_store8(void* base_uniform, int voff_bytes, unsigned v) {
+#if R2_STASH_AUX == 0
+    *((unsigned char*)base_uniform + voff_bytes) = (unsigned char)v;
+#else
+    const __amdgpu_buffer_rsrc_t rs = __builtin_amdgcn_make_buffer_rsrc(base_uniform, 0, 0x7fffffff, 0x00020000);
+    __builtin_amdgcn_raw_buffer_store_b8((unsigned char)v, rs, voff_bytes, 0, R2_STASH_AUX);
+#endif
+}
+
 template <typename P, bool SRC16 = false>
 __device__ __forceinline__ void stash_tile(const typename P::T* lds, int ldl, int fbase, typename P::T* stash_tile_ptr, int64_t spl,
-                                           int64_t b0, int l31, int h, float scale = 1.f, int col_limit = 1 << 30, int nplanes = P::NP) {
+                                           int64_t b0, int l31, int h, float scale = 1.f, int col_limit = 1 << 30, int nplanes = P::NP,
+                                           unsigned char* bits_tile = nullptr) {
     typedef typename P::T T;
     typedef typename P::Frag Frag;
     constexpr int E = P::E;
@@ -118,6 +129,15 @@
                 s16x8 raw = {r0[0], r0[1], r0[2], r0[3], r1[0], r1[1], r1[2], r1[3]};
                 f[pl] = __builtin_bit_cast(Frag, raw);
             }
+            if (bits_tile != nullptr) {
+                const s16x8 raw = __builtin_bit_cast(s16x8, f[0]);
+                unsigned by = 0u;
+#pragma unroll
+                for (int j = 0; j < 8; ++j) by |= (raw[j] != 0 ? 1u : 0u) << j;
+                if (!keep) by = 0u;
+                stash_store8(bits_tile, (int)((b0 / P::KSTEP + i) * 64) + h * 32 + l31, by);
+                continue;
+            }
             if constexpr (SRC16 && P::NP == 2) {
 #pragma unroll
                 for (int j = 0; j < E; ++j) {
@@ -159,10 +179,15 @@
     }
 }
 
+__device__ __forceinline__ unsigned nonbinary_bits(float v) {
+    const unsigned u = __float_as_uint(v), w = u ^ 0x3F800000u;
+    return u < w ? u : w;
+}
+
 template <typename P, bool F16 = false, typename RowOf>
 __device__ __forceinline__ void load_rows_to_lds(const float* __restrict__ src, int ld, int ncols, int pcols, int64_t b0, int64_t B,
                                                  typename P::T* U, int ldu, int tid, RowOf rowof, float* xf = nullptr,
-                                                 float* log2sum = nullptr, float eps = 0.f) {
+                                                 float* log2sum = nullptr, float eps = 0.f, unsigned* nonbin = nullptr) {
     const int total = TB * pcols;
     for (int idx = tid; idx < total; idx += 256) {
         const int row = idx / pcols, col = idx - row * pcols;
@@ -171,6 +196,7 @@
             v = src[rowof(row) * ld + col];
             if (log2sum && col < XD - 1) *log2sum += __builtin_amdgcn_logf(v + eps);
         }
+        if (nonbin) *nonbin |= nonbinary_bits(v);
         if constexpr (F16 && P::NP == 2) {
             const float vs = v * X16::XS;
             const typename P::T vh = X16::hi<typename P::T>(vs);
@@ -224,7 +250,8 @@
     __builtin_amdgcn_sched_barrier(0);
 }
 template <typename P, int I0, int I1, bool F16 = false>
-__device__ __forceinline__ void tile513_commit_part(const f32x4 (&v)[NQ513], typename P::T* U, int ldu, int tid, float* xf, unsigned long long& lo_bits) {
+__device__ __forceinline__ void tile513_commit_part(const f32x4 (&v)[NQ513], typename P::T* U, int ldu, int tid, float* xf, unsigned long long& lo_bits,
+                                                    unsigned* nonbin = nullptr, bool nonbin_on = false) {
     typedef typename P::Pack4 Pack4;
 #pragma unroll
     for (int i = I0; i < I1; ++i) {
@@ -249,6 +276,14 @@
         Pack4 pk;
         pk[0] = P::cvt(v[i][0]); pk[1] = P::cvt(v[i][1]); pk[2] = P::cvt(v[i][2]); pk[3] = P::cvt(v[i][3]);
         *reinterpret_cast<Pack4*>(U + row * ldu + col) = pk;
+        if (nonbin && nonbin_on) {
+            if constexpr (P::NP == 2) {
+                typedef unsigned int u32x2 __attribute__((ext_vector_type(2)));
+                const u32x2 w = __builtin_bit_cast(u32x2, pk);
+                *nonbin |= (w[0] & 0xC07FC07Fu) | ((w[0] ^ (w[0] >> 1)) & 0x1F801F80u);
+                *nonbin |= (w[1] & 0xC07FC07Fu) | ((w[1] ^ (w[1] >> 1)) & 0x1F801F80u);
+            } else *nonbin |= nonbinary_bits(v[i][0]) | nonbinary_bits(v[i][1]) | nonbinary_bits(v[i][2]) | nonbinary_bits(v[i][3]);
+        }
         if constexpr (P::NP == 2) {
             Pack4 pl;
             pl[0] = P::cvt(v[i][0] - (float)pk[0]); pl[1] = P::cvt(v[i][1] - (float)pk[1]);
@@ -259,9 +294,11 @@
     }
 }
 template <typename P, int PCOLS, bool F16 = false>
-__device__ __forceinline__ void tile513_commit_last(const f32x4 (&v)[NQ513], typename P::T* U, int ldu, int tid, float* xf, unsigned long long& lo_bits) {
+__device__ __forceinline__ void tile513_commit_last(const f32x4 (&v)[NQ513], typename P::T* U, int ldu, int tid, float* xf, unsigned long long& lo_bits,
+                                                    unsigned* nonbin = nullptr, bool nonbin_on = false) {
     constexpr int PADC = PCOLS - XD;
     if (tid < TB) {
+        if (nonbin && nonbin_on) *nonbin |= nonbinary_bits(v[16][0]);
         if (xf) xf[tid * XD + XD - 1] = v[16][0];
         if constexpr (F16 && P::NP == 2) {
             const float vs = v[16][0] * X16::XS;
@@ -285,11 +322,13 @@
     }
 }
 template <typename P, int PCOLS, bool F16 = false>
-__device__ __forceinline__ void tile513_commit(const f32x4 (&v)[NQ513], typename P::T* U, int ldu, int tid, float* xf = nullptr, bool* any_lo = nullptr) {
+__device__ __forceinline__ void tile513_commit(const f32x4 (&v)[NQ513], typename P::T* U, int ldu, int tid, float* xf = nullptr, bool* any_lo = nullptr,
+                                               unsigned* nonbin = nullptr, bool nonbin_on = false) {
     unsigned long long lo_bits = 0ull;
-    tile513_commit_part<P, 0, 16, F16>(v, U, ldu, tid, xf, lo_bits);
-    tile513_commit_last<P, PCOLS, F16>(v, U, ldu, tid, xf, lo_bits);
+    tile513_commit_part<P, 0, 16, F16>(v, U, ldu, tid, xf, lo_bits, nonbin, nonbin_on);
+    tile513_commit_last<P, PCOLS, F16>(v, U, ldu, tid, xf, lo_bits, nonbin, nonbin_on);
     if (any_lo) *any_lo = lo_bits != 0ull;
+    if constexpr (P::NP == 2) { if (nonbin && nonbin_on && lo_bits != 0ull) *nonbin |= 1u; }
 }
 template <typename P, int Q0, int Q1, typename RowOf>
 __device__ __forceinline__ void xstash_reload(const float* __restrict__ src, int ld, RowOf rowof, int64_t b0, int64_t B, typename P::T* xT,
@@ -340,14 +379,16 @@
 
 template <typename P, bool SRC16 = false>
 __device__ __forceinline__ void stash_from_lds(const typename P::T* U, int ldu, int pcols, int srows, typename P::T* stash, int64_t spl,
-                                               int64_t Bp, int64_t b0, int tid, int ft0 = 0, int ft1 = 1 << 30, int nplanes = P::NP) {
+                                               int64_t Bp, int64_t b0, int tid, int ft0 = 0, int ft1 = 1 << 30, int nplanes = P::NP,
+                                               unsigned char* bits = nullptr) {
     typedef typename P::Frag Frag;
     constexpr int E = P::E;
     if constexpr (sizeof(typename P::T) == 2) {
         const int lane = tid & 63, wave = __builtin_amdgcn_readfirstlane(tid >> 6);
         const int fte = ft1 < srows / 32 ? ft1 : srows / 32;
         for (int ft = ft0 + wave; ft < fte; ft += 4)
-            stash_tile<P, SRC16>(U, ldu, 32 * ft, stash + (int64_t)ft * 32 * Bp, spl, b0, lane & 31, lane >> 5, 1.f, pcols, nplanes);
+            stash_tile<P, SRC16>(U, ldu, 32 * ft, stash + (int64_t)ft * 32 * Bp, spl, b0, lane & 31, lane >> 5, 1.f, pcols, nplanes,
+                                 bits ? bits + (int64_t)ft * 4 * Bp : nullptr);
         return;
     }
     constexpr int groups = TB / E;
diff --git a/disentangled-vae_amd/csrc/rows_helper.inc b/disentangled-vae_amd/csrc/rows_helper.inc
--- a/disentangled-vae_amd/csrc/rows_helper.inc
+++ b/disentangled-vae_amd/csrc/rows_helper.inc
@@ -121,7 +121,7 @@
                         Binfo[i] = v;
                     }
                 }
-                if (ht == 0) flags[0] = 0;
+                if (ht == 0) { flags[0] = 0; flags[1] = 0; }
                 if constexpr (DEFER) {
                     wg_barrier();
                     load_bias();
@@ -155,6 +155,7 @@
             int yplanes = NP;
             int ydirty = 0;
             if constexpr (NP == 2 && YP > 0) { if (g.ylo_skip && st2) ydirty = g.ylo_dirty[tile]; }
+            unsigned char* ybits = nullptr;
             if (YP > 0) {
                 if (Y513 && yfast && !y_early) tile513_issue(g.y, rowof, yv, tl);
                 R2_HSTAMP(16);
@@ -164,8 +165,11 @@
                 if constexpr (HS::HELPY && HS::n(H_W1X) == 0) hws.fill();
                 R2_HSTAMP(18);
                 bool any = false;
-                if (Y513 && yfast) tile513_commit<P, ROWS_XP>(yv, U, LDU, tl, nullptr, NP == 2 ? &any : nullptr);
-                else load_rows_to_lds<P>(g.y, g.ldy, g.ydim, YP, b0, g.B, U, LDU, tl, rowof);
+                const bool ybit_on = sizeof(T) == 2 && g.ybT != nullptr && st2;
+                unsigned ynb = 0u;
+                if (Y513 && yfast) tile513_commit<P, ROWS_XP>(yv, U, LDU, tl, nullptr, NP == 2 ? &any : nullptr, sizeof(T) == 2 ? &ynb : nullptr, ybit_on);
+                else load_rows_to_lds<P>(g.y, g.ldy, g.ydim, YP, b0, g.B, U, LDU, tl, rowof, nullptr, nullptr, 0.f, sizeof(T) == 2 ? &ynb : nullptr);
+                if (ybit_on) { if (__ballot(ynb != 0u) != 0ull && lane == 0) atomicOr(&flags[1], 1); }
                 R2_HSTAMP(19);
                 if constexpr (NP == 2) {
                     if (Y513 && yfast) {
@@ -178,9 +182,13 @@
                 R2_HSTAMP(20);
                 if constexpr (INFO) put_lds<P>(c1r, U + IMA, LDU, 32 * hw, l31, h);
                 wg_barrier();
+                if (ybit_on && __builtin_amdgcn_readfirstlane(flags[1]) == 0) {
+                    ybits = g.ybT;
+                    if (ht == 0) g.ybit_tile[tile] = g.launch_id;
+                } else if (ybit_on && ht == 0) *g.ynonbin_epoch = g.launch_id;
                 if constexpr (NP == 2) {
                     const bool ylo_t = __builtin_amdgcn_readfirstlane(flags[0]) != 0;
-                    if (g.ylo_skip && st2) {
+                    if (g.ylo_skip && st2 && ybits == nullptr) {
                         ydirty = __builtin_amdgcn_readfirstlane(ydirty);
                         yplanes = (ylo_t || ydirty != 0) ? 2 : 1;
                         if (ht == 0) {
@@ -190,7 +198,7 @@
                     }
                 }
 #if !R2_LATE_Y
-                if (st2) stash_from_lds<P>(U, LDU, YP, (YP + 31) / 32 * 32, (T*)g.yT, g.spl, g.Bp, b0, tl, 0, 1 << 30, yplanes);
+                if (st2) stash_from_lds<P>(U, LDU, YP, (YP + 31) / 32 * 32, (T*)g.yT, g.spl, g.Bp, b0, tl, 0, 1 << 30, yplanes, ybits);
 #endif
                 if constexpr (HS::HELPY) {
                     const bool ylo = NP == 2 && __builtin_amdgcn_readfirstlane(flags[0]) != 0;
@@ -247,7 +255,7 @@
 #endif
             if constexpr (XFH && !INFO && R2_XSP == 0) { if (st2x) xstash_reload<P, 0, 4>(g.x, g.ldx, rowof, b0, g.B, (T*)g.xT, g.spl, g.Bp, tl); }
 #if R2_LATE_Y
-            if (YP > 0 && st2) stash_from_lds<P>(U, LDU, YP, (YP + 31) / 32 * 32, (T*)g.yT, g.spl, g.Bp, b0, tl, 0, R2_YSPREAD, yplanes);
+            if (YP > 0 && st2) stash_from_lds<P>(U, LDU, YP, (YP + 31) / 32 * 32, (T*)g.yT, g.spl, g.Bp, b0, tl, 0, R2_YSPREAD, yplanes, ybits);
 #endif
             wg_barrier();
             if constexpr (INFO) {
@@ -269,7 +277,7 @@
                 }
             }
 #if R2_LATE_Y
-            if (YP > 0 && st2) stash_from_lds<P>(U, LDU, YP, (YP + 31) / 32 * 32, (T*)g.yT, g.spl, g.Bp, b0, tl, R2_YSPREAD, 1 << 30, yplanes);
+            if (YP > 0 && st2) stash_from_lds<P>(U, LDU, YP, (YP + 31) / 32 * 32, (T*)g.yT, g.spl, g.Bp, b0, tl, R2_YSPREAD, 1 << 30, yplanes, ybits);
 #endif
             wg_barrier();
             if constexpr (HS::HELPY) {
@@ -284,7 +292,7 @@
             }
             if (hw == 0 && st1) stash_tile<P>(Zb, LDZ, 0, (T*)g.zT, g.spl, b0, l31, h);
             if constexpr (XFH && !INFO && R2_XSP == 2) { if (st2x) xstash_reload<P, 5, 9>(g.x, g.ldx, rowof, b0, g.B, (T*)g.xT, g.spl, g.Bp, tl); }
-            if (ht == 0) flags[0] = 0;
+            if (ht == 0) { flags[0] = 0; flags[1] = 0; }
             if constexpr (INFO) {
                 if (st1) stash_tile<P>(U + IMA, LDU, 32 * hw, (T*)g.dc1T + (int64_t)hw * 32 * g.Bp, g.spl, b0, l31, h, g.alpha);
                 const float sa = g.gamma - g.beta;
diff --git a/disentangled-vae_amd/csrc/train_fused.hip b/disentangled-vae_amd/csrc/train_fused.hip
--- a/disentangled-vae_amd/csrc/train_fused.hip
+++ b/disentangled-vae_amd/csrc/train_fused.hip
@@ -22,7 +22,7 @@
     bool info;
     int ld1, ld3, yp, ye, yd;
     int64_t xT, yT, h1T, h2T, dh1T, dh2T, dmlvT, zT, d1T, d2T, dd1T, dd2T, daT, stash_rows;
-    int64_t o_tiles, o_blocks, o_blocks4, o_items4, o_tensors, o_chunks, o_partials, o_flags, o_defer, o_wcopy, o_stash, o_grads, total;
+    int64_t o_tiles, o_blocks, o_blocks4, o_items4, o_tensors, o_chunks, o_partials, o_flags, o_defer, o_wcopy, o_stash, o_ybits, o_grads, total;
     int ntiles, nblocks, nblocks4;
 };
 constexpr int DEFER_MAX_TASKS = 640;
@@ -83,10 +83,11 @@
     L.o_tensors = bytes(DVAE_TRAIN_MAX_TENSORS * sizeof(TensorDesc));
     L.o_chunks = bytes(p.n_params / 64 + 64);
     L.o_partials = bytes(p.rows_grid * 4 * sizeof(double));
-    L.o_flags = bytes(1024 + 4 * (p.Bp / TB + 1));
+    L.o_flags = bytes(1024 + 2 * 4 * (p.Bp / TB + 1));
     L.o_defer = bytes(DEFER_BYTES);
     L.o_wcopy = bytes(L.wcopy_elems * esz * np);
     L.o_stash = bytes(L.stash_rows * p.Bp * esz * np);
+    L.o_ybits = bytes((L.yp ? al(L.yp, 32) / 32 : 0) * 4 * p.Bp);
     L.o_grads = bytes((int64_t)p.ksplit * p.n_params * sizeof(float));
     L.total = b;
     return 0;
@@ -206,6 +207,8 @@
     plan->min_hbm_bytes_per_step = 4.0 * (XD + y_dim + ZD) * (double)B;
     return 0;
 }
+
+static bool label_bits_env() { return env_int("DVAE_LABEL_BITS", 1) != 0; }
 
 static int64_t kper_of(const dvae_train_plan_t* p) {
     const int ks = is_bf(p->precision) ? 16 : 8;
@@ -376,6 +379,9 @@
 static std::unordered_map<const void*, W4Grids> g_w4_grid;
 static void w4_grid_put(const void* ws, const W4Grids& grids) { std::lock_guard<std::mutex> lk(g_fold_mu); g_w4_grid[ws] = grids; }
 static int w4_grid_get(const void* ws, int table) { std::lock_guard<std::mutex> lk(g_fold_mu); auto it = g_w4_grid.find(ws); return it == g_w4_grid.end() ? -1 : it->second.g[table]; }
+static std::unordered_map<const void*, unsigned> g_label_mode;
+static void label_mode_put(const void* ws, unsigned id) { std::lock_guard<std::mutex> lk(g_fold_mu); g_label_mode[ws] = id; }
+static unsigned label_mode_get(const void* ws) { std::lock_guard<std::mutex> lk(g_fold_mu); auto it = g_label_mode.find(ws); return it == g_label_mode.end() ? 0u : it->second; }
 static unsigned fold_seq_next(const void* ws) { std::lock_guard<std::mutex> lk(g_fold_mu); return ++g_fold_seq[ws]; }
 static void fold_seq_reset(const void* ws) { std::lock_guard<std::mutex> lk(g_fold_mu); g_fold_seq.erase(ws); }
 
@@ -460,11 +466,12 @@
     for (int k = 0; k < 4; ++k) { if (b.At[k]) na = k + 1; if (b.Bt[k]) nb = k + 1; bias = bias || b.bias_off[k] >= 0; }
     const bool x3 = p.precision == DVAE_PREC_BF16X3, bf = is_bf(p.precision);
     const bool one_plane_b = x3 && b.raw == 2 && p.rows_kernel >= 2;
+    const bool bits_b = bf && b.raw == 2 && p.rows_kernel >= 2 && label_bits_env();
     double mfma, load, fsum;
     static const double kb_clocks = getenv("DVAE_W4_KB_CLOCKS") ? atof(getenv("DVAE_W4_KB_CLOCKS")) : 70.0;
     if (bf) {
         mfma = (double)na * nb * (x3 ? (one_plane_b ? 2 : 3) : 1) * 32.0;
-        load = ((double)na * (x3 ? 2 : 1) + (double)nb * (x3 ? (one_plane_b ? 1 : 2) : 1)) * kb_clocks;
+        load = ((double)na * (x3 ? 2 : 1) + (double)nb * (bits_b ? 1.0 / 16 : (x3 ? (one_plane_b ? 1 : 2) : 1))) * kb_clocks;
         fsum = bias ? (double)na * (x3 ? 2 : 1) * 16 * 4 * 0.5 : 0.0;
     } else {
         mfma = (double)na * nb * 2 * 4 * 64.0;
@@ -750,6 +757,7 @@
     int raw_inputs = -1;
     int64_t raw_auto_b = env_ll("DVAE_RAW_AUTO_B", 131072);
     bool ylo_always = getenv("DVAE_YLO_ALWAYS") != nullptr;
+    bool label_bits = label_bits_env();
     int wgrad_repeat = std::max(env_int("DVAE_WGRAD_REPEAT", 1), 1);
     int gpw = env_int("DVAE_GPW", 2);
     unsigned fold_max_polls = 1u << 20;
@@ -815,6 +823,8 @@
     a.stash_inputs = 3 & ~raw_mask;
     a.mode = o.mode;
     a.ylo_epoch = (unsigned*)(w + L.o_flags); a.ylo_dirty = (int*)(w + L.o_flags + 1024);
+    a.ybT = nullptr;
+    a.ybit_tile = (unsigned*)(w + L.o_flags + 1024) + (plan->Bp / TB + 1); a.ynonbin_epoch = (unsigned*)(w + L.o_flags) + 3;
     static std::atomic<unsigned> launch_counter{1};
     if (o.group == 1) {
         DVAE_CHECK_ARG(g_pairing.last_ws == w && g_pairing.last_id != 0, "train_grads_group: group 1 must follow a group 0 call on the same workspace");
@@ -886,8 +896,9 @@
                     fin_block = (int)g3.x; fin_err = a.defer.err;
                     g3l = dim3(g3.x + 1);
                 }
+                const YBits yb{a.ybT, a.ybit_tile, a.ynonbin_epoch};
                 const Wgrad4Args w4a{bl, w4items, ks, plan->Bp, a.spl, slabs, plan->n_params, ri, use_raw,
-                                     a.ylo_skip ? a.ylo_epoch : nullptr, x3 ? a.launch_id : 0u , fa_apply, fold, fin_block, fin_err};
+                                     a.ylo_skip ? a.ylo_epoch : nullptr, (x3 || a.ybT) ? a.launch_id : 0u , yb, fa_apply, fold, fin_block, fin_err};
                 const int rc = launch_wgrad4(plan->precision, w4a, (int)g3l.x, s);
                 if (rc) return rc;
             }
@@ -924,6 +935,10 @@
     const bool wg4 = env.wgrad_form == 4 && (plan->Bp > 128 || a.stash_inputs != 3  || env.wgrad_set);
     a.ylo_skip = (plan->precision == DVAE_PREC_BF16X3 && plan->y_dim > 0 && plan->rows_kernel >= 2 && rows2_supported(plan->precision, plan->model) && wg4 &&
                   (a.stash_inputs & 2) && !env.ylo_always) ? 1 : 0;
+    if (is_bf(plan->precision) && plan->y_dim > 0 && plan->rows_kernel >= 2 && rows2_supported(plan->precision, plan->model) && wg4 &&
+        (a.stash_inputs & 2) && o.mode == 0 && env.label_bits)
+        a.ybT = (unsigned char*)ws + L.o_ybits;
+    label_mode_put(ws, a.ybT != nullptr && !o.rows_only ? a.launch_id : 0u);
     DVAE_CHECK_ARG(o.group < 0 || (w4_grouped(*plan) && o.mode == 0 && !o.rows_only), "train_grads_group: the plan was not made for two weight-gradient launches (DVAE_EXCHANGE_GROUPS=2 when the plan is made)");
     if (o.group != 1) {
         ProfScope ps(s, 0);
@@ -1034,6 +1049,21 @@
     return launch_slab_sum(slabs, plan->n_params, used_slabs(plan), plan->n_params, grad_flat, accumulate, (hipStream_t)stream);
 }
 
+extern "C" int dvae_train_debug_label_mode(const dvae_train_plan_t* plan, const void* ws, void* stream) {
+    DVAE_CHECK_ARG(plan && ws, "train_debug_label_mode: bad argument");
+    const unsigned id = label_mode_get(ws);
+    if (id == 0u) return 0;
+    Layout L;
+    make_layout(*plan, L);
+    unsigned epoch = 0u;
+    if (hipStreamSynchronize((hipStream_t)stream) != hipSuccess ||
+        hipMemcpy(&epoch, (const char*)ws + L.o_flags + 3 * sizeof(unsigned), sizeof(unsigned), hipMemcpyDeviceToHost) != hipSuccess) {
+        set_error("train_debug_label_mode: reading the workspace failed");
+        return -1;
+    }
+    return epoch == id ? 2 : 1;
+}
+
 extern "C" int dvae_train_debug_stamps(void* buf) {
     g_dbg = (unsigned long long*)buf;
     return 0;
diff --git a/disentangled-vae_amd/csrc/train_wgrad.hip b/disentangled-vae_amd/csrc/train_wgrad.hip
--- a/disentangled-vae_amd/csrc/train_wgrad.hip
+++ b/disentangled-vae_amd/csrc/train_wgrad.hip
@@ -238,9 +238,10 @@
     static constexpr size_t BYTES = (size_t)(8 * 16) * 64 * 16 + 12 * 64 * 4;
 };
 
-template <typename P, int NA, int NB, int RAW, bool BLO = true, bool BIAS = true>
+template <typename P, int NA, int NB, int RAW, bool BLO = true, bool BIAS = true, int YB = 0>
 __device__ __forceinline__ void wgrad4_body(const Block4& bd, const Block4* __restrict__ bdg, char* wsm, int slice, int64_t Bp, int64_t spl, int64_t kbeg, int64_t kend_,
-                                            float* __restrict__ slabs, int64_t slab_stride, int lane, int wave, const RawIn& ri) {
+                                            float* __restrict__ slabs, int64_t slab_stride, int lane, int wave, const RawIn& ri,
+                                            const YBits& yb = YBits{}, unsigned launch_id = 0u) {
     typedef typename P::T T;
     typedef typename P::Frag Frag;
     typedef Wg4<P> W;
@@ -273,7 +274,16 @@
 #pragma unroll
             for (int r = 0; r < 16; ++r) c[i][j][r] = 0.f;
     float bs[4] = {0.f, 0.f, 0.f, 0.f};
-    Frag a[RD][NA][NP], b[RAW == 1 ? 1 : (RAW == 2 ? 1 : RD)][RAW == 1 ? 1 : NB][NP];
+    static_assert(YB == 0 || (RAW == 0 && sizeof(T) == 2 && E == 8 && TB == 2 * KS), "label bits: stash-fed blocks of the 16-bit operand policies");
+    Frag a[RD][NA][NP], b[(RAW == 1 || RAW == 2 || YB == 1) ? 1 : RD][(RAW == 1 || YB == 1) ? 1 : NB][NP];
+    unsigned ybyte[YB ? RD : 1][YB ? NB : 1], ytile[YB == 2 ? RD : 1];
+    typedef const __attribute__((address_space(1))) unsigned char* gbyte;
+    typedef const __attribute__((address_space(1))) unsigned* gword;
+    gbyte ybp[YB ? NB : 1];
+    if constexpr (YB != 0) {
+#pragma unroll
+        for (int k = 0; k < NB; ++k) ybp[k] = (gbyte)(uintptr_t)(yb.plane + (int64_t)((bd.Bt[k] ? bd.rcol[k] : bd.rcol[0]) >> 5) * 4 * Bp) + lane;
+    }
     float braw[RAW == 1 ? RD : 1][RAW == 1 ? NB : 1][E];
     f32x4 rawq[RAW == 2 ? RD : 1][RAW == 2 ? 8 : 1];
     typedef const __attribute__((address_space(1))) float* gflt;
@@ -310,12 +320,29 @@
                 rawq[s][u] = reinterpret_cast<const __attribute__((address_space(1))) F4U*>(rsrc + fr * rld + rcol4)->v;
             }
         } else {
-#pragma unroll
-            for (int k = 0; k < NB; ++k) {
-                b[s][k][0] = *(gfrag)(bp[k] + o + loff);
-                if constexpr (NP == 2 && BLO) b[s][k][1] = *(gfrag)(bp[k] + plb + o + loff);
-            }
-        }
+            if constexpr (YB != 1) {
+#pragma unroll
+                for (int k = 0; k < NB; ++k) {
+                    b[s][k][0] = *(gfrag)(bp[k] + o + loff);
+                    if constexpr (NP == 2 && BLO) b[s][k][1] = *(gfrag)(bp[k] + plb + o + loff);
+                }
+            }
+            if constexpr (YB != 0) {
+#pragma unroll
+                for (int k = 0; k < NB; ++k) ybyte[s][k] = ybp[k][sk * 64];
+                if constexpr (YB == 2) ytile[s] = ((gword)(uintptr_t)yb.tile)[sk >> 1];
+            }
+        }
+    };
+    auto ydecode = [&](unsigned by) __attribute__((always_inline)) {
+        typedef unsigned int u32x4_ __attribute__((ext_vector_type(4)));
+        u32x4_ w;
+#pragma unroll
+        for (int q = 0; q < 4; ++q) {
+            const unsigned t = by >> (2 * q);
+            w[q] = (t & 1u) * 0x3F80u + (t & 2u) * 0x1FC00000u;
+        }
+        return __builtin_bit_cast(Frag, w);
     };
     auto fsum = [&](const Frag& f) __attribute__((always_inline)) {
         float t = 0.f;
@@ -384,6 +411,34 @@
                 }
 #pragma unroll
                 for (int i = 0; i < NA; ++i) mmap<P>(c[i][j], a[s][i], bj);
+            }
+            if constexpr (BIAS) {
+#pragma unroll
+                for (int i = 0; i < NA; ++i) {
+                    bs[i] += fsum(a[s][i][0]);
+                    if constexpr (NP == 2) bs[i] += fsum(a[s][i][1]);
+                }
+            }
+        } else if constexpr (YB != 0) {
+            typedef unsigned int u32x4_ __attribute__((ext_vector_type(4)));
+#pragma unroll
+            for (int j = 0; j < NB; ++j) {
+                Frag bj[NP];
+                bj[0] = ydecode(ybyte[s][j]);
+                if constexpr (NP == 2) bj[1] = __builtin_bit_cast(Frag, u32x4_{0u, 0u, 0u, 0u});
+                if constexpr (YB == 2) {
+                    const bool bit_tile = ytile[s] == launch_id;
+#pragma unroll
+                    for (int pl = 0; pl < NP; ++pl) {
+                        const u32x4_ d = __builtin_bit_cast(u32x4_, bj[pl]), m = __builtin_bit_cast(u32x4_, b[s][j][pl]);
+                        u32x4_ r;
+#pragma unroll
+                        for (int q = 0; q < 4; ++q) r[q] = bit_tile ? d[q] : m[q];
+                        bj[pl] = __builtin_bit_cast(Frag, r);
+                    }
+                }
+#pragma unroll
+                for (int i = 0; i < NA; ++i) mmap<P>(c[i][j], a[s][i], bj, YB == 2);
             }
             if constexpr (BIAS) {
 #pragma unroll
@@ -630,7 +685,7 @@
 template <typename P>
 __global__ __launch_bounds__(256, 1) void wgrad4_kernel(const Block4* __restrict__ blocks, const W4Item* __restrict__ items, int ksplit, int64_t Bp,
                                                         int64_t spl, float* __restrict__ slabs, int64_t slab_stride,
-                                                        const RawIn ri, int use_raw, const unsigned* __restrict__ ylo_epoch, unsigned launch_id,
+                                                        const RawIn ri, int use_raw, const unsigned* __restrict__ ylo_epoch, unsigned launch_id, const YBits yb,
                                                         const ApplyArgs fold_apply, const FoldArgs fold, int fin_block, const unsigned* fin_err) {
     extern __shared__ __attribute__((aligned(16))) char wsm[];
     const int lane = threadIdx.x & 63;
@@ -650,6 +705,7 @@
     for (int k = 0; k < 4; ++k) { if (bd.At[k] != nullptr) na = k + 1; if (bd.Bt[k] != nullptr) nb = k + 1; }
 #define W4_GO_(NA_, NB_, RAW_, BLO_) wgrad4_body<P, NA_, NB_, RAW_, BLO_, true>(bd, blocks + bi, wsm, slice, Bp, spl, it.kbeg, it.kend, slabs, slab_stride, lane, wave, ri)
 #define W4_GO(NA_, NB_, RAW_) W4_GO_(NA_, NB_, RAW_, true)
+#define W4_GOY(NB_, YB_) wgrad4_body<P, 4, NB_, 0, true, true, YB_>(bd, blocks + bi, wsm, slice, Bp, spl, it.kbeg, it.kend, slabs, slab_stride, lane, wave, ri, yb, launch_id)
     bool raw = false;
     if constexpr (sizeof(typename P::T) == 2) raw = (use_raw & bd.raw) != 0;
     if (raw) {
@@ -658,6 +714,18 @@
             else if (nb == 1) W4_GO(4, 1, 1);
             else if (nb == 2) W4_GO(4, 2, 1);
             else W4_GO(4, 4, 1);
+        }
+    } else if (sizeof(typename P::T) == 2 && bd.raw == 2 && yb.plane != nullptr) {
+        if constexpr (sizeof(typename P::T) == 2) {
+            if (*yb.nonbin_epoch != launch_id) {
+                if (nb == 1) W4_GOY(1, 1);
+                else if (nb == 2) W4_GOY(2, 1);
+                else W4_GOY(4, 1);
+            } else {
+                if (nb == 1) W4_GOY(1, 2);
+                else if (nb == 2) W4_GOY(2, 2);
+                else W4_GOY(4, 2);
+            }
         }
     } else if (sizeof(typename P::T) == 2 && P::NP == 2 && bd.raw == 2 && ylo_epoch != nullptr && *ylo_epoch != launch_id) {
         if (nb == 1) W4_GO_(4, 1, 0, false);
@@ -672,6 +740,7 @@
         else if (nb == 2) W4_GO(4, 2, 0);
         else W4_GO(4, 4, 0);
     }
+#undef W4_GOY
 #undef W4_GO
 #undef W4_GO_
 #ifndef W4_FOLD
@@ -791,7 +860,7 @@
         static bool attr_done[64] = {};
         if (!attr_done[dev]) { DVAE_HIP(hipFuncSetAttribute((const void*)wgrad4_kernel<P>, hipFuncAttributeMaxDynamicSharedMemorySize, (int)Wg4<P>::BYTES)); attr_done[dev] = true; }
         hipLaunchKernelGGL((wgrad4_kernel<P>), dim3((unsigned)grid), dim3(256), Wg4<P>::BYTES, s, a.blocks, a.items, a.ksplit, a.Bp, a.spl, a.slabs, a.slab_stride, a.ri, a.use_raw,
-                           a.ylo_epoch, a.launch_id, a.fold_apply, a.fold, a.fin_block, a.fin_err);
+                           a.ylo_epoch, a.launch_id, a.yb, a.fold_apply, a.fold, a.fin_block, a.fin_err);
         return 0;
     });
     if (rc) return rc;
diff --git a/disentangled-vae_amd/csrc/wgrad_types.hpp b/disentangled-vae_amd/csrc/wgrad_types.hpp
--- a/disentangled-vae_amd/csrc/wgrad_types.hpp
+++ b/disentangled-vae_amd/csrc/wgrad_types.hpp
@@ -50,6 +50,8 @@
 
 struct RawIn { const float* x; const float* y; int ldx, ldy; int64_t B; };
 
+struct YBits { const unsigned char* plane; const unsigned* tile; const unsigned* nonbin_epoch; };
+
 constexpr int FOLD_MAXB = 120;
 struct FoldArgs { unsigned* cnt; unsigned target; unsigned max_polls; };
 
@@ -58,7 +60,7 @@
 int launch_wgrad_lds(int precision, const BlockDesc* blocks, int nblocks, const WgradArgs& a, hipStream_t s);
 struct Wgrad4Args {
     const Block4* blocks; const W4Item* items; int ksplit; int64_t Bp, spl; float* slabs; int64_t slab_stride;
-    RawIn ri; int use_raw; const unsigned* ylo_epoch; unsigned launch_id;
+    RawIn ri; int use_raw; const unsigned* ylo_epoch; unsigned launch_id; YBits yb;
     ApplyArgs fold_apply; FoldArgs fold; int fin_block; const unsigned* fin_err;
 };
 int launch_wgrad4(int precision, const Wgrad4Args& a, int grid, hipStream_t s);
diff --git a/disentangled-vae_amd/native.py b/disentangled-vae_amd/native.py
--- a/disentangled-vae_amd/native.py
+++ b/disentangled-vae_amd/native.py
@@ -91,6 +91,7 @@
     "dvae_module_backward": (c_i, [c_vp, c_vp, c_vp, c_vp, c_i, c_vp, c_i, c_vp, c_vp, c_i, c_vp, c_vp, c_vp, c_vp, c_i, c_vp]),
     "dvae_train_profile": (c_i, [c_i]),
     "dvae_train_debug_stamps": (c_i, [c_vp]),
+    "dvae_train_debug_label_mode": (c_i, [c_vp, c_vp, c_vp]),
     "dvae_mcem_debug_stamps": (c_i, [c_vp]),
     "dvae_train_profile_read": (c_i, [c_vp, c_vp]),
     "dvae_comm_create": (c_i, [c_i, c_i, c_i64, c_vp, c_vp]),
diff --git a/include/dvae_train.h b/include/dvae_train.h
--- a/include/dvae_train.h
+++ b/include/dvae_train.h
@@ -84,6 +84,7 @@
 
 int dvae_train_profile(int enable);
 int dvae_train_debug_stamps(void* buf);
+int dvae_train_debug_label_mode(const dvae_train_plan_t* plan, const void* ws, void* stream);
 int dvae_train_profile_read(double ms[4], int64_t calls[4]);
 
 #define DVAE_IPC_HANDLE_BYTES 128
```

Result: slower. 104.9 million frames/s (-3.8%).
